# ielab/llm-rankers

Measured on AMD Instinct MI355X. Metric: passages/sec (pointwise yes_no reranking, flan-t5-large shape), higher is better.
Workload: dtype f16 (MFMA inputs), f32 accumulate + residual stream

## Files before the change

### llm-rankers_amd/csrc/rk_engine.hip

```cpp
#include <hip/hip_runtime.h>
#include <dlfcn.h>
#include <rccl/rccl.h>

#include <algorithm>
#include <cmath>
#include <cstdarg>
#include <cstdio>
#include <cstdlib>
#include <cstring>
#include <map>
#include <atomic>
#include <string>
#include <vector>

#include "../../include/rk_engine.h"
#include "attention.h"
#include "attention_d128.h"
#include "decoder_kernels.h"
#include "gemm.h"
#include "gemv_rows.h"
#include "llama_kernels.h"
#include "llama_kernels_hd64.h"
#include "llama_kernels_qknorm.h"
#include "misc_kernels.h"
// ... 36 lines not shown
struct Gemm;

struct NormStream {
  float* hidden = nullptr;
  half_t* xraw[2] = {nullptr, nullptr};
  float* ssq[2] = {nullptr, nullptr};
  float* factors = nullptr;
  half_t* xn = nullptr;
  int rows = 0; bool fold = false;
  int cur = 0, nb = 0;
  void begin(rk_engine* e, hipStream_t st, const int* ids, int rows_, bool fold_);
  const half_t* x() const { return fold ? xraw[cur] : xn; }
  Gemm consumer(rk_engine* e, hipStream_t st, const float* ln, Gemm c, bool own_factors) const;
  int producer(rk_engine* e, hipStream_t st, Gemm c, bool stats = true);
};

template <class T>
struct Grown {
  T* p = nullptr; size_t cap = 0;
  Grown() = default;
  Grown(const Grown&) = delete;
  Grown& operator=(const Grown&) = delete;
  ~Grown() { if (p) hipFree(p); }
  int reserve(rk_engine* e, size_t n, int* gen = nullptr);
};

enum DecBuf { IX_DEC_IDS, IX_OUT_IDS, IX_LAST_ROWS, IX_N_CACHED, IX_ROW_LABEL = IX_N_CACHED, IX_ROW_OFF, IX_OUT_IDX, IX_ROW_SEQ, IX_TREE_KEYS, IX_TREE_POS, IX_COUNT };
struct DecIndex {
  struct Src { DecBuf b; const std::vector<int>& v; };
  int* d[IX_COUNT] = {nullptr};
  int* pin = nullptr;
  static constexpr int PIN_INTS = 8192;
  int put(rk_engine* e, hipStream_t st, DecBuf b, const int* src, int n);
  int write(rk_engine* e, hipStream_t st, std::initializer_list<Src> srcs);
  int tree(rk_engine* e, hipStream_t st, std::vector<int>& sig, std::initializer_list<Src> srcs);
 private:
  std::vector<int> held[IX_N_CACHED], tree_sig;
  unsigned long epoch = 0, tree_epoch = ~0ul;
};

}

#define RK_SLOTS 2

struct Slot {
  hipStream_t se = nullptr, sd = nullptr;
  NormStream enc;
  half_t *qkv = nullptr, *ctx = nullptr, *ffh = nullptr, *enc_out = nullptr;
  int* d_tokens = nullptr; int* d_seq_off = nullptr;
  int* dec_seq_off = nullptr;
  int *stg_tokens[2] = {nullptr, nullptr}, *stg_seq_off[2] = {nullptr, nullptr};
  int gen = 0; bool gen_launched = false; unsigned stage_no = 0, off_of = 0;
  int n_seq = 0, T = 0, maxL = 0, minL = 0; bool staged = false; int last_floats = 0;
  half_t* cross_kv = nullptr;
  DecIndex idx; int* d_argmax = nullptr;
  NormStream dec;
  half_t *dqkv = nullptr, *dctx = nullptr, *dq = nullptr, *dffh = nullptr, *dlast = nullptr;
  float* dssq_few[2] = {nullptr, nullptr};
  half_t *xqk = nullptr, *xctx = nullptr;
  float *xpart = nullptr, *xstat = nullptr; bool have_cross_kv = false;
  float* d_scores = nullptr; float* h_scores = nullptr;
  hipEvent_t ev_enc[2] = {nullptr, nullptr}, ev_dec = nullptr; int enc_gen = -1; bool dec_pending = false;
};

struct rk_engine {
  rk_model_desc d{};
  int dev = 0;
  std::string err;
  bool finalized = false;
  int inner = 0;
  std::map<std::string, HostTensor> host;
  std::vector<void*> allocs;
  half_t *emb = nullptr, *lm_head = nullptr, *cross_kv_w = nullptr;
  std::vector<EncLayerW> enc;
  std::vector<DecLayerW> dec;
  float *enc_final_ln = nullptr, *dec_final_ln = nullptr, *lut_enc = nullptr, *lut_dec = nullptr;
  Grown<float> logits; int logits_gen = 0;
  Grown<float> amax_val; Grown<int> amax_idx; int amax_gen = 0;
  Grown<half_t> kv_cache; int kv_gen = 0;
  Grown<int> gen_buf; int* gen_pin = nullptr; hipEvent_t ev_gen[2] = {nullptr, nullptr};
  size_t scores_cap = 0;
  Slot slots[RK_SLOTS];
  struct Options {
    int glds = 1, skinny = 0x3F, overlap = 1, gemm_variant = 0, attn_short = 5, xattn_direct = 1, attn_heads_per_wg = 0, attn_ko = 0,
        gemm_persistent = 1, fold_norm = 1, s64_stages = 0, dec_fold_norm = 1, greedy_spec = 160, consumer_stats = 1, xattn_mfma = 1,
        dec_ffn_tiled = 1, gemm_split = 1, dec_fuse = 1, dec_fuse_rows = 0, dec_attn_seq = 1, attn_long = 1, attn_long_nw = 0,
        llama_attn_dma = 1, attn_long_xcd = 1, llama_attn_nw = 0, dec_graph = 1, gemm_sk = 1, dec_cross_mfma = 1, dec_gemv = 1, dec_gemv_rows = 4,
        dec_cached_attn = 1, llama_dec_r = 0, enc_serial = 0;
  } opt;
  float* attn_trace = nullptr;
  int n_cu = 256;
  struct SkWs { hipStream_t st = nullptr; float* slabs = nullptr; int* cnt = nullptr; };
  SkWs sk_ws[2 * RK_SLOTS];
  hipEvent_t t0 = nullptr, t1 = nullptr, t_tmp = nullptr;
  bool prof_on = false;
  std::vector<ProfRec> prof_recs; size_t prof_used = 0;
  double prof_flops[PC_COUNT] = {0}, prof_bytes[PC_COUNT] = {0}; int64_t prof_n[PC_COUNT] = {0};
  int family = 0; rk_llama_desc ld{};
  float rope_factor = 0.f, rope_low = 1.f, rope_high = 4.f; int rope_orig = 0;
  bool qkv_bias = false;
  bool qk_norm = false;
  int window = 0;
  std::vector<LlamaLayerW> ll; float *l_final_ln = nullptr, *rope_cos = nullptr, *rope_sin = nullptr; int* d_pos = nullptr;
  struct Sampling { float T = 0.f; int k = 0; float p = 1.f; bool on() const { return T > 0.f; } } samp;
  unsigned long long* d_seeds = nullptr;
  Grown<half_t> lkv; Grown<float> lpart; Grown<int> lints; int lkv_gen = 0;
  struct LlamaStep { NormStream stream; half_t *qkv = nullptr, *ctx = nullptr, *ffh = nullptr; } lg;
  struct LlamaSession {
    bool open = false; int n_slots = 0, max_len = 0, cap = 0, seen = 0;
    std::vector<int> busy, told, len, max_new, col, done;
    bool sampled = false; std::vector<unsigned long long> seeds;
  } ls;
  struct GraphEntry { int seen = 0; bool failed = false; hipGraphExec_t exec = nullptr; };
  std::map<std::vector<int>, GraphEntry> graphs; int opt_epoch = 0;
  struct GraphCount { int64_t eager = 0, captures = 0, replays = 0, failed = 0, evictions = 0; } graph_count;
  ncclComm_t comm = nullptr; int comm_rank = 0, comm_world = 1;
  float* d_gather[RK_SLOTS] = {nullptr}; float* h_gather[RK_SLOTS] = {nullptr}; size_t gather_cap = 0;
  hipEvent_t ev_gather[RK_SLOTS] = {nullptr}; bool gather_pending[RK_SLOTS] = {false}; int gather_n[RK_SLOTS] = {0};
  float *d_gsend = nullptr, *d_gall = nullptr, *h_gall = nullptr, *h_gstage = nullptr;
  hipEvent_t ev_gall = nullptr, ev_append = nullptr; bool gall_pending = false, append_foreign = false; int gall_n = 0;
};

namespace {

int fail(rk_engine* e, int code, const char* fmt, ...) {
  char buf[1024];
  va_list ap;
  va_start(ap, fmt);
  vsnprintf(buf, sizeof buf, fmt, ap);
  va_end(ap);
  if (e) e->err = buf; else g_create_error = buf;
  return code;
}

#define HIPCHK(E, call)                                                                              \
  do {                                                                                               \
    hipError_t _s = (call);                                                                          \
    if (_s != hipSuccess) return fail((E), RK_ERR_HIP, "%s failed: %s", #call, hipGetErrorString(_s)); \
  } while (0)
#define RC(x) do { rc = (x); if (rc) return rc; } while (0)

template <class T>
int dalloc(rk_engine* e, T** p, size_t n) {
  void* q = nullptr;
  HIPCHK(e, hipMalloc(&q, std::max<size_t>(n, 1) * sizeof(T)));
  e->allocs.push_back(q);
  *p = (T*)q;
  return RK_OK;
}

template <class T>
int upload(rk_engine* e, T** p, const T* src, size_t n) {
  int rc = dalloc(e, p, n);
  if (rc) return rc;
  HIPCHK(e, hipMemcpy(*p, src, n * sizeof(T), hipMemcpyHostToDevice));
  return RK_OK;
}

struct Bracket {
  rk_engine* e; hipStream_t st; int idx = -1;
  Bracket(rk_engine* e_, hipStream_t st_, int cls, double flops, double bytes) : e(e_), st(st_) {
    if (!e->prof_on) return;
    if (e->prof_used == e->prof_recs.size()) {
      ProfRec r{};
      if (hipEventCreate(&r.a) != hipSuccess || hipEventCreate(&r.b) != hipSuccess) return;
      e->prof_recs.push_back(r);
    }
    idx = (int)e->prof_used++;
    e->prof_recs[idx].cls = cls;
    e->prof_flops[cls] += flops; e->prof_bytes[cls] += bytes; e->prof_n[cls]++;
    hipEventRecord(e->prof_recs[idx].a, st);
  }
  ~Bracket() { if (idx >= 0) hipEventRecord(e->prof_recs[idx].b, st); }
};

hipStream_t enc_stream(rk_engine* e, Slot& sl) { return e->opt.overlap ? e->slots[(&sl - e->slots) & 1].se : e->slots[0].se; }
hipStream_t dec_stream(rk_engine* e, Slot& sl) { return e->opt.overlap ? sl.sd : e->slots[0].se; }

template <auto K, class Args>
void launch_lds(hipStream_t st, dim3 grid, dim3 block, int lds, int opt_in, const Args& a) {
  static std::atomic<uint64_t> done{0};
  if (opt_in > 0) {
    int dev = 0;
    if (hipGetDevice(&dev) != hipSuccess) dev = 0;
    const uint64_t bit = 1ull << (dev & 63);
    if (!(done.load(std::memory_order_acquire) & bit)) {
      hipError_t rc = hipFuncSetAttribute((const void*)K, hipFuncAttributeMaxDynamicSharedMemorySize, opt_in);
      if (rc != hipSuccess) fprintf(stderr, "[rk_engine] hipFuncSetAttribute(%d B LDS) failed: %s\n", opt_in, hipGetErrorString(rc));
      done.fetch_or(bit, std::memory_order_release);
    }
  }
  hipLaunchKernelGGL(K, grid, block, lds, st, a);
}

// ... 748 lines not shown
  else launch_lds<attn_causal128_dma_kernel<4>>(st, p.grid, p.block, p.lds, p.lds_opt_in, a);
}
int refuse_window(rk_engine* e, const char* entry, int maxL) {
  return fail(e, RK_ERR_STATE, "%s: a sequence of %d tokens on an engine with sliding window %d needs a windowed attention kernel, and option llama_attn_dma = 0 selects attn_causal128_kernel, which has none", entry, maxL, e->window);
}

struct LlamaDecAttnPlan { int R = 1, nch = 1, hd = 128, window = 0; dim3 grid, cgrid; };
LlamaDecAttnPlan plan_llama_dec_attn(const rk_engine* e, int rows, int P, int n_heads, int n_kv) {
  LlamaDecAttnPlan p;
  const int G = n_heads / n_kv;
  p.hd = head_width(e);
  p.R = G % 8 == 0 ? 8 : (G % 4 == 0 ? 4 : (G % 2 == 0 ? 2 : 1));
  if (e->opt.llama_dec_r == 1) p.R = 1;
  if (e->opt.llama_dec_r == 2 && G == 7 && p.hd == 128) p.R = 7;
  p.nch = (P + LDC_CHUNK - 1) / LDC_CHUNK;
  p.grid = dim3(p.nch, n_heads / p.R, rows);
  p.cgrid = dim3(n_heads, rows);
  p.window = e->window;
  return p;
}

void launch_llama_dec_attn(rk_engine* e, hipStream_t st, const LlamaDecAttnPlan& p, LlamaDecAttnArgs a, int rows) {
  a.nch = p.nch; a.window = p.window;
  Bracket br(e, st, PC_DEC_ATTN, 4.0 * rows * (double)a.P * a.n_heads * p.hd, 2.0 * rows * (double)a.P * a.n_kv * p.hd * 2.0);
  with_width(p.hd, [&](auto W) {
    constexpr int D = decltype(W)::value;
    auto go = [&](auto rc) {
      constexpr int R = decltype(rc)::value;
      if constexpr (R == 7 && D != 128) abort();
      else if (a.qkn) {
        if constexpr (D == 128) hipLaunchKernelGGL((attn_dec_cached_qkn_kernel<D, R>), p.grid, dim3(256), 0, st, a);
        else abort();
      }
      else if (p.window > 0) {
        if (a.bias) hipLaunchKernelGGL((attn_dec_cached_win_kernel<D, R, true>), p.grid, dim3(256), 0, st, a);
        else hipLaunchKernelGGL((attn_dec_cached_win_kernel<D, R, false>), p.grid, dim3(256), 0, st, a);
      }
      else if (a.bias) hipLaunchKernelGGL((attn_dec_cached_kernel<D, R, true>), p.grid, dim3(256), 0, st, a);
      else hipLaunchKernelGGL((attn_dec_cached_kernel<D, R, false>), p.grid, dim3(256), 0, st, a);
    };
    using std::integral_constant;
    switch (p.R) {
      case 8: go(integral_constant<int, 8>{}); break;
      case 7: go(integral_constant<int, 7>{}); break;
      case 4: go(integral_constant<int, 4>{}); break;
      case 2: go(integral_constant<int, 2>{}); break;
      default: go(integral_constant<int, 1>{}); break;
    }
    if (p.window > 0) hipLaunchKernelGGL(attn_dec_combine_win_kernel<D>, p.cgrid, dim3(D), 0, st, a);
    else hipLaunchKernelGGL(attn_dec_combine_kernel<D>, p.cgrid, dim3(D), 0, st, a);
  });
}

int wait_prev_decoder(rk_engine* e, Slot& sl) {
  hipStream_t se = enc_stream(e, sl);
  if (sl.dec_pending && dec_stream(e, sl) != se) HIPCHK(e, hipStreamWaitEvent(se, sl.ev_dec, 0));
  return RK_OK;
}

int run_encoder(rk_engine* e, Slot& sl, bool need_cross_kv) {
  const rk_model_desc& d = e->d;
  hipStream_t st = enc_stream(e, sl);
  const int T = sl.T, I = e->inner, dm = d.d_model, F = d.d_ff;
  const bool own = e->opt.consumer_stats != 0;
  int rc = RK_OK;
  NormStream ns = sl.enc;
  const EncAttnPlan ap = plan_enc_attn(e, sl.n_seq, sl.maxL, sl.minL, d.n_heads);
  const int* seq_off = sl.stg_seq_off[sl.gen];
  ns.begin(e, st, sl.stg_tokens[sl.gen], T, e->opt.fold_norm != 0);
  for (int l = 0; l < d.n_enc_layers; ++l) {
    const EncLayerW& w = e->enc[l];
    const bool last = l + 1 == d.n_enc_layers;
    RC(gemm(e, st, ns.consumer(e, st, w.ln0, Gemm(PC_ENC_GEMM_QKV, EPI_STORE_F16, ns.x(), dm, ns.fold ? w.qkv_f : w.qkv, dm, sl.qkv, 3 * I, T, 3 * I, dm), own)));
    launch_enc_attn(e, st, EncAttnCall{sl.qkv, sl.ctx, seq_off, e->lut_enc, 3 * I, I, I, d.n_heads, sl.n_seq, sl.maxL, sl.T}, ap);
    RC(ns.producer(e, st, Gemm(PC_ENC_GEMM_O, EPI_RESID_F32, sl.ctx, I, w.o, I, ns.hidden, dm, T, dm, I)));
    RC(gemm(e, st, ns.consumer(e, st, w.ln1, Gemm(PC_ENC_GEMM_FFN_IN, d.gated_gelu ? EPI_GEGLU_F16 : EPI_RELU_F16, ns.x(), dm, ns.fold ? w.ffn_in_f : w.ffn_in, dm,
                                                 sl.ffh, F, T, d.gated_gelu ? 2 * F : F, dm), own)));
    RC(ns.producer(e, st, Gemm(PC_ENC_GEMM_FFN_OUT, EPI_RESID_F32, sl.ffh, F, w.ffn_out, F, ns.hidden, dm, T, dm, F), !last));
  }
  RC(wait_prev_decoder(e, sl));
  if (sl.off_of != sl.stage_no) {
    HIPCHK(e, hipMemcpyAsync(sl.dec_seq_off, seq_off, (size_t)(sl.n_seq + 1) * sizeof(int), hipMemcpyDeviceToDevice, st));
    sl.off_of = sl.stage_no;
  }
  rmsnorm(e, st, ns.hidden, e->enc_final_ln, sl.enc_out, nullptr, T);
  if (need_cross_kv)
    RC(gemm(e, st, Gemm(PC_GEMM_CROSS_KV, EPI_STORE_F16, sl.enc_out, dm, e->cross_kv_w, dm, sl.cross_kv, 2 * I, T, d.n_dec_layers * 2 * I, dm)
                       .split(2 * I, (long)d.max_tokens * 2 * I)));
  sl.have_cross_kv = need_cross_kv;
  HIPCHK(e, hipGetLastError());
  return RK_OK;
}

struct DecRows {
  int rows; const int* keys; const int* pos; const int* seq;
  const int* row_off; int seq0, n_seq; bool cross_kv; const int* ids;
  bool tree() const { return keys != nullptr; }
};
struct DecCache { half_t* kv; int P; const int* pos; const int* tree_keys; int* tree_pos; };
void launch_dec_cached_step(const rk_engine* e, hipStream_t st, const AttnCachedArgs& ca, int B, int H, const int* tree_keys, int* tree_pos) {
  if (e->opt.dec_cached_attn) {
    hipLaunchKernelGGL(attn_dec_cached_kernel, dim3(H, B), dim3(256), attn_dec_lds(ca.P), st, ca);
  } else {
    hipLaunchKernelGGL(kv_append_kernel, dim3(B), dim3(256), 0, st, ca, tree_pos);
    hipLaunchKernelGGL(attn_dec_kernel, dim3(1, H, B), dim3(256), attn_dec_lds(ca.P), st,
                       AttnDecArgs{ca.qkv, ca.ldqkv, ca.cache, ca.cache + ca.inner, 2 * ca.inner, nullptr, ca.ctx, ca.ldctx, ca.bias_lut, ca.P, 1, ca.P,
                                   tree_keys, tree_pos});
  }
}
int run_decoder(rk_engine* e, Slot& sl, int Ld, const DecRows* rows = nullptr, const DecCache* cache = nullptr) {
  const rk_model_desc& d = e->d;
  hipStream_t st = dec_stream(e, sl);
  const bool tree = rows && rows->tree(), ragged = rows && !rows->tree();
  const int B = ragged ? rows->n_seq : sl.n_seq, M = rows ? rows->rows : B * Ld, I = e->inner, dm = d.d_model, F = d.d_ff;
  const bool have_kv = ragged ? rows->cross_kv : sl.have_cross_kv;
  const int* seq_off = sl.dec_seq_off + (ragged ? rows->seq0 : 0);
  const DecLenClass lc = dec_len_class(e, Ld);
  if (tree && (have_kv || lc.one)) return fail(e, RK_ERR_STATE, "the tree form needs the query-side cross-attention and L_d >= 2");
  if (ragged && have_kv && !sl.have_cross_kv) return fail(e, RK_ERR_STATE, "the ragged pass needs the K / V the encoder did not materialise");
  if (cache && (rows || have_kv || Ld != 1)) return fail(e, RK_ERR_STATE, "the incremental pass needs the query-side cross-attention and one row per sequence");
  if (wide_heads(e) && (!lc.one || rows || cache || have_kv || e->opt.dec_fuse == 2))
    return refuse_wide(e, "run_decoder", "this pass would launch a 64-wide kernel");
  const bool ws = lc.stream;
  const bool dfold = ws && e->opt.dec_fold_norm && (e->opt.skinny & 0x3F) == 0x3F;
  const bool fuse_asked = e->opt.dec_fuse == 2 || (e->opt.dec_fuse == 1 && lc.one);
  const bool few = dfold && e->opt.dec_gemv && !lc.one && M <= e->opt.dec_gemv_rows && !fuse_asked &&
                   gemv_fits(M, dm) && gemv_fits(M, I) && gemv_fits(M, F);
  const GemmFamily fam = few ? GEMM_GEMV : (ws ? GEMM_STREAM : GEMM_TILED);
  int rc = RK_OK;
  NormStream ns = sl.dec;
  if (few) { ns.ssq[0] = sl.dssq_few[0]; ns.ssq[1] = sl.dssq_few[1]; }
  auto normed = [&](const float* ln, Gemm c) { return ns.consumer(e, st, ln, c.on(fam), true); };
  auto resid = [&](Gemm c, bool stats = true) { return ns.producer(e, st, c.on(fam), stats); };
  ns.begin(e, st, ragged && rows->ids ? rows->ids : sl.idx.d[IX_DEC_IDS], M, dfold);
  const DecAttnPlan self_plan = plan_dec_attn(e, false, B, Ld, Ld, d.n_heads, tree ? rows->rows : 0);
  const DecAttnPlan cross_plan = plan_dec_attn(e, true, B, Ld, sl.maxL, d.n_heads, 0);
  for (int l = 0; l < d.n_dec_layers; ++l) {
    const DecLayerW& w = e->dec[l];
    if (!cache && lc.one) {
      RC(resid(normed(w.ln0, Gemm(PC_DEC_GEMM, EPI_RESID_F32, ns.x(), dm, dfold ? w.ov_f : w.ov, dm, ns.hidden, dm, M, dm, dm))));
    } else {
      RC(gemm(e, st, normed(w.ln0, Gemm(PC_DEC_GEMM, EPI_STORE_F16, ns.x(), dm, dfold ? w.qkv_f : w.qkv, dm, sl.dqkv, 3 * I, M, 3 * I, dm))));
      if (cache) {
        const AttnCachedArgs ca{sl.dqkv, 3 * I, cache->kv + (size_t)l * B * cache->P * 2 * I, cache->P, I, cache->pos, sl.dctx, I, e->lut_dec};
        Bracket br(e, st, PC_DEC_ATTN, 4.0 * B * (double)cache->P * I, (double)B * cache->P * 2 * I * 2.0);
        launch_dec_cached_step(e, st, ca, B, d.n_heads, cache->tree_keys, cache->tree_pos);
      } else {
        launch_dec_attn(e, st, self_plan, AttnDecArgs{sl.dqkv, 3 * I, sl.dqkv + I, sl.dqkv + 2 * I, 3 * I, nullptr, sl.dctx, I, e->lut_dec, Ld, 1, Ld,
                                                      tree ? rows->keys : nullptr, tree ? rows->pos : nullptr, 0, ragged ? rows->row_off : nullptr},
                        4.0 * M * Ld * I, 0);
      }
      RC(resid(Gemm(PC_DEC_GEMM, EPI_RESID_F32, sl.dctx, I, w.o, I, ns.hidden, dm, M, dm, I)));
    }
    const Gemm cq = normed(w.ln1, Gemm(PC_DEC_GEMM, EPI_STORE_F16, ns.x(), dm, dfold ? w.cq_f : w.cq, dm, sl.dq, I, M, I, dm));
    if (!have_kv) {
      RC(run_xattn_chain(e, st, XAttnChain{cq.A, cq.lda, cq.W, w.ckT, e->cross_kv_w + ((size_t)l * 2 * I + I) * dm, cq.fold, cq.family,
                                           sl.enc_out, sl.dec_seq_off, rows ? rows->seq : nullptr, Ld, 0, sl.dq, sl.xqk, sl.xpart, sl.xstat, sl.xctx,
                                           sl.dctx, I, M, d.n_heads, dm, sl.maxL, sl.T, fuse_asked, head_width(e)}));
    } else {
      RC(gemm(e, st, cq));
      const half_t* kv = sl.cross_kv + (size_t)l * d.max_tokens * 2 * I;
      launch_dec_attn(e, st, cross_plan, AttnDecArgs{sl.dq, I, kv, kv + I, 2 * I, seq_off, sl.dctx, I, nullptr, Ld, 0, sl.maxL, nullptr, nullptr, 0,
                                                       ragged ? rows->row_off : nullptr},
                      4.0 * Ld * (double)sl.T * I, (double)sl.T * 2 * I * 2.0);
    }
    RC(resid(Gemm(PC_DEC_GEMM, EPI_RESID_F32, sl.dctx, I, w.co, I, ns.hidden, dm, M, dm, I)));
    {
      const bool tiled_in = dfold && e->opt.dec_ffn_tiled && lc.one;
      RC(gemm(e, st, ns.consumer(e, st, w.ln2, Gemm(PC_DEC_GEMM, d.gated_gelu ? EPI_GEGLU_F16 : EPI_RELU_F16, ns.x(), dm, dfold ? w.ffn_in_f : w.ffn_in, dm,
                                                   sl.dffh, F, M, d.gated_gelu ? 2 * F : F, dm).on(tiled_in ? GEMM_TILED : fam), true)));
    }
    RC(resid(Gemm(PC_DEC_GEMM, EPI_RESID_F32, sl.dffh, F, w.ffn_out, F, ns.hidden, dm, M, dm, F), l + 1 < d.n_dec_layers));
  }
  HIPCHK(e, hipGetLastError());
  return RK_OK;
}

int encoder_then_handoff_kv(rk_engine* e, Slot& sl, bool need_cross_kv) {
  hipStream_t se = enc_stream(e, sl), sd = dec_stream(e, sl);
  if (need_cross_kv && !sl.cross_kv) return refuse_wide(e, "encoder", "the materialised cross-attention K / V are not allocated");
  static_assert(RK_SLOTS == 2, "the other slot");
  const Slot& other = e->slots[(&sl - e->slots) ^ 1];
  if (e->opt.enc_serial && sd != se && other.enc_gen >= 0) HIPCHK(e, hipStreamWaitEvent(se, other.ev_enc[other.enc_gen], 0));
  sl.gen_launched = true;
  const int rc = run_encoder(e, sl, need_cross_kv);
  HIPCHK(e, hipEventRecord(sl.ev_enc[sl.gen], se));
  sl.enc_gen = sl.gen;
  if (rc) return rc;
  if (sd != se) HIPCHK(e, hipStreamWaitEvent(sd, sl.ev_enc[sl.gen], 0));
  return RK_OK;
}

int encoder_then_handoff(rk_engine* e, Slot& sl, int max_ld, bool query_side = false) {
  return encoder_then_handoff_kv(e, sl, !query_side && !use_xattn_direct(e, sl, max_ld));
}

int mark_decoder_done(rk_engine* e, Slot& sl) {
  HIPCHK(e, hipEventRecord(sl.ev_dec, dec_stream(e, sl)));
  sl.dec_pending = true;
  return RK_OK;
}

int sync_all(rk_engine* e) {
  for (Slot& sl : e->slots) {
    HIPCHK(e, hipStreamSynchronize(sl.se));
    HIPCHK(e, hipStreamSynchronize(sl.sd));
  }
  return RK_OK;
}

int finish_blocking(rk_engine* e, Slot& sl) {
  int rc = mark_decoder_done(e, sl);
  if (rc || (rc = sync_all(e))) return rc;
  sl.dec_pending = false;
  return RK_OK;
}

template <class T>
int Grown<T>::reserve(rk_engine* e, size_t n, int* gen) {
  if (n <= cap) return RK_OK;
  int rc = sync_all(e);
  if (rc) return rc;
  if (p) HIPCHK(e, hipFree(p));
  p = nullptr; cap = 0;
  HIPCHK(e, hipMalloc((void**)&p, n * sizeof(T)));
  cap = n;
  if (gen) ++*gen;
  return RK_OK;
}

int ensure_logits(rk_engine* e, size_t rows) {
  return e->logits.reserve(e, rows * (2 * ((size_t)(e->d.vocab + 31) / 32) + 1), &e->logits_gen);
}

float head_scale(const rk_engine* e) {
  return e->d.tied_head ? 1.0f / std::sqrt((float)e->d.d_model) : 1.0f;
}

int check_batch(rk_engine* e, Slot* sl, const int32_t* tokens, const int32_t* off, int n_seq) {
  if (!e->finalized) return fail(e, RK_ERR_STATE, "engine not finalized");
  if (!tokens || !off || n_seq <= 0) return fail(e, RK_ERR_INVALID, "empty batch (n_seq=%d)", n_seq);
  if (n_seq > e->d.max_seqs) return fail(e, RK_ERR_CAPACITY, "n_seq %d > max_seqs %d", n_seq, e->d.max_seqs);
  if (off[0] != 0) return fail(e, RK_ERR_INVALID, "seq_offsets[0] must be 0");
  int maxL = 0, minL = 1 << 30;
  for (int b = 0; b < n_seq; ++b) {
    const int L = off[b + 1] - off[b];
    if (L <= 0) return fail(e, RK_ERR_INVALID, "sequence %d is empty", b);
    maxL = std::max(maxL, L);
    minL = std::min(minL, L);
  }
  const int T = off[n_seq];
  if (T > e->d.max_tokens) return fail(e, RK_ERR_CAPACITY, "%d tokens > max_tokens %d", T, e->d.max_tokens);
  for (int t = 0; t < T; ++t)
    if (tokens[t] < 0 || tokens[t] >= e->d.vocab) return fail(e, RK_ERR_INVALID, "token id %d out of range at %d", tokens[t], t);
  if (attn_dec_lds(maxL) > 160 * 1024 || maxL > 65536)
    return fail(e, RK_ERR_CAPACITY, "sequence of %d tokens exceeds the cross-attention LDS budget", maxL);
  if (sl) { sl->maxL = maxL; sl->minL = minL; sl->T = T; sl->n_seq = n_seq; }
  return RK_OK;
}

int check_ids(rk_engine* e, const int32_t* ids, int n, const char* what) {
  for (int i = 0; i < n; ++i)
    if (ids[i] < 0 || ids[i] >= e->d.vocab) return fail(e, RK_ERR_INVALID, "%s id %d out of range", what, ids[i]);
  return RK_OK;
}

int put_dec_ids_shared(rk_engine* e, Slot& sl, const int32_t* prefix, int Ld) {
  std::vector<int> ids((size_t)sl.n_seq * Ld);
  for (int b = 0; b < sl.n_seq; ++b) memcpy(&ids[(size_t)b * Ld], prefix, Ld * sizeof(int));
  return sl.idx.put(e, dec_stream(e, sl), IX_DEC_IDS, ids.data(), (int)ids.size());
}

void shift_right(const int32_t* labels, int n, std::vector<int>* out) {
  for (int t = 0; t < n; ++t) out->push_back(t ? labels[t - 1] : 0);
}

int check_greedy_args(rk_engine* e, const int32_t* dec_prefix, int dec_len, int max_new) {
  if (!dec_prefix || dec_len <= 0 || max_new <= 0 || dec_len + max_new - 1 > e->d.max_dec_len)
    return fail(e, RK_ERR_CAPACITY, "dec_len %d + max_new %d exceeds max_dec_len %d", dec_len, max_new, e->d.max_dec_len);
  return RK_OK;
}

int read_scores_blocking(rk_engine* e, Slot& sl, hipStream_t st, size_t n, float* out) {
  HIPCHK(e, hipMemcpyAsync(sl.h_scores, sl.d_scores, n * sizeof(float), hipMemcpyDeviceToHost, st));
  if (e->family == 0) { const int rc = finish_blocking(e, sl); if (rc) return rc; }
  else HIPCHK(e, hipStreamSynchronize(st));
  HIPCHK(e, hipGetLastError());
  memcpy(out, sl.h_scores, n * sizeof(float));
  return RK_OK;
}

int stage_slot(rk_engine* e, int slot, const int32_t* tokens, const int32_t* seq_offsets, int n_seq) {
  if (slot < 0 || slot >= RK_SLOTS) return fail(e, RK_ERR_INVALID, "slot %d out of range", slot);
  if (e->family != 0) return fail(e, RK_ERR_STATE, "T5 entry point called on a Llama engine (use rk_llama_*)");
  int rc = set_device(e);
  if (rc) return rc;
  Slot& sl = e->slots[slot];
  sl.staged = false;
  if ((rc = check_batch(e, &sl, tokens, seq_offsets, n_seq))) return rc;
  const int g = sl.gen_launched ? sl.gen ^ 1 : sl.gen;
  HIPCHK(e, hipEventSynchronize(sl.ev_enc[g]));
  HIPCHK(e, hipMemcpy(sl.stg_tokens[g], tokens, (size_t)sl.T * sizeof(int), hipMemcpyHostToDevice));
  HIPCHK(e, hipMemcpy(sl.stg_seq_off[g], seq_offsets, (size_t)(n_seq + 1) * sizeof(int), hipMemcpyHostToDevice));
  sl.gen = g; sl.gen_launched = false; ++sl.stage_no;
  sl.staged = true;
  return RK_OK;
}

enum GraphKind { GK_T5_SCORE, GK_T5_GREEDY_STEP, GK_T5_GREEDY2, GK_T5_GENERATE_STEP, GK_LLAMA_STEP, GK_T5_COMPARE, GK_LLAMA_SESSION_STEP, GK_LLAMA_STEP_SAMPLED, GK_LLAMA_SESSION_STEP_SAMPLED };
int evict_graphs(rk_engine* e, const rk_engine::GraphEntry* keep) {
  for (Slot& sl : e->slots) HIPCHK(e, hipStreamSynchronize(sl.sd));
  HIPCHK(e, hipStreamSynchronize(e->slots[0].se));
  for (auto it = e->graphs.begin(); it != e->graphs.end();) {
    if (&it->second == keep) { ++it; continue; }
    if (it->second.exec) { hipGraphExecDestroy(it->second.exec); ++e->graph_count.evictions; }
    it = e->graphs.erase(it);
  }
  return RK_OK;
}
template <class F>
int run_graphed(rk_engine* e, hipStream_t st, std::vector<int> key, F&& body) {
  auto& n = e->graph_count;
  auto eager = [&]() -> int { ++n.eager; return body(); };
  key.push_back(e->opt_epoch);
  if (!e->opt.dec_graph || e->prof_on) return eager();
  auto& g = e->graphs[key];
  if (g.exec) { HIPCHK(e, hipGraphLaunch(g.exec, st)); ++n.replays; return RK_OK; }
  if ((int)e->graphs.size() > RK_GRAPH_CACHE_KEYS) {
    const int rc = evict_graphs(e, &g);
    if (rc) return rc;
  }
  if (g.failed || g.seen++ == 0) return eager();
  auto failed = [&]() -> int { g.failed = true; ++n.failed; return eager(); };
  hipGraph_t graph = nullptr;
  if (hipStreamBeginCapture(st, hipStreamCaptureModeThreadLocal) != hipSuccess) { (void)hipGetLastError(); return failed(); }
  const int rc = body();
  const hipError_t ec = hipStreamEndCapture(st, &graph);
  if (rc != RK_OK || ec != hipSuccess || !graph) {
    (void)hipGetLastError();
    if (graph) hipGraphDestroy(graph);
    if (rc != RK_OK) { g.failed = true; ++n.failed; return rc; }
    return failed();
  }
  const hipError_t ei = hipGraphInstantiate(&g.exec, graph, nullptr, nullptr, 0);
  hipGraphDestroy(graph);
  if (ei != hipSuccess || !g.exec) { (void)hipGetLastError(); g.exec = nullptr; return failed(); }
  HIPCHK(e, hipGraphLaunch(g.exec, st));
  ++n.captures;
  return RK_OK;
}

int ensure_decode_ring(rk_engine* e) {
  if (e->gen_pin) return RK_OK;
  HIPCHK(e, hipHostMalloc((void**)&e->gen_pin, 16 * sizeof(int), hipHostMallocDefault));
  for (hipEvent_t& ev : e->ev_gen) HIPCHK(e, hipEventCreateWithFlags(&ev, hipEventDisableTiming));
  return RK_OK;
}
template <class F>
int decode_cached(rk_engine* e, hipStream_t st, const std::vector<int>& key, F&& step, int forced, int first_col, int n_seq, int max_new,
                  const int* d_word, const int* d_out, int32_t* out_tokens, int32_t* out_steps) {
  int* pin = e->gen_pin;
  auto request = [&](int c) -> int {
    HIPCHK(e, hipMemcpyAsync(pin + (c & 1), d_word, sizeof(int), hipMemcpyDeviceToHost, st));
    HIPCHK(e, hipEventRecord(e->ev_gen[c & 1], st));
    return RK_OK;
  };
  int rc = RK_OK;
  if (first_col > 0) RC(request(first_col - 1));
  bool stop = false;
  for (int c = first_col - forced; c < max_new && !stop; ++c) {
    RC(run_graphed(e, st, key, step));
    if (c >= 0) RC(request(c));
    if (c >= 1) {
      HIPCHK(e, hipEventSynchronize(e->ev_gen[(c - 1) & 1]));
      stop = pin[(c - 1) & 1] != 0;
    }
  }
  std::vector<int> res((size_t)n_seq * max_new + 1);
  HIPCHK(e, hipMemcpyAsync(res.data(), d_out, (size_t)n_seq * max_new * sizeof(int), hipMemcpyDeviceToHost, st));
  HIPCHK(e, hipMemcpyAsync(res.data() + (size_t)n_seq * max_new, d_word, sizeof(int), hipMemcpyDeviceToHost, st));
  HIPCHK(e, hipStreamSynchronize(st));
  HIPCHK(e, hipGetLastError());
  memcpy(out_tokens, res.data(), (size_t)n_seq * max_new * sizeof(int));
  if (out_steps) *out_steps = res[(size_t)n_seq * max_new];
  return RK_OK;
}

int score_slot(rk_engine* e, int slot, const int32_t* dec_prefix, int dec_len, const int32_t* out_token_ids, int n_out) {
  if (slot < 0 || slot >= RK_SLOTS) return fail(e, RK_ERR_INVALID, "slot %d out of range", slot);
  int rc = set_device(e);
  if (rc) return rc;
  Slot& sl = e->slots[slot];
  if (!sl.staged) return fail(e, RK_ERR_STATE, "no staged batch in slot %d", slot);
  if (!dec_prefix || dec_len <= 0 || dec_len > e->d.max_dec_len) return fail(e, RK_ERR_CAPACITY, "dec_len %d out of range (max %d)", dec_len, e->d.max_dec_len);
  if (!out_token_ids || n_out <= 0 || n_out > 64) return fail(e, RK_ERR_INVALID, "n_out must be in 1..64 (got %d)", n_out);
  if ((rc = check_ids(e, dec_prefix, dec_len, "decoder")) || (rc = check_ids(e, out_token_ids, n_out, "output"))) return rc;
  if (wide_heads(e) && dec_len > 1) return refuse_wide(e, "rk_t5_score", "dec_len > 1 has no 128-wide decoder self-attention");
  if ((rc = check_wide_one(e, "rk_t5_score"))) return rc;
  hipStream_t sd = dec_stream(e, sl);
  if ((rc = put_dec_ids_shared(e, sl, dec_prefix, dec_len))) return rc;
  if ((rc = sl.idx.put(e, sd, IX_OUT_IDS, out_token_ids, n_out))) return rc;
  std::vector<int> rows(sl.n_seq);
  for (int b = 0; b < sl.n_seq; ++b) rows[b] = b * dec_len + dec_len - 1;
  if ((rc = sl.idx.put(e, sd, IX_LAST_ROWS, rows.data(), sl.n_seq))) return rc;
  if ((rc = encoder_then_handoff(e, sl, dec_len))) return rc;
#ifdef RK_MEASURE
  static const bool skip_dec = getenv("RK_DEBUG_SKIP_DECODER") != nullptr;
#else
  constexpr bool skip_dec = false;
#endif
  rc = run_graphed(e, sd, {GK_T5_SCORE, slot, sl.n_seq, dec_len, sl.have_cross_kv ? sl.maxL : (sl.maxL + 63) / 64, (int)sl.have_cross_kv, n_out, (int)skip_dec}, [&]() -> int {
    int r = RK_OK;
    if (!skip_dec && (r = run_decoder(e, sl, dec_len))) return r;
    rmsnorm(e, sd, sl.dec.hidden, e->dec_final_ln, sl.dlast, sl.idx.d[IX_LAST_ROWS], sl.n_seq, head_scale(e));
    Bracket br(e, sd, PC_HEAD, 2.0 * sl.n_seq * n_out * e->d.d_model, 0);
    launch_head_rows(sd, sl.dlast, e->lm_head, sl.idx.d[IX_OUT_IDS], sl.d_scores, sl.n_seq, n_out, e->d.d_model);
    return RK_OK;
  });
  if (rc) return rc;
  HIPCHK(e, hipMemcpyAsync(sl.h_scores, sl.d_scores, (size_t)sl.n_seq * n_out * sizeof(float), hipMemcpyDeviceToHost, sd));
  HIPCHK(e, hipGetLastError());
  sl.last_floats = sl.n_seq * n_out;
  return mark_decoder_done(e, sl);
}

int compare_slot(rk_engine* e, int slot, int dec_start_id, int false_id, int true_id) {
  if (slot < 0 || slot >= RK_SLOTS) return fail(e, RK_ERR_INVALID, "slot %d out of range", slot);
  if (e->family != 0) return fail(e, RK_ERR_STATE, "T5 entry point called on a Llama engine (use rk_llama_*)");
  int rc = set_device(e);
  if (rc) return rc;
  Slot& sl = e->slots[slot];
  if (!sl.staged) return fail(e, RK_ERR_STATE, "no staged batch in slot %d", slot);
  if (sl.n_seq % 2) return fail(e, RK_ERR_INVALID, "a compare needs pairs of sequences (staged n_seq = %d)", sl.n_seq);
  const int32_t out_ids[2] = {false_id, true_id};
  if ((rc = check_ids(e, &dec_start_id, 1, "decoder")) || (rc = check_ids(e, out_ids, 2, "output"))) return rc;
  if (false_id == true_id) return fail(e, RK_ERR_INVALID, "false_id and true_id are the same id %d", false_id);
  if ((rc = check_wide_one(e, "rk_t5_compare"))) return rc;
  hipStream_t sd = dec_stream(e, sl);
  if ((rc = put_dec_ids_shared(e, sl, &dec_start_id, 1))) return rc;
  std::vector<int> rows(sl.n_seq);
  for (int b = 0; b < sl.n_seq; ++b) rows[b] = b;
  if ((rc = sl.idx.put(e, sd, IX_LAST_ROWS, rows.data(), sl.n_seq))) return rc;
  if ((rc = encoder_then_handoff(e, sl, 1))) return rc;
  rc = run_graphed(e, sd, {GK_T5_COMPARE, slot, sl.n_seq, sl.have_cross_kv ? sl.maxL : (sl.maxL + 63) / 64, (int)sl.have_cross_kv, false_id, true_id}, [&]() -> int {
    int r = RK_OK;
    if ((r = run_decoder(e, sl, 1))) return r;
    rmsnorm(e, sd, sl.dec.hidden, e->dec_final_ln, sl.dlast, sl.idx.d[IX_LAST_ROWS], sl.n_seq, head_scale(e));
    Bracket br(e, sd, PC_HEAD, 2.0 * sl.n_seq * 2 * e->d.d_model, 0);
    launch_pair_verdict(sd, sl.dlast, e->lm_head, false_id, true_id, sl.d_scores, sl.n_seq, e->d.d_model);
    return RK_OK;
  });
  if (rc) return rc;
  const int n_floats = 3 * sl.n_seq + sl.n_seq / 2;
  HIPCHK(e, hipMemcpyAsync(sl.h_scores, sl.d_scores, (size_t)n_floats * sizeof(float), hipMemcpyDeviceToHost, sd));
  HIPCHK(e, hipGetLastError());
  sl.last_floats = n_floats;
  return mark_decoder_done(e, sl);
}


struct RcclApi {
  void* h = nullptr; bool tried = false; std::string err;
  decltype(&ncclGetUniqueId) GetUniqueId = nullptr;
  decltype(&ncclCommInitRank) CommInitRank = nullptr;
  decltype(&ncclCommDestroy) CommDestroy = nullptr;
  decltype(&ncclAllGather) AllGather = nullptr;
  decltype(&ncclGetErrorString) GetErrorString = nullptr;
  decltype(&ncclGetVersion) GetVersion = nullptr;
};
RcclApi g_rccl;

std::string mapped_rccl_path() {
  FILE* f = fopen("/proc/self/maps", "r");
  if (!f) return "";
  char line[4096];
  std::string found;
  while (fgets(line, sizeof line, f)) {
    const char* p = strstr(line, "librccl");
    if (!p) continue;
    const char* path = strchr(line, '/');
    if (!path) continue;
    found.assign(path);
    while (!found.empty() && (found.back() == '\n' || found.back() == ' ')) found.pop_back();
// ... 81 lines not shown
    return fail(nullptr, RK_ERR_INVALID, "d_kv=%d unsupported: the gfx950 attention kernels are built for d_kv=64 and, for one decoder position, d_kv=128", d.d_kv);
  if (d.d_model % 64 || (d.n_heads * d.d_kv) % 64 || d.d_ff % 64 || d.vocab % 4)
    return fail(nullptr, RK_ERR_INVALID, "d_model, n_heads*d_kv, d_ff must be multiples of 64 and vocab of 4");
  if (d.d_model > 4096)
    return fail(nullptr, RK_ERR_INVALID, "d_model=%d unsupported: rmsnorm_kernel holds a row of at most 4096 columns in registers (d_model <= 4096)", d.d_model);
  if (d.max_distance > RK_LUT_R || d.n_buckets < 4 || d.n_buckets > 256)
    return fail(nullptr, RK_ERR_INVALID, "relative attention config unsupported (max_distance<=%d)", RK_LUT_R);
  if (d.max_tokens <= 0 || d.max_seqs <= 0 || d.max_dec_len <= 0 || d.n_enc_layers <= 0 || d.n_dec_layers <= 0)
    return fail(nullptr, RK_ERR_INVALID, "capacities and layer counts must be positive");
  if ((long)d.max_seqs * d.max_dec_len > 8192 * 8) return fail(nullptr, RK_ERR_INVALID, "max_seqs*max_dec_len too large");
  int n_dev = 0;
  if (hipGetDeviceCount(&n_dev) != hipSuccess || n_dev <= 0)
    return fail(nullptr, RK_ERR_NO_DEVICE, "no HIP device visible: this engine has no CPU path");
  if (device_ordinal < 0 || device_ordinal >= n_dev)
    return fail(nullptr, RK_ERR_NO_DEVICE, "device ordinal %d out of range (%d devices)", device_ordinal, n_dev);
  hipDeviceProp_t prop;
  if (hipGetDeviceProperties(&prop, device_ordinal) != hipSuccess)
    return fail(nullptr, RK_ERR_HIP, "hipGetDeviceProperties failed");
  if (strncmp(prop.gcnArchName, "gfx950", 6) != 0)
    return fail(nullptr, RK_ERR_NO_DEVICE, "device %d is %s; kernels are built for gfx950 (MI355X) only", device_ordinal, prop.gcnArchName);
  rk_engine* e = new rk_engine();
  e->d = d; e->dev = device_ordinal; e->n_cu = prop.multiProcessorCount > 0 ? prop.multiProcessorCount : 256; e->inner = d.n_heads * d.d_kv;
  int prio_lo = 0, prio_hi = 0;
  bool ok = hipSetDevice(device_ordinal) == hipSuccess;
  ok = ok && hipDeviceGetStreamPriorityRange(&prio_lo, &prio_hi) == hipSuccess;
  for (int i = 0; ok && i < RK_SLOTS; ++i)
    ok = hipStreamCreateWithPriority(&e->slots[i].se, hipStreamNonBlocking, prio_lo) == hipSuccess &&
         hipStreamCreateWithPriority(&e->slots[i].sd, hipStreamNonBlocking, prio_hi) == hipSuccess;
  ok = ok && hipEventCreate(&e->t0) == hipSuccess && hipEventCreate(&e->t1) == hipSuccess &&
       hipEventCreateWithFlags(&e->t_tmp, hipEventDisableTiming) == hipSuccess;
  for (int i = 0; ok && i < RK_SLOTS; ++i)
    ok = hipEventCreateWithFlags(&e->slots[i].ev_enc[0], hipEventDisableTiming) == hipSuccess &&
         hipEventCreateWithFlags(&e->slots[i].ev_enc[1], hipEventDisableTiming) == hipSuccess &&
         hipEventCreateWithFlags(&e->slots[i].ev_dec, hipEventDisableTiming) == hipSuccess;
  for (int i = 0; ok && i < 2 * RK_SLOTS; ++i) {
    rk_engine::SkWs& w = e->sk_ws[i];
    w.st = (i & 1) ? e->slots[i >> 1].sd : e->slots[i >> 1].se;
    ok = hipMalloc((void**)&w.slabs, (size_t)KSPLIT_MAX_SLABS * 65536 * sizeof(float)) == hipSuccess &&
         hipMalloc((void**)&w.cnt, KSPLIT_MAX_SLABS * sizeof(int)) == hipSuccess &&
         hipMemset(w.cnt, 0, KSPLIT_MAX_SLABS * sizeof(int)) == hipSuccess;
  }
  if (!ok) {
    for (auto& w : e->sk_ws) { if (w.slabs) hipFree(w.slabs); if (w.cnt) hipFree(w.cnt); }
    delete e;
    return fail(nullptr, RK_ERR_HIP, "stream/event/workspace creation failed");
  }
  *out = e;
  return RK_OK;
}

void rk_engine_destroy(rk_engine* e) {
  if (!e) return;
  hipSetDevice(e->dev);
  for (auto& sl : e->slots) {
    if (sl.se) hipStreamSynchronize(sl.se);
    if (sl.sd) hipStreamSynchronize(sl.sd);
  }
  comm_release(e);
  for (auto& kv : e->graphs) if (kv.second.exec) hipGraphExecDestroy(kv.second.exec);
  e->graphs.clear();
  for (void* p : e->allocs) hipFree(p);
  if (e->gen_pin) hipHostFree(e->gen_pin);
  for (hipEvent_t ev : e->ev_gen) if (ev) hipEventDestroy(ev);
  for (auto& w : e->sk_ws) { if (w.slabs) hipFree(w.slabs); if (w.cnt) hipFree(w.cnt); }
  for (auto& sl : e->slots) {
    if (sl.h_scores) hipHostFree(sl.h_scores);
    if (sl.idx.pin) hipHostFree(sl.idx.pin);
    for (hipEvent_t ev : sl.ev_enc) if (ev) hipEventDestroy(ev);
    if (sl.ev_dec) hipEventDestroy(sl.ev_dec);
  }
  for (auto& r : e->prof_recs) { hipEventDestroy(r.a); hipEventDestroy(r.b); }
  if (e->t0) hipEventDestroy(e->t0);
  if (e->t1) hipEventDestroy(e->t1);
  if (e->t_tmp) hipEventDestroy(e->t_tmp);
  for (auto& sl : e->slots) {
    if (sl.se) hipStreamDestroy(sl.se);
    if (sl.sd) hipStreamDestroy(sl.sd);
  }
  delete e;
}

int rk_engine_load_tensor(rk_engine* e, const char* hf_name, const void* data, int dtype, const int64_t* shape, int ndim) {
  if (!e || !hf_name || !data || !shape) return fail(e, RK_ERR_INVALID, "null argument");
  if (e->finalized) return fail(e, RK_ERR_STATE, "engine already finalized");
  if (ndim < 1 || ndim > 2) return RK_OK;
  std::string name(hf_name);
  if (name == "encoder.embed_tokens.weight" || name == "decoder.embed_tokens.weight") return RK_OK;
  size_t n = 1;
  for (int i = 0; i < ndim; ++i) n *= (size_t)shape[i];
  HostTensor t;
  t.shape.assign(shape, shape + ndim);
  const bool keep_f32 = ndim == 1 || name.find("relative_attention_bias") != std::string::npos;
  auto get = [&](size_t i) -> float {
    switch (dtype) {
      case RK_F32: return ((const float*)data)[i];
      case RK_F16: return (float)((const half_t*)data)[i];
      case RK_BF16: { uint32_t u = (uint32_t)((const uint16_t*)data)[i] << 16; float f; memcpy(&f, &u, 4); return f; }
      default: return 0.f;
    }
  };
  if (dtype < RK_F32 || dtype > RK_BF16) return fail(e, RK_ERR_INVALID, "unknown dtype %d", dtype);
  if (keep_f32) { t.f.resize(n); for (size_t i = 0; i < n; ++i) t.f[i] = get(i); }
  else if (dtype == RK_F16) { t.h.assign((const half_t*)data, (const half_t*)data + n); }
  else { t.h.resize(n); for (size_t i = 0; i < n; ++i) t.h[i] = (half_t)get(i); }
  e->host[name] = std::move(t);
  return RK_OK;
}

static int llama_finalize(rk_engine* e);

// ... 91 lines not shown
    RC(up_f(&w.ln1, Fv(p + ".1.layer_norm.weight")));
    RC(up_h(&w.qkv_f, folded(cat3(p + ".0.SelfAttention."), Fv(p + ".0.layer_norm.weight"))));
    RC(up_h(&w.ffn_in_f, folded(ffn_in(p + ".1.DenseReluDense"), Fv(p + ".1.layer_norm.weight"))));
  }
  e->dec.resize(d.n_dec_layers);
  std::vector<half_t> ckv;
  ckv.reserve((size_t)d.n_dec_layers * 2 * I * dm);
  for (int l = 0; l < d.n_dec_layers; ++l) {
    const std::string p = "decoder.block." + std::to_string(l) + ".layer";
    DecLayerW& w = e->dec[l];
    RC(up_h(&w.qkv, cat3(p + ".0.SelfAttention.")));
    RC(up_h(&w.o, H(p + ".0.SelfAttention.o.weight")));
    RC(up_h(&w.cq, H(p + ".1.EncDecAttention.q.weight")));
    RC(up_h(&w.co, H(p + ".1.EncDecAttention.o.weight")));
    RC(up_h(&w.ckT, regroup_ckT(H(p + ".1.EncDecAttention.k.weight").data(), d.n_heads, dm, d.d_kv)));
    RC(up_h(&w.ffn_in, ffn_in(p + ".2.DenseReluDense")));
    RC(up_h(&w.ffn_out, H(p + ".2.DenseReluDense.wo.weight")));
    RC(up_f(&w.ln0, Fv(p + ".0.layer_norm.weight")));
    RC(up_f(&w.ln1, Fv(p + ".1.layer_norm.weight")));
    RC(up_f(&w.ln2, Fv(p + ".2.layer_norm.weight")));
    RC(up_h(&w.qkv_f, folded(cat3(p + ".0.SelfAttention."), Fv(p + ".0.layer_norm.weight"))));
    RC(up_h(&w.cq_f, folded(H(p + ".1.EncDecAttention.q.weight"), Fv(p + ".1.layer_norm.weight"))));
    RC(up_h(&w.ffn_in_f, folded(ffn_in(p + ".2.DenseReluDense"), Fv(p + ".2.layer_norm.weight"))));
    for (const char* m : {"k", "v"}) { const auto& s = H(p + ".1.EncDecAttention." + m + ".weight"); ckv.insert(ckv.end(), s.begin(), s.end()); }
  }
  RC(up_h(&e->cross_kv_w, ckv));
  {
    half_t* d_vT = nullptr; float* d_ov32 = nullptr;
    RC(dalloc(e, &d_vT, (size_t)dm * I)); RC(dalloc(e, &d_ov32, (size_t)dm * dm));
    std::vector<half_t> vT((size_t)dm * I), ov16((size_t)dm * dm);
    std::vector<float> ov32((size_t)dm * dm);
    for (int l = 0; l < d.n_dec_layers; ++l) {
      const std::string p = "decoder.block." + std::to_string(l) + ".layer.0.SelfAttention.";
      const auto& wv = H(p + "v.weight");
      for (int j = 0; j < I; ++j)
        for (int k = 0; k < dm; ++k) vT[(size_t)k * I + j] = wv[(size_t)j * dm + k];
      HIPCHK(e, hipMemcpy(d_vT, vT.data(), vT.size() * 2, hipMemcpyHostToDevice));
      RC(gemm(e, e->slots[0].se, Gemm(PC_OTHER, EPI_STORE_F32, e->dec[l].o, I, d_vT, I, d_ov32, dm, dm, dm, I)));
      HIPCHK(e, hipStreamSynchronize(e->slots[0].se));
      HIPCHK(e, hipMemcpy(ov32.data(), d_ov32, ov32.size() * 4, hipMemcpyDeviceToHost));
      for (size_t i = 0; i < ov32.size(); ++i) ov16[i] = (half_t)ov32[i];
      RC(up_h(&e->dec[l].ov, ov16));
      const auto& ln0 = Fv("decoder.block." + std::to_string(l) + ".layer.0.layer_norm.weight");
      for (size_t i = 0; i < ov32.size(); ++i) ov16[i] = (half_t)(ov32[i] * ln0[i % dm]);
      RC(up_h(&e->dec[l].ov_f, ov16));
    }
    HIPCHK(e, hipGetLastError());
  }
  e->host.clear();

  const size_t Tc = d.max_tokens, Bc = d.max_seqs, Mc = (size_t)d.max_seqs * d.max_dec_len;
  e->scores_cap = Bc * 64;
  if (2 * e->scores_cap < 7 * Bc) return fail(e, RK_ERR_CAPACITY, "score buffer of %zu floats cannot hold a compare of %zu sequences", e->scores_cap, Bc);
  for (Slot& sl : e->slots) {
    RC(dalloc(e, &sl.enc.hidden, Tc * dm)); RC(dalloc(e, &sl.enc.xn, Tc * dm)); RC(dalloc(e, &sl.qkv, Tc * 3 * I));
    RC(dalloc(e, &sl.ctx, Tc * I)); RC(dalloc(e, &sl.ffh, Tc * F)); RC(dalloc(e, &sl.enc_out, Tc * dm));
    RC(dalloc(e, &sl.enc.xraw[0], Tc * dm)); RC(dalloc(e, &sl.enc.ssq[0], Tc * ((dm + 63) / 64))); RC(dalloc(e, &sl.enc.factors, Tc + 512));
    HIPCHK(e, hipMemset(sl.enc.factors, 0, (Tc + 512) * sizeof(float)));
    for (int g = 0; g < 2; ++g) { RC(dalloc(e, &sl.stg_tokens[g], Tc)); RC(dalloc(e, &sl.stg_seq_off[g], Bc + 1)); }
    RC(dalloc(e, &sl.dec_seq_off, Bc + 1));
    if (!wide_heads(e)) RC(dalloc(e, &sl.cross_kv, (size_t)d.n_dec_layers * Tc * 2 * I));
    RC(dalloc(e, &sl.idx.d[IX_DEC_IDS], Mc)); RC(dalloc(e, &sl.idx.d[IX_LAST_ROWS], Bc)); RC(dalloc(e, &sl.idx.d[IX_OUT_IDS], 8192));
    RC(dalloc(e, &sl.idx.d[IX_ROW_LABEL], Mc)); RC(dalloc(e, &sl.idx.d[IX_ROW_OFF], 2 * Bc + 1)); RC(dalloc(e, &sl.idx.d[IX_OUT_IDX], Bc)); RC(dalloc(e, &sl.d_argmax, Bc));
    RC(dalloc(e, &sl.idx.d[IX_ROW_SEQ], Mc)); RC(dalloc(e, &sl.idx.d[IX_TREE_KEYS], Mc * (size_t)d.max_dec_len)); RC(dalloc(e, &sl.idx.d[IX_TREE_POS], Mc));
    RC(dalloc(e, &sl.dec.hidden, Mc * dm)); RC(dalloc(e, &sl.dec.xn, Mc * dm)); RC(dalloc(e, &sl.dqkv, Mc * 3 * I));
    RC(dalloc(e, &sl.dctx, Mc * I)); RC(dalloc(e, &sl.dq, Mc * I)); RC(dalloc(e, &sl.dffh, Mc * F));
    RC(dalloc(e, &sl.dlast, Bc * dm));
    for (int i = 0; i < 2; ++i) { RC(dalloc(e, &sl.dec.xraw[i], Mc * dm)); RC(dalloc(e, &sl.dec.ssq[i], Mc * ((dm + 31) / 32))); RC(dalloc(e, &sl.dssq_few[i], (size_t)GEMV_MAX_ROWS * e->n_cu)); }
    RC(dalloc(e, &sl.dec.factors, Mc));
    RC(dalloc(e, &sl.xqk, (size_t)XA_MAX_ROWS * d.n_heads * dm)); RC(dalloc(e, &sl.xctx, (size_t)XA_MAX_ROWS * d.n_heads * dm));
    RC(dalloc(e, &sl.xpart, (size_t)XA_MAX_CHUNKS * d.n_heads * dm)); RC(dalloc(e, &sl.xstat, (size_t)XA_MAX_CHUNKS * d.n_heads * 2));
    RC(dalloc(e, &sl.d_scores, e->scores_cap));
    HIPCHK(e, hipHostMalloc((void**)&sl.h_scores, e->scores_cap * sizeof(float), hipHostMallocDefault));
    HIPCHK(e, hipHostMalloc((void**)&sl.idx.pin, IX_N_CACHED * DecIndex::PIN_INTS * sizeof(int), hipHostMallocDefault));
  }
  const int dec_smem_max = (int)attn_dec_lds(std::max(d.max_tokens, d.max_dec_len));
  (void)hipFuncSetAttribute((const void*)attn_dec_kernel, hipFuncAttributeMaxDynamicSharedMemorySize, std::min(dec_smem_max, 160 * 1024));
  (void)hipFuncSetAttribute((const void*)attn_dec_seq_kernel, hipFuncAttributeMaxDynamicSharedMemorySize, 160 * 1024);
#define GEMM_ATTR(EPI)                                                                                              \
  (void)hipFuncSetAttribute((const void*)gemm_f16_kernel<EPI, true>, hipFuncAttributeMaxDynamicSharedMemorySize, GEMM_LDS_BYTES); \
  (void)hipFuncSetAttribute((const void*)gemm_f16_kernel<EPI, false>, hipFuncAttributeMaxDynamicSharedMemorySize, GEMM_LDS_BYTES);
  GEMM_ATTR(EPI_STORE_F16) GEMM_ATTR(EPI_RESID_F32) GEMM_ATTR(EPI_GEGLU_F16) GEMM_ATTR(EPI_RELU_F16) GEMM_ATTR(EPI_STORE_F32) GEMM_ATTR(EPI_SWIGLU_F16)
#undef GEMM_ATTR
  (void)hipGetLastError();
  HIPCHK(e, hipDeviceSynchronize());
  e->finalized = true;
  return RK_OK;
}

int rk_t5_stage_slot(rk_engine* e, int slot, const int32_t* tokens, const int32_t* seq_offsets, int n_seq) {
  if (!e) return RK_ERR_INVALID;
  return stage_slot(e, slot, tokens, seq_offsets, n_seq);
}
int rk_t5_stage(rk_engine* e, const int32_t* tokens, const int32_t* seq_offsets, int n_seq) {
  return rk_t5_stage_slot(e, 0, tokens, seq_offsets, n_seq);
}

int rk_t5_score_slot(rk_engine* e, int slot, const int32_t* dec_prefix, int dec_len, const int32_t* out_token_ids, int n_out) {
  if (!e) return RK_ERR_INVALID;
  return score_slot(e, slot, dec_prefix, dec_len, out_token_ids, n_out);
}
int rk_t5_score_staged(rk_engine* e, const int32_t* dec_prefix, int dec_len, const int32_t* out_token_ids, int n_out) {
  return rk_t5_score_slot(e, 0, dec_prefix, dec_len, out_token_ids, n_out);
}

int rk_engine_sync(rk_engine* e) {
  if (!e) return RK_ERR_INVALID;
  int rc = set_device(e);
  if (rc) return rc;
  return sync_all(e);
}

int rk_t5_read_scores_slot(rk_engine* e, int slot, float* out_logits, int n_floats) {
  if (!e || !out_logits || slot < 0 || slot >= RK_SLOTS) return RK_ERR_INVALID;
  Slot& sl = e->slots[slot];
  if (n_floats > sl.last_floats) return fail(e, RK_ERR_INVALID, "asked for %d floats, have %d", n_floats, sl.last_floats);
  if (sl.dec_pending) { HIPCHK(e, hipEventSynchronize(sl.ev_dec)); sl.dec_pending = false; }
  memcpy(out_logits, sl.h_scores, (size_t)n_floats * sizeof(float));
  return RK_OK;
}
int rk_t5_read_scores(rk_engine* e, float* out_logits, int n_floats) { return rk_t5_read_scores_slot(e, 0, out_logits, n_floats); }

int rk_t5_scores_device_ptr(rk_engine* e, void** out_ptr) {
  if (!e || !out_ptr) return RK_ERR_INVALID;
  *out_ptr = e->slots[0].d_scores;
  return RK_OK;
}

int rk_engine_num_slots(void) { return RK_SLOTS; }

int rk_t5_score(rk_engine* e, const int32_t* tokens, const int32_t* seq_offsets, int n_seq, const int32_t* dec_prefix,
                int dec_len, const int32_t* out_token_ids, int n_out, float* out_logits) {
  int rc;
  if ((rc = rk_t5_stage(e, tokens, seq_offsets, n_seq))) return rc;
  if ((rc = rk_t5_score_staged(e, dec_prefix, dec_len, out_token_ids, n_out))) return rc;
  return rk_t5_read_scores(e, out_logits, n_seq * n_out);
}

int rk_t5_compare_slot(rk_engine* e, int slot, int dec_start_id, int false_id, int true_id) {
  if (!e) return RK_ERR_INVALID;
  return compare_slot(e, slot, dec_start_id, false_id, true_id);
}

int rk_t5_compare(rk_engine* e, const int32_t* tokens, const int32_t* seq_offsets, int n_pairs, int dec_start_id, int false_id,
                  int true_id, float* out_logits, float* out_p_true, int32_t* out_first_wins) {
  if (!e) return RK_ERR_INVALID;
  if (n_pairs <= 0 || n_pairs > (1 << 28) || !out_logits || !out_p_true || !out_first_wins) return fail(e, RK_ERR_INVALID, "empty compare (n_pairs=%d)", n_pairs);
  const int n_seq = 2 * n_pairs;
  int rc;
  if ((rc = rk_t5_stage(e, tokens, seq_offsets, n_seq))) return rc;
  if ((rc = rk_t5_compare_slot(e, 0, dec_start_id, false_id, true_id))) return rc;
  std::vector<float> res((size_t)7 * n_pairs);
  if ((rc = rk_t5_read_scores(e, res.data(), 7 * n_pairs))) return rc;
  memcpy(out_logits, res.data(), (size_t)2 * n_seq * sizeof(float));
  memcpy(out_p_true, res.data() + (size_t)2 * n_seq, (size_t)n_seq * sizeof(float));
  for (int p = 0; p < n_pairs; ++p) out_first_wins[p] = res[(size_t)3 * n_seq + p] != 0.f;
  return RK_OK;
}

struct QlmPass { int s0, n_seq, r0, rows, ld, off0; bool cross_kv; };

static int run_qlm(rk_engine* e, Slot& sl, const std::vector<QlmPass>& passes, float* out_scores) {
  hipStream_t sd = dec_stream(e, sl);
  int* const* ix = sl.idx.d;
  int rc = RK_OK, max_rows = 0;
  bool need_kv = false;
  for (const QlmPass& p : passes) { max_rows = std::max(max_rows, p.rows); need_kv = need_kv || p.cross_kv; }
  RC(ensure_logits(e, (size_t)max_rows));
  RC(encoder_then_handoff_kv(e, sl, need_kv));
  const int nblk = (e->d.vocab + 31) / 32, dm = e->d.d_model;
  for (const QlmPass& p : passes) {
    const bool ragged = p.off0 >= 0;
    const int* off = ragged ? ix[IX_ROW_OFF] + p.off0 : nullptr;
    const DecRows rows{p.rows, nullptr, nullptr, ix[IX_ROW_SEQ] + p.r0, off, p.s0, p.n_seq, p.cross_kv, ix[IX_DEC_IDS] + p.r0};
    RC(run_decoder(e, sl, p.ld, ragged ? &rows : nullptr));
    rmsnorm(e, sd, sl.dec.hidden, e->dec_final_ln, sl.dec.xn, nullptr, p.rows, head_scale(e));
    float* xlab = e->logits.p + (size_t)p.rows * nblk * 2;
    RC(gemm(e, sd, Gemm(PC_HEAD, EPI_LSE_F32, sl.dec.xn, dm, e->lm_head, dm, e->logits.p, nblk, p.rows, e->d.vocab, dm).lse(ix[IX_ROW_LABEL] + p.r0, xlab)));
    launch_qlm_lse(sd, (const float2*)e->logits.p, nblk, xlab, ragged ? 0 : p.ld, off, ragged ? ix[IX_OUT_IDX] + p.s0 : nullptr, sl.d_scores, p.n_seq);
  }
  return read_scores_blocking(e, sl, sd, (size_t)sl.n_seq, out_scores);
}

int rk_t5_qlm(rk_engine* e, const int32_t* tokens, const int32_t* seq_offsets, int n_seq, const int32_t* labels,
              int n_labels, float* out_scores) {
  int rc;
  if (e && wide_heads(e)) return refuse_wide(e, "rk_t5_qlm", "qlm scores several decoder positions");
  if ((rc = rk_t5_stage(e, tokens, seq_offsets, n_seq))) return rc;
  Slot& sl = e->slots[0];
  if (!labels || n_labels <= 0 || n_labels > e->d.max_dec_len) return fail(e, RK_ERR_CAPACITY, "n_labels %d out of range (max %d)", n_labels, e->d.max_dec_len);
  if ((rc = check_ids(e, labels, n_labels, "label"))) return rc;
  std::vector<int> dec_in, row_label;
  shift_right(labels, n_labels, &dec_in);
  for (int b = 0; b < n_seq; ++b) row_label.insert(row_label.end(), labels, labels + n_labels);
  if ((rc = put_dec_ids_shared(e, sl, dec_in.data(), n_labels))) return rc;
  if ((rc = sl.idx.write(e, dec_stream(e, sl), {{IX_ROW_LABEL, row_label}}))) return rc;
  return run_qlm(e, sl, {{0, n_seq, 0, n_seq * n_labels, n_labels, -1, !use_xattn_direct(e, sl, n_labels)}}, out_scores);
}

int rk_t5_qlm_many(rk_engine* e, const int32_t* tokens, const int32_t* seq_offsets, int n_seq, const int32_t* labels,
                   const int32_t* label_offsets, float* out_scores) {
  if (!e) return RK_ERR_INVALID;
  if (e->family != 0) return fail(e, RK_ERR_STATE, "T5 entry point called on a Llama engine (use rk_llama_*)");
  if (wide_heads(e)) return refuse_wide(e, "rk_t5_qlm_many", "qlm scores several decoder positions");
  int rc;
  if ((rc = check_batch(e, nullptr, tokens, seq_offsets, n_seq))) return rc;
  if (!out_scores || !labels || !label_offsets || label_offsets[0] != 0) return fail(e, RK_ERR_INVALID, "labels, label_offsets (from 0) or output missing");
  const int max_ld = e->d.max_dec_len;
  auto n_of = [&](int b) { return label_offsets[b + 1] - label_offsets[b]; };
  for (int b = 0; b < n_seq; ++b)
    if (n_of(b) <= 0 || n_of(b) > max_ld) return fail(e, RK_ERR_CAPACITY, "sequence %d: n_labels %d out of range (max %d)", b, n_of(b), max_ld);
  if ((rc = check_ids(e, labels, label_offsets[n_seq], "label"))) return rc;
  std::vector<int> cls_of((size_t)max_ld + 1, 0), keys;
  std::vector<DecLenClass> classes;
  for (int n = 1; n <= max_ld; ++n) {
    const DecLenClass c = dec_len_class(e, n);
    size_t i = 0;
    while (i < keys.size() && keys[i] != c.key()) ++i;
    if (i == keys.size()) { keys.push_back(c.key()); classes.push_back(c); }
    cls_of[n] = (int)i;
  }
  std::vector<int> order((size_t)n_seq);
  for (int b = 0; b < n_seq; ++b) order[b] = b;
  std::stable_sort(order.begin(), order.end(), [&](int x, int y) { return cls_of[n_of(x)] < cls_of[n_of(y)]; });
  std::vector<int> ptok((size_t)seq_offsets[n_seq]), poff((size_t)n_seq + 1, 0);
  for (int s = 0; s < n_seq; ++s) {
    const int b = order[s], L = seq_offsets[b + 1] - seq_offsets[b];
    memcpy(&ptok[poff[s]], tokens + seq_offsets[b], (size_t)L * sizeof(int));
    poff[s + 1] = poff[s] + L;
  }
  if ((rc = rk_t5_stage(e, ptok.data(), poff.data(), n_seq))) return rc;
  Slot& sl = e->slots[0];
  std::vector<QlmPass> passes;
  std::vector<int> ids, rlab, rseq, roff;
  for (int s = 0; s < n_seq;) {
    const int cls = cls_of[n_of(order[s])];
    QlmPass p{s, 0, (int)ids.size(), 0, 0, (int)roff.size(), !classes[cls].direct};
    for (; s < n_seq && cls_of[n_of(order[s])] == cls; ++s, ++p.n_seq) {
      const int b = order[s], nb = n_of(b);
      const int32_t* lab = labels + label_offsets[b];
      roff.push_back(p.rows);
      shift_right(lab, nb, &ids);
      rlab.insert(rlab.end(), lab, lab + nb);
      rseq.insert(rseq.end(), nb, s);
      p.rows += nb; p.ld = std::max(p.ld, nb);
    }
    roff.push_back(p.rows);
    passes.push_back(p);
  }
  if ((rc = sl.idx.write(e, dec_stream(e, sl), {{IX_DEC_IDS, ids}, {IX_ROW_LABEL, rlab}, {IX_ROW_SEQ, rseq}, {IX_ROW_OFF, roff}, {IX_OUT_IDX, order}}))) return rc;
  return run_qlm(e, sl, passes, out_scores);
}

static int ensure_amax(rk_engine* e, size_t rows) {
  const size_t n = rows * ((size_t)(e->d.vocab + 31) / 32);
// ... 6 lines not shown
  if (rc == RK_OK) launch_argmax_blocks(st, e->amax_val.p, e->amax_idx.p, nblk, d_out, rows);
  return rc;
}
static int ensure_sample_head(rk_engine* e, size_t rows) {
  if (e->d.vocab > sampling::MAX_VOCAB) return fail(e, RK_ERR_STATE, "sampling head: vocabulary %d beyond %d (the fixed-point sums' headroom)", e->d.vocab, sampling::MAX_VOCAB);
  int rc = e->logits.reserve(e, rows * (size_t)e->d.vocab, &e->logits_gen);
  if (rc == RK_OK && !e->d_seeds) rc = dalloc(e, &e->d_seeds, (size_t)e->d.max_seqs);
  return rc;
}
static void launch_sample_rows(hipStream_t st, const float* logits, int n_logit_rows, int vocab, const rk_engine::Sampling& sp,
                               const unsigned long long* seeds, const int* seed_map, const int* pos, const int* pos_map, int pos_add,
                               int* d_out, int* kept, int rows) {
  hipLaunchKernelGGL(sample_rows_kernel, dim3(rows), dim3(sampling::THREADS), 0, st, logits, n_logit_rows, (long)vocab, vocab, sp.T, sp.k, sp.p,
                     seeds, seed_map, pos, pos_map, pos_add, d_out, kept);
}
static int head_sample(rk_engine* e, hipStream_t st, const half_t* x, int rows, int d_model, int vocab, const rk_engine::Sampling& sp,
                       const int* seed_map, const int* pos, const int* pos_map, int* d_out) {
  const int rc = gemm(e, st, Gemm(PC_HEAD, EPI_STORE_F32, x, d_model, e->lm_head, d_model, e->logits.p, vocab, rows, vocab, d_model).on(GEMM_STREAM));
  if (rc) return rc;
  Bracket br(e, st, PC_HEAD, 0, 10.0 * rows * vocab * 4.0);
  launch_sample_rows(st, e->logits.p, rows, vocab, sp, e->d_seeds, seed_map, pos, pos_map, 1, d_out, nullptr, rows);
  return RK_OK;
}
static int final_argmax(rk_engine* e, hipStream_t st, Slot& sl, const int* row_map, int rows) {
  rmsnorm(e, st, sl.dec.hidden, e->dec_final_ln, sl.dlast, row_map, rows, head_scale(e));
  return head_argmax(e, st, sl.dlast, rows, e->d.d_model, e->d.vocab, sl.d_argmax);
}
static int read_argmax(rk_engine* e, hipStream_t st, const Slot& sl, int* out, int n) {
  HIPCHK(e, hipMemcpyAsync(out, sl.d_argmax, (size_t)n * sizeof(int), hipMemcpyDeviceToHost, st));
  HIPCHK(e, hipStreamSynchronize(st));
  HIPCHK(e, hipGetLastError());
  return RK_OK;
}

static int greedy_step(rk_engine* e, Slot& sl, const std::vector<std::vector<int>>& rows, int Ld, std::vector<int>& amax) {
  const int n_seq = (int)rows.size();
  hipStream_t sd = dec_stream(e, sl);
  std::vector<int> flat((size_t)n_seq * Ld), rowmap(n_seq);
  for (int b = 0; b < n_seq; ++b) { memcpy(&flat[(size_t)b * Ld], rows[b].data(), Ld * sizeof(int)); rowmap[b] = b * Ld + Ld - 1; }
  int rc = sl.idx.write(e, sd, {{IX_DEC_IDS, flat}, {IX_LAST_ROWS, rowmap}});
  if (rc) return rc;
  rc = run_graphed(e, sd, {GK_T5_GREEDY_STEP, 0, n_seq, Ld, sl.have_cross_kv ? sl.maxL : (sl.maxL + 63) / 64, (int)sl.have_cross_kv, e->amax_gen}, [&]() -> int {
    const int r = run_decoder(e, sl, Ld);
    return r ? r : final_argmax(e, sd, sl, sl.idx.d[IX_LAST_ROWS], n_seq);
  });
  if (rc) return rc;
  amax.resize(n_seq);
  return read_argmax(e, sd, sl, amax.data(), n_seq);
}

int rk_t5_greedy(rk_engine* e, const int32_t* tokens, const int32_t* seq_offsets, int n_seq, const int32_t* dec_prefix,
                 int dec_len, int max_new, int eos_id, int pad_id, int32_t* out_tokens, int32_t* out_steps) {
  int rc;
  if (e && wide_heads(e)) return refuse_wide(e, "rk_t5_greedy", "greedy decoding runs the decoder self-attention");
  if ((rc = rk_t5_stage(e, tokens, seq_offsets, n_seq))) return rc;
  Slot& sl = e->slots[0];
  if ((rc = check_greedy_args(e, dec_prefix, dec_len, max_new))) return rc;
  if ((rc = check_ids(e, dec_prefix, dec_len, "decoder"))) return rc;
  if ((rc = ensure_amax(e, (size_t)n_seq))) return rc;
  if ((rc = encoder_then_handoff(e, sl, dec_len + max_new - 1))) return rc;
  std::vector<std::vector<int>> rows(n_seq, std::vector<int>(dec_prefix, dec_prefix + dec_len));
  std::vector<char> done(n_seq, 0);
  std::vector<int> amax(n_seq);
  for (int b = 0; b < n_seq; ++b)
    for (int t = 0; t < max_new; ++t) out_tokens[b * max_new + t] = pad_id;
  int steps = 0;
  for (int t = 0; t < max_new; ++t) {
    if ((rc = greedy_step(e, sl, rows, dec_len + t, amax))) return rc;
    ++steps;
    bool all_done = true;
    for (int b = 0; b < n_seq; ++b) {
      const int tok = done[b] ? pad_id : amax[b];
      out_tokens[b * max_new + t] = tok;
      rows[b].push_back(tok);
      if (tok == eos_id) done[b] = 1;
      all_done = all_done && done[b];
    }
    if (all_done) break;
  }
  if ((rc = finish_blocking(e, sl))) return rc;
  if (out_steps) *out_steps = steps;
  return RK_OK;
}

static int ensure_gen(rk_engine* e, int n_seq, int P) {
  const size_t L = (size_t)e->d.max_dec_len, S = (size_t)e->d.max_seqs;
  int rc = RK_OK;
  RC(e->kv_cache.reserve(e, (size_t)e->d.n_dec_layers * n_seq * P * 2 * e->inner, &e->kv_gen));
  RC(e->gen_buf.reserve(e, 8 + L + 2 * S + S * L + S * (L + 1)));
  return ensure_decode_ring(e);
}

int rk_t5_generate(rk_engine* e, const int32_t* tokens, const int32_t* seq_offsets, int n_seq, const int32_t* dec_prefix,
                   int dec_len, int max_new, int eos_id, int pad_id, int32_t* out_tokens, int32_t* out_steps) {
  int rc;
  if (e && wide_heads(e)) return refuse_wide(e, "rk_t5_generate", "cached decoding runs the decoder self-attention");
  if ((rc = rk_t5_stage(e, tokens, seq_offsets, n_seq))) return rc;
  Slot& sl = e->slots[0];
  if ((rc = check_greedy_args(e, dec_prefix, dec_len, max_new))) return rc;
  if (!out_tokens) return fail(e, RK_ERR_INVALID, "null output");
  if ((rc = check_ids(e, dec_prefix, dec_len, "decoder"))) return rc;
  const int P = dec_len + max_new;
  if ((rc = ensure_amax(e, (size_t)n_seq))) return rc;
  if ((rc = ensure_gen(e, n_seq, P))) return rc;
  if ((rc = encoder_then_handoff(e, sl, 1, true))) return rc;
  hipStream_t sd = dec_stream(e, sl);
  const size_t o_pre = 8, o_done = o_pre + dec_len, o_tpos = o_done + n_seq, o_out = o_tpos + n_seq, o_keys = o_out + (size_t)n_seq * max_new;
  const size_t n_ints = o_keys + (size_t)n_seq * P;
  std::vector<int> init(n_ints, 0);
  init[2] = eos_id; init[3] = pad_id;
  memcpy(&init[o_pre], dec_prefix, dec_len * sizeof(int));
  for (size_t k = 0; k < (size_t)n_seq * max_new; ++k) init[o_out + k] = pad_id;
  for (int b = 0; b < n_seq; ++b)
    for (int j = 0; j < P; ++j) init[o_keys + (size_t)b * P + j] = b * P + j;
  std::vector<int> ids0(n_seq, dec_prefix[0]);
  int* g = e->gen_buf.p;
  if ((rc = sl.idx.write(e, sd, {{IX_DEC_IDS, ids0}}))) return rc;
  HIPCHK(e, hipMemcpy(g, init.data(), n_ints * sizeof(int), hipMemcpyHostToDevice));
  const DecCache kc{e->kv_cache.p, P, g, g + o_keys, g + o_tpos};
  auto step = [&]() -> int {
    int r = run_decoder(e, sl, 1, nullptr, &kc);
    if (r || (r = final_argmax(e, sd, sl, nullptr, n_seq))) return r;
    Bracket br(e, sd, PC_OTHER, 0, 0);
    launch_greedy_advance(sd, sl.d_argmax, g, g + o_pre, g + o_done, g + o_out, sl.idx.d[IX_DEC_IDS], n_seq, dec_len, max_new);
    return RK_OK;
  };
  const std::vector<int> key{GK_T5_GENERATE_STEP, 0, n_seq, (sl.maxL + 63) / 64, dec_len, max_new, e->amax_gen, e->kv_gen};
  if ((rc = decode_cached(e, sd, key, step, dec_len - 1, 0, n_seq, max_new, g + 1, g + o_out, out_tokens, out_steps))) return rc;
  return finish_blocking(e, sl);
}

int rk_t5_greedy2(rk_engine* e, const int32_t* tokens, const int32_t* seq_offsets, int n_seq, const int32_t* dec_prefix,
                  int dec_len, const int32_t* cand_ids, int n_cand, int eos_id, int pad_id, int32_t* out_tokens, int32_t* out_steps) {
  if (!e) return RK_ERR_INVALID;
  if (wide_heads(e)) return refuse_wide(e, "rk_t5_greedy2", "greedy decoding runs the decoder self-attention");
  const int Ld = dec_len + 1;
  const long per_seq = (long)dec_len + n_cand;
  const long M = (long)n_seq * per_seq, R = (long)n_seq * (1 + n_cand);
  const bool fits = cand_ids && n_cand > 0 && dec_prefix && dec_len > 0 && Ld <= e->d.max_dec_len && R <= e->d.max_seqs &&
                    M <= (long)e->d.max_seqs * e->d.max_dec_len && M <= XA_MAX_ROWS && M <= e->opt.greedy_spec &&
                    use_xattn_direct(e, e->slots[0], Ld);
  if (!fits) return rk_t5_greedy(e, tokens, seq_offsets, n_seq, dec_prefix, dec_len, 2, eos_id, pad_id, out_tokens, out_steps);
  int rc;
  if ((rc = check_ids(e, cand_ids, n_cand, "candidate"))) return rc;
  if ((rc = rk_t5_stage(e, tokens, seq_offsets, n_seq))) return rc;
  Slot& sl = e->slots[0];
  if ((rc = check_ids(e, dec_prefix, dec_len, "decoder"))) return rc;
  if ((rc = ensure_amax(e, (size_t)R))) return rc;
  if ((rc = encoder_then_handoff(e, sl, Ld))) return rc;
  hipStream_t sd = dec_stream(e, sl);
  std::vector<int> ids((size_t)M), rows((size_t)R), rseq((size_t)M), rpos((size_t)M), keys((size_t)M * Ld, 0), amax((size_t)R);
  for (int b = 0; b < n_seq; ++b) {
    const int r0 = (int)(b * per_seq);
    for (int i = 0; i < dec_len; ++i) {
      const int r = r0 + i;
      ids[r] = dec_prefix[i]; rseq[r] = b; rpos[r] = i;
      for (int j = 0; j <= i; ++j) keys[(size_t)r * Ld + j] = r0 + j;
    }
    rows[b] = r0 + dec_len - 1;
    for (int c = 0; c < n_cand; ++c) {
      const int r = r0 + dec_len + c;
      ids[r] = cand_ids[c]; rseq[r] = b; rpos[r] = dec_len;
      for (int j = 0; j < dec_len; ++j) keys[(size_t)r * Ld + j] = r0 + j;
      keys[(size_t)r * Ld + dec_len] = r;
      rows[n_seq + b * n_cand + c] = r;
    }
  }
  std::vector<int> sig;
  sig.reserve(ids.size() + rows.size() + rseq.size() + rpos.size() + keys.size() + 2);
  sig.push_back(n_seq); sig.push_back(Ld);
  for (const std::vector<int>* v : {&ids, &rows, &rseq, &rpos, &keys}) sig.insert(sig.end(), v->begin(), v->end());
  if ((rc = sl.idx.tree(e, sd, sig, {{IX_DEC_IDS, ids}, {IX_LAST_ROWS, rows}, {IX_ROW_SEQ, rseq}, {IX_TREE_POS, rpos}, {IX_TREE_KEYS, keys}}))) return rc;
  const DecRows tree{(int)M, sl.idx.d[IX_TREE_KEYS], sl.idx.d[IX_TREE_POS], sl.idx.d[IX_ROW_SEQ]};
  rc = run_graphed(e, sd, {GK_T5_GREEDY2, 0, n_seq, Ld, (sl.maxL + 63) / 64, n_cand, e->amax_gen}, [&]() -> int {
    const int r = run_decoder(e, sl, Ld, &tree);
    return r ? r : final_argmax(e, sd, sl, sl.idx.d[IX_LAST_ROWS], (int)R);
  });
  if (rc || (rc = read_argmax(e, sd, sl, amax.data(), (int)R))) return rc;
  bool all_done = true, miss = false;
  for (int b = 0; b < n_seq; ++b) {
    const int t1 = amax[b];
    out_tokens[b * 2] = t1;
    out_tokens[b * 2 + 1] = pad_id;
    if (t1 == eos_id) continue;
    all_done = false;
    int c = 0;
    while (c < n_cand && cand_ids[c] != t1) ++c;
// ... 525 lines not shown
  }
  int nf = 0;
  for (int b = 0; b < ls.n_slots; ++b)
    if (ls.busy[b] && ls.done[b] && !ls.told[b]) { out_finished[nf++] = b; ls.told[b] = 1; }
  *out_n_finished = nf;
  if (out_steps) *out_steps = steps;
  return RK_OK;
}

int rk_llama_session_read(rk_engine* e, int slot, int32_t* out_tokens, int cap, int32_t* out_n) {
  int rc = session_check(e, "rk_llama_session_read");
  if (rc) return rc;
  auto& ls = e->ls;
  if (!out_tokens || !out_n) return fail(e, RK_ERR_INVALID, "null output");
  if (slot < 0 || slot >= ls.n_slots) return fail(e, RK_ERR_INVALID, "slot %d out of range (the session has %d)", slot, ls.n_slots);
  if (!ls.busy[slot] || !ls.done[slot]) return fail(e, RK_ERR_STATE, "slot %d %s", slot, ls.busy[slot] ? "has not finished" : "is idle");
  const int n = ls.col[slot];
  if (cap < n) return fail(e, RK_ERR_CAPACITY, "slot %d holds %d tokens, the caller's buffer %d", slot, n, cap);
  const SessionInts d = session_ints(e);
  HIPCHK(e, hipMemcpy(out_tokens, d.out + (size_t)slot * ls.cap, (size_t)n * sizeof(int), hipMemcpyDeviceToHost));
  const int zero = 0;
  HIPCHK(e, hipMemcpy(d.pos + slot, &zero, sizeof(int), hipMemcpyHostToDevice));
  *out_n = n;
  ls.busy[slot] = 0; ls.told[slot] = 0;
  return RK_OK;
}

int rk_llama_session_close(rk_engine* e) {
  if (!e) return RK_ERR_INVALID;
  if (!e->ls.open) return RK_OK;
  int rc = set_device(e);
  if (rc) return rc;
  e->ls.open = false;
  HIPCHK(e, hipStreamSynchronize(e->slots[0].se));
  return RK_OK;
}

int rk_comm_unique_id(uint8_t* out_id, int n_bytes) {
  if (!out_id || n_bytes != RK_COMM_ID_BYTES) return fail(nullptr, RK_ERR_INVALID, "unique id buffer must be %d bytes", RK_COMM_ID_BYTES);
  static_assert(RK_COMM_ID_BYTES == NCCL_UNIQUE_ID_BYTES, "rk_engine.h and rccl.h disagree on the id size");
  const RcclApi* r = rccl_api();
  if (!r) return fail(nullptr, RK_ERR_HIP, "%s", g_rccl.err.c_str());
  ncclUniqueId id;
  const ncclResult_t rc = r->GetUniqueId(&id);
  if (rc != ncclSuccess) return fail(nullptr, RK_ERR_HIP, "ncclGetUniqueId: %s", r->GetErrorString(rc));
  memcpy(out_id, id.internal, RK_COMM_ID_BYTES);
  return RK_OK;
}

int rk_comm_init(rk_engine* e, const uint8_t* id_bytes, int n_bytes, int rank, int world, int max_floats_per_rank) {
  if (!e || !id_bytes || n_bytes != RK_COMM_ID_BYTES) return fail(e, RK_ERR_INVALID, "bad unique id");
  if (world < 1 || rank < 0 || rank >= world || max_floats_per_rank <= 0) return fail(e, RK_ERR_INVALID, "bad rank %d / world %d / capacity %d", rank, world, max_floats_per_rank);
  if (!e->finalized) return fail(e, RK_ERR_STATE, "engine not finalized");
  int rc = set_device(e);
  if (rc) return rc;
  const RcclApi* r = rccl_api();
  if (!r) return fail(e, RK_ERR_HIP, "%s", g_rccl.err.c_str());
  comm_release(e);
  ncclUniqueId id;
  memcpy(id.internal, id_bytes, RK_COMM_ID_BYTES);
  const ncclResult_t nrc = r->CommInitRank(&e->comm, world, id, rank);
  if (nrc != ncclSuccess) { e->comm = nullptr; return fail(e, RK_ERR_HIP, "ncclCommInitRank(rank %d of %d): %s", rank, world, r->GetErrorString(nrc)); }
  e->comm_rank = rank; e->comm_world = world; e->gather_cap = (size_t)max_floats_per_rank;
  if ((rc = comm_alloc_buffers(e))) {
    const std::string why = e->err;
    comm_release(e);
    e->err = why;
    return rc;
  }
  return RK_OK;
}

int rk_comm_world(const rk_engine* e, int* out_rank, int* out_world) {
  if (!e) return RK_ERR_INVALID;
  if (out_rank) *out_rank = e->comm ? e->comm_rank : 0;
  if (out_world) *out_world = e->comm ? e->comm_world : 1;
  return RK_OK;
}

int rk_comm_capacity(const rk_engine* e) { return (e && e->comm) ? (int)e->gather_cap : 0; }

int rk_comm_library_info(char* buf, int n_bytes) {
  if (!buf || n_bytes <= 1) return RK_ERR_INVALID;
  const RcclApi* r = rccl_api();
  if (!r) return fail(nullptr, RK_ERR_HIP, "%s", g_rccl.err.c_str());
  Dl_info info{};
  const char* path = (dladdr((void*)r->AllGather, &info) && info.dli_fname) ? info.dli_fname : "?";
  int ver = 0;
  if (r->GetVersion) r->GetVersion(&ver);
  const int n = snprintf(buf, (size_t)n_bytes, "%s|%d", path, ver);
  return n < n_bytes ? n : n_bytes - 1;
}

int rk_comm_all_gather_slot(rk_engine* e, int slot, int n_floats) {
  if (!e || slot < 0 || slot >= RK_SLOTS) return RK_ERR_INVALID;
  if (!e->comm) return fail(e, RK_ERR_STATE, "rk_comm_init has not been called");
  if (n_floats <= 0 || (size_t)n_floats > e->gather_cap || (size_t)n_floats > e->scores_cap) return fail(e, RK_ERR_CAPACITY, "n_floats %d out of range (capacity %zu, score buffer %zu)", n_floats, e->gather_cap, e->scores_cap);
  int rc = set_device(e);
  if (rc) return rc;
  Slot& sl = e->slots[slot];
  hipStream_t sd = dec_stream(e, sl);
  if (e->gather_pending[slot]) { HIPCHK(e, hipEventSynchronize(e->ev_gather[slot])); e->gather_pending[slot] = false; }
  const ncclResult_t nrc = rccl_api()->AllGather(sl.d_scores, e->d_gather[slot], (size_t)n_floats, ncclFloat, e->comm, sd);
  if (nrc != ncclSuccess) return fail(e, RK_ERR_HIP, "ncclAllGather: %s", rccl_api()->GetErrorString(nrc));
  HIPCHK(e, hipMemcpyAsync(e->h_gather[slot], e->d_gather[slot], (size_t)n_floats * e->comm_world * sizeof(float), hipMemcpyDeviceToHost, sd));
  HIPCHK(e, hipEventRecord(e->ev_gather[slot], sd));
  e->gather_pending[slot] = true; e->gather_n[slot] = n_floats;
  return mark_decoder_done(e, sl);
}

int rk_comm_read_gathered_slot(rk_engine* e, int slot, float* out, int n_floats_total) {
  if (!e || !out || slot < 0 || slot >= RK_SLOTS) return RK_ERR_INVALID;
  if (!e->comm) return fail(e, RK_ERR_STATE, "rk_comm_init has not been called");
  if (n_floats_total != e->gather_n[slot] * e->comm_world) return fail(e, RK_ERR_INVALID, "asked for %d floats, the last gather of slot %d holds %d", n_floats_total, slot, e->gather_n[slot] * e->comm_world);
  if (e->gather_pending[slot]) { HIPCHK(e, hipEventSynchronize(e->ev_gather[slot])); e->gather_pending[slot] = false; }
  memcpy(out, e->h_gather[slot], (size_t)n_floats_total * sizeof(float));
  return RK_OK;
}

int rk_comm_append_scores_slot(rk_engine* e, int slot, int n_floats, int dst_offset) {
  if (!e || slot < 0 || slot >= RK_SLOTS) return RK_ERR_INVALID;
  if (!e->comm) return fail(e, RK_ERR_STATE, "rk_comm_init has not been called");
  if (n_floats < 0 || dst_offset < 0 || (size_t)n_floats + (size_t)dst_offset > e->gather_cap || (size_t)n_floats > e->scores_cap)
    return fail(e, RK_ERR_CAPACITY, "append of %d floats at %d exceeds the send buffer (%zu) or the score buffer (%zu)", n_floats, dst_offset, e->gather_cap, e->scores_cap);
  int rc = set_device(e);
  if (rc) return rc;
  if (n_floats == 0) return RK_OK;
  Slot& sl = e->slots[slot];
  hipStream_t sd = dec_stream(e, sl);
  if (e->gall_pending) { HIPCHK(e, hipEventSynchronize(e->ev_gall)); e->gall_pending = false; }
  HIPCHK(e, hipMemcpyAsync(e->d_gsend + dst_offset, sl.d_scores, (size_t)n_floats * sizeof(float), hipMemcpyDeviceToDevice, sd));
  if (sd != dec_stream(e, e->slots[0])) { HIPCHK(e, hipEventRecord(e->ev_append, sd)); e->append_foreign = true; }
  return mark_decoder_done(e, sl);
}

int rk_comm_append_host(rk_engine* e, const float* values, int n_floats, int dst_offset) {
  if (!e || (!values && n_floats > 0)) return RK_ERR_INVALID;
  if (!e->comm) return fail(e, RK_ERR_STATE, "rk_comm_init has not been called");
  if (n_floats < 0 || dst_offset < 0 || (size_t)n_floats + (size_t)dst_offset > e->gather_cap)
    return fail(e, RK_ERR_CAPACITY, "append of %d host floats at %d exceeds the send buffer (%zu)", n_floats, dst_offset, e->gather_cap);
  int rc = set_device(e);
  if (rc) return rc;
  if (n_floats == 0) return RK_OK;
  if (e->gall_pending) { HIPCHK(e, hipEventSynchronize(e->ev_gall)); e->gall_pending = false; }
  hipStream_t s0 = dec_stream(e, e->slots[0]);
  memcpy(e->h_gstage + dst_offset, values, (size_t)n_floats * sizeof(float));
  HIPCHK(e, hipMemcpyAsync(e->d_gsend + dst_offset, e->h_gstage + dst_offset, (size_t)n_floats * sizeof(float), hipMemcpyHostToDevice, s0));
  return RK_OK;
}

int rk_comm_all_gather_appended(rk_engine* e, int n_floats) {
  if (!e) return RK_ERR_INVALID;
  if (!e->comm) return fail(e, RK_ERR_STATE, "rk_comm_init has not been called");
  if (n_floats <= 0 || (size_t)n_floats > e->gather_cap) return fail(e, RK_ERR_CAPACITY, "n_floats %d out of range (capacity %zu)", n_floats, e->gather_cap);
  int rc = set_device(e);
  if (rc) return rc;
  hipStream_t s0 = dec_stream(e, e->slots[0]);
  if (e->gall_pending) { HIPCHK(e, hipEventSynchronize(e->ev_gall)); e->gall_pending = false; }
  if (e->append_foreign) { HIPCHK(e, hipStreamWaitEvent(s0, e->ev_append, 0)); e->append_foreign = false; }
  const ncclResult_t nrc = rccl_api()->AllGather(e->d_gsend, e->d_gall, (size_t)n_floats, ncclFloat, e->comm, s0);
  if (nrc != ncclSuccess) return fail(e, RK_ERR_HIP, "ncclAllGather: %s", rccl_api()->GetErrorString(nrc));
  HIPCHK(e, hipMemcpyAsync(e->h_gall, e->d_gall, (size_t)n_floats * e->comm_world * sizeof(float), hipMemcpyDeviceToHost, s0));
  HIPCHK(e, hipEventRecord(e->ev_gall, s0));
  e->gall_pending = true; e->gall_n = n_floats;
  return RK_OK;
}

int rk_comm_read_appended(rk_engine* e, float* out, int n_floats_total) {
  if (!e || !out) return RK_ERR_INVALID;
  if (!e->comm) return fail(e, RK_ERR_STATE, "rk_comm_init has not been called");
  if (n_floats_total != e->gall_n * e->comm_world) return fail(e, RK_ERR_INVALID, "asked for %d floats, the last appended gather holds %d", n_floats_total, e->gall_n * e->comm_world);
  if (e->gall_pending) { HIPCHK(e, hipEventSynchronize(e->ev_gall)); e->gall_pending = false; }
  memcpy(out, e->h_gall, (size_t)n_floats_total * sizeof(float));
  return RK_OK;
}

int rk_comm_destroy(rk_engine* e) {
  if (!e) return RK_ERR_INVALID;
  if (set_device(e) == RK_OK) sync_all(e);
  comm_release(e);
  return RK_OK;
}

int rk_timer_begin(rk_engine* e) {
  if (!e) return RK_ERR_INVALID;
  int rc = set_device(e);
  if (rc) return rc;
  hipStream_t s0 = e->slots[0].se;
  HIPCHK(e, hipEventRecord(e->t0, s0));
  for (Slot& sl : e->slots) {
    if (sl.se != s0) HIPCHK(e, hipStreamWaitEvent(sl.se, e->t0, 0));
    HIPCHK(e, hipStreamWaitEvent(sl.sd, e->t0, 0));
  }
  return RK_OK;
}

int rk_timer_end(rk_engine* e, float* out_ms) {
  if (!e || !out_ms) return RK_ERR_INVALID;
  int rc = set_device(e);
  if (rc) return rc;
  hipStream_t s0 = e->slots[0].se;
  for (Slot& sl : e->slots) {
    if (sl.se != s0) { HIPCHK(e, hipEventRecord(e->t_tmp, sl.se)); HIPCHK(e, hipStreamWaitEvent(s0, e->t_tmp, 0)); }
    HIPCHK(e, hipEventRecord(e->t_tmp, sl.sd)); HIPCHK(e, hipStreamWaitEvent(s0, e->t_tmp, 0));
  }
  HIPCHK(e, hipEventRecord(e->t1, s0));
  HIPCHK(e, hipEventSynchronize(e->t1));
  HIPCHK(e, hipEventElapsedTime(out_ms, e->t0, e->t1));
  return RK_OK;
}

int rk_profile_enable(rk_engine* e, int on) { if (!e) return RK_ERR_INVALID; e->prof_on = on != 0; return RK_OK; }

int rk_profile_reset(rk_engine* e) {
  if (!e) return RK_ERR_INVALID;
  int rc = set_device(e);
  if (rc) return rc;
  if ((rc = sync_all(e))) return rc;
  e->prof_used = 0;
  for (int c = 0; c < PC_COUNT; ++c) { e->prof_flops[c] = 0; e->prof_bytes[c] = 0; e->prof_n[c] = 0; }
  return RK_OK;
}

int rk_profile_get(rk_engine* e, int cls, double* total_ms, int64_t* launches, double* flops, double* bytes) {
  if (!e || cls < 0 || cls >= PC_COUNT) return RK_ERR_INVALID;
  int rc = set_device(e);
  if (rc) return rc;
  if ((rc = sync_all(e))) return rc;
  double ms = 0;
  for (size_t i = 0; i < e->prof_used; ++i) {
    if (e->prof_recs[i].cls != cls) continue;
    float t = 0;
    HIPCHK(e, hipEventElapsedTime(&t, e->prof_recs[i].a, e->prof_recs[i].b));
    ms += t;
  }
  if (total_ms) *total_ms = ms;
  if (launches) *launches = e->prof_n[cls];
  if (flops) *flops = e->prof_flops[cls];
  if (bytes) *bytes = e->prof_bytes[cls];
  return RK_OK;
}

}

namespace {
struct OptionDesc { const char* key; int rk_engine::Options::*field; int lo, hi; const char* allowed; const char* what; };
const OptionDesc kOptions[] = {
  {"dec_graph", &rk_engine::Options::dec_graph, 0, 1, nullptr, "decoder chains replayed as HIP graphs (1) or launched eagerly (0)"},
  {"gemm_glds", &rk_engine::Options::glds, 0, 1, nullptr, "128x128 GEMM staging by LDS-DMA (1) or through registers (0); same bits"},
  {"gemm_skinny", &rk_engine::Options::skinny, 0, 0x3F, nullptr, "bit per epilogue kind: few-row GEMMs on the weight-streaming kernel (1 = all)"},
  {"dec_ffn_tiled", &rk_engine::Options::dec_ffn_tiled, 0, 1, nullptr, "one-position decoder: FFN-in on the tiled kernels (1) or the weight-streaming kernel (0)"},
  {"gemm_persistent", &rk_engine::Options::gemm_persistent, 0, 1024, nullptr, "ping-pong GEMM: 1 = one workgroup per CU walks the tiles, 0 = one per tile, n > 1 = n workgroups"},
  {"gemm_s64_stages", &rk_engine::Options::s64_stages, 0, 4, "0,2,3,4", "LDS stages of the 64x64 GEMM (0 = from the tile count); same bits"},
  {"consumer_stats", &rk_engine::Options::consumer_stats, 0, 1, nullptr, "encoder row factors formed by the non-persistent consumer GEMMs themselves (1) or always by rowscale_kernel (0); same bits"},
  {"greedy_spec", &rk_engine::Options::greedy_spec, 0, 65536, nullptr, "rk_t5_greedy2: most decoder rows of a speculative pass; 0 = never speculate; same tokens"},
  {"dec_fold_norm", &rk_engine::Options::dec_fold_norm, 0, 1, nullptr, "decoder RMSNorms folded into the weight-streaming GEMMs (1) or separate kernels (0)"},
  {"fold_norm", &rk_engine::Options::fold_norm, 0, 1, nullptr, "encoder RMSNorm folded into the GEMMs (1) or separate kernels (0)"},
  {"xattn_mfma", &rk_engine::Options::xattn_mfma, 0, 1, nullptr, "query-side cross-attention: weighted sums on the matrix cores (1) or the VALU form (0)"},
  {"attn_heads_per_wg", &rk_engine::Options::attn_heads_per_wg, 0, 4096, nullptr, "short-sequence attention: (sequence, head) items per wave group, 0 = dealt evenly; same bits"},
  {"xattn_direct", &rk_engine::Options::xattn_direct, 0, 1, nullptr, "decoder prefixes <= 16: query-side cross-attention (1) or materialised K / V (0)"},
  {"attn_short", &rk_engine::Options::attn_short, 0, 6, "0,5,6", "sequences <= 192 keys: DMA kernel with two (5) / one (6) wave group per workgroup, or the tiled kernel (0); same bits"},
  {"gemm_variant", &rk_engine::Options::gemm_variant, 0, 120, nullptr, "tile variant: 0 auto, 1..6 see choose_variant; measurement builds: 80+ / 100+ knock-outs"},
  {"dec_fuse_rows", &rk_engine::Options::dec_fuse_rows, 0, 32, nullptr, "rows per workgroup of dec_cross_qk_kernel (0 = auto); same bits"},
  {"dec_fuse", &rk_engine::Options::dec_fuse, 0, 2, nullptr, "few-row decoder: projections around the query-side cross-attention fused at one position (1), always (2), never (0)"},
  {"llama_attn_nw", &rk_engine::Options::llama_attn_nw, 0, 8, "0,4,8", "waves per workgroup of the Llama LDS-DMA attention kernel (0 = default 4); same bits"},
  {"llama_attn_dma", &rk_engine::Options::llama_attn_dma, 0, 1, nullptr, "Llama causal attention: LDS-DMA kernel (1) or the register-staged first kernel (0); differ within fp16 noise"},
  {"attn_long_xcd", &rk_engine::Options::attn_long_xcd, 0, 1, nullptr, "long-sequence attention: workgroups of a (sequence, head) pair on one XCD (1) or dealt over all eight (0); same bits"},
  {"attn_long_nw", &rk_engine::Options::attn_long_nw, 0, 12, "0,3,4,6,12", "waves per workgroup of the long-sequence attention kernel (0 = default 4); same bits"},
  {"attn_long", &rk_engine::Options::attn_long, 0, 1, nullptr, "sequences > 192 keys: the chunked LDS-DMA kernel (1) or the tiled kernel (0)"},
  {"dec_gemv", &rk_engine::Options::dec_gemv, 0, 1, nullptr, "decoder pass of at most 16 rows at >= 2 positions (one setwise compare): plain projections on the wave-per-column GEMV kernel (1) or the weight-streaming MFMA kernel (0); differ within fp32 summation-order noise"},
  {"dec_gemv_rows", &rk_engine::Options::dec_gemv_rows, 1, GEMV_MAX_ROWS, nullptr, "largest row count of a decoder pass that takes the few-row GEMV family (default 4 = the measured cross-over; the kernel takes up to 16)"},
  {"dec_cross_mfma", &rk_engine::Options::dec_cross_mfma, 0, 1, nullptr, "long decoder prefixes (qlm), cross-attention over the materialised K / V: matrix-core kernel for sequences <= 192 keys (1) or the staged fma-chain kernels (0); differ within fp16 noise"},
  {"dec_attn_seq", &rk_engine::Options::dec_attn_seq, 0, 1, nullptr, "decoder attention at several positions: one workgroup per (head, sequence) (1) or per query row (0); same bits"},
  {"gemm_sk", &rk_engine::Options::gemm_sk, 0, 2, nullptr, "ping-pong GEMM, fp32 residual projections with few tiles and a long K: K split over two workgroups (1: choose_ksplit), never (0), wherever it fits (2: tests)"},
  {"dec_cached_attn", &rk_engine::Options::dec_cached_attn, 0, 1, nullptr, "rk_t5_generate's self-attention: attn_dec_cached_kernel (1) or the cache append + attn_dec_kernel's tree form (0); same bits"},
  {"llama_dec_r", &rk_engine::Options::llama_dec_r, 0, 2, nullptr, "rk_llama_generate's attention: query heads per workgroup by plan_llama_dec_attn's rule (0), one (1), or, where a kv head has 7, all seven (2: measurement and tests; every cached K / V byte read once per step); same bits"},
  {"enc_serial", &rk_engine::Options::enc_serial, 0, 1, nullptr, "two slots: an encoder chain starts behind the other slot's (1: one encoder at a time beside the decoder before it) or as soon as it is enqueued (0: two chains interleave); same bits"},
  {"gemm_split", &rk_engine::Options::gemm_split, 0, 1, nullptr, "rows beyond the ping-pong kernel's last whole round on a fill-in tile variant (1) or one launch (0); same bits"},
#ifdef RK_MEASURE
  {"attn_ko", &rk_engine::Options::attn_ko, 0, 1 << 20, nullptr, "timing-only knock-outs of the attention kernels (measurement builds)"},
#endif
};
bool option_value_ok(const OptionDesc& o, int value) {
  if (value < o.lo || value > o.hi) return false;
  if (!o.allowed) return true;
  for (const char* p = o.allowed; *p;) {
    if (atoi(p) == value) return true;
    while (*p && *p != ',') ++p;
    if (*p == ',') ++p;
  }
  return false;
}
}

extern "C" {

int rk_engine_set_option(rk_engine* e, const char* key, int value) {
  if (!e || !key) return RK_ERR_INVALID;
  if (!strcmp(key, "overlap")) {
    if (value < 0 || value > 1) return fail(e, RK_ERR_INVALID, "option overlap: 0..1");
    if (set_device(e) || sync_all(e)) return RK_ERR_HIP;
    for (Slot& sl : e->slots) sl.dec_pending = false;
    e->opt.overlap = value;
    e->opt_epoch++;
    return RK_OK;
  }
#ifdef RK_MEASURE
  if (!strcmp(key, "attn_trace")) {
    if (value && !e->attn_trace) { if (hipMalloc(&e->attn_trace, 12 * 16 * 16 * sizeof(float)) != hipSuccess) return RK_ERR_HIP; hipMemset(e->attn_trace, 0, 12 * 16 * 16 * sizeof(float)); }
    if (!value && e->attn_trace) { hipFree(e->attn_trace); e->attn_trace = nullptr; }
    return RK_OK;
  }
#endif
  for (const OptionDesc& o : kOptions) {
    if (strcmp(key, o.key)) continue;
    if (!strcmp(key, "gemm_skinny") && value == 1) value = 0x3F;
    if (!option_value_ok(o, value))
      return fail(e, RK_ERR_INVALID, "option %s: value %d outside %d..%d%s%s (%s)", key, value, o.lo, o.hi, o.allowed ? ", allowed: " : "", o.allowed ? o.allowed : "", o.what);
    e->opt.*(o.field) = value;
    e->opt_epoch++;
    return RK_OK;
  }
  return fail(e, RK_ERR_INVALID, "unknown option %s", key);
}

int rk_debug_gemm_ex(rk_engine* e, rk_debug_gemm_call* q) {
  if (!e || !q) return RK_ERR_INVALID;
  int rc = set_device(e);
  if (rc) return rc;
  const int epi = q->epi, M = q->M, N = q->N, K = q->K, batch = q->batch > 0 ? q->batch : 1;
  if (epi < 0 || epi > EPI_LSE_F32 || q->family < 0 || q->family > 2 || M <= 0 || N <= 0 || K <= 0 || q->lda <= 0 || q->ldw <= 0 || q->ldc <= 0 ||
      q->n_split < 0 || q->split_stride < 0 || q->bsA < 0 || q->bsW < 0 || q->bsC < 0 || q->c_off < 0 || (long)M * batch > (1 << 22))
    return fail(e, RK_ERR_INVALID, "debug gemm: bad shape");
  const bool gated = EPI_IS_GATED(epi), blocks = epi == EPI_ARGMAX_F32 || epi == EPI_LSE_F32;
  const bool f16 = epi == EPI_STORE_F16 || epi == EPI_RELU_F16 || gated;
  const size_t celt = f16 ? 2 : (epi == EPI_LSE_F32 ? 8 : 4);
  const GemmFamily fam = q->family == 2 ? GEMM_GEMV : (q->family == 1 ? GEMM_STREAM : GEMM_TILED);
  const bool producer = q->xraw_out || q->ssq_out, planning = q->plan_only != 0;
  half_t* const dummy = (half_t*)(uintptr_t)256;
  Gemm c(PC_OTHER, epi, dummy, q->lda, dummy, q->ldw, (char*)dummy + (size_t)q->c_off * celt, q->ldc, M, N, K);
  c.on(fam).heads(batch, q->bsA, q->bsW, q->bsC).split(q->n_split, q->split_stride);
  if (q->rowscale || (q->ssq_in && q->factors_kernel)) c.fold.rowscale = (const float*)dummy;
  else if (q->ssq_in) { c.fold.ssq_in = (const float*)dummy; c.fold.nb_in = q->nb_in; }
  if (q->ssq_in && q->nb_in <= 0) return fail(e, RK_ERR_INVALID, "debug gemm: ssq_in without nb_in");
  if (producer) { c.fold.xraw = dummy; c.fold.ssq = (float*)dummy; }
  c.lse((const int*)dummy, (float*)dummy).argmax((int*)dummy);
  hipStream_t st = e->slots[0].se;
  const GemmPlan p = plan_gemm(e, c, st);
  q->out_family = (int)p.family; q->out_variant = p.variant; q->out_m_pp2 = p.m_pp2; q->out_ksplit = p.m_pp2 > 0 ? p.ks_pp2 : p.ksplit;
  q->out_nb = p.nb; q->out_n_cu = e->n_cu; q->out_eps = e->d.eps; q->out_xs = RK_XRAW_SCALE;
  if (p.family == GEMM_NONE)
    return fail(e, RK_ERR_STATE, "no kernel of family %d takes the GEMM M=%d N=%d K=%d (epilogue %d, batch %d): %s", (int)fam, M, N, K, epi, batch, p.why ? p.why : "");
  if (planning) return RK_OK;
  if (!q->A || !q->W || !q->C || !q->C_out || q->band_rows < 256) return fail(e, RK_ERR_INVALID, "debug gemm: A, W, C, C_out and band_rows >= 256");
  const long nsb = q->n_split > 0 ? (N + q->n_split - 1) / q->n_split : 1;
  const long width = blocks ? (N + 31) / 32 : (q->n_split > 0 ? q->n_split : (gated ? N / 2 : N));
  const long a_need = (long)(batch - 1) * q->bsA + (long)(M - 1) * q->lda + K, w_need = (long)(batch - 1) * q->bsW + (long)(N - 1) * q->ldw + K;
  const long c_need = q->c_off + (long)(batch - 1) * q->bsC + (nsb - 1) * q->split_stride + (long)(M - 1) * q->ldc + width;
  if (a_need > q->a_elems || w_need > q->w_elems || c_need > q->c_elems)
    return fail(e, RK_ERR_INVALID, "debug gemm: the call reaches beyond A (%ld of %ld), W (%ld of %ld) or C (%ld of %ld)", a_need, (long)q->a_elems, w_need, (long)q->w_elems, c_need, (long)q->c_elems);
  if (epi == EPI_ARGMAX_F32 && !q->idx_out) return fail(e, RK_ERR_INVALID, "debug gemm: argmax needs idx_out");
  if (epi == EPI_LSE_F32 && (!q->labels || !q->xlab)) return fail(e, RK_ERR_INVALID, "debug gemm: LSE needs labels and xlab");
  if (producer && (!q->xraw_out || !q->ssq_out || (long)(M + 2 * q->band_rows) * p.nb > q->ssq_cap))
    return fail(e, RK_ERR_INVALID, "debug gemm: producer needs xraw_out and ssq_out of (M + 2 band_rows) x %d floats", p.nb);
  const size_t band = (size_t)q->band_rows * q->ldc, c_all = 2 * band + (size_t)q->c_elems;
  const size_t xband = (size_t)q->band_rows * N, x_all = 2 * xband + (size_t)M * N;
  const size_t sband = (size_t)q->band_rows * p.nb, s_all = 2 * sband + (size_t)M * p.nb;
  const size_t m_pad = ((size_t)M + 255) / 256 * 256 + 256;
  std::vector<void*> dev;
  auto alloc = [&](size_t bytes, int fill) -> void* {
    void* ptr = nullptr;
    if (hipMalloc(&ptr, bytes ? bytes : 16) != hipSuccess) return nullptr;
    dev.push_back(ptr);
    if (fill >= 0 && hipMemset(ptr, fill, bytes) != hipSuccess) return nullptr;
    return ptr;
  };
  auto done = [&](int r) { for (void* ptr : dev) hipFree(ptr); return r; };
#define DBG_HIP(x) do { if ((x) != hipSuccess) return done(fail(e, RK_ERR_HIP, "debug gemm: %s", #x)); } while (0)
  half_t* dA = (half_t*)alloc((size_t)q->a_elems * 2, -1);
  half_t* dW = (half_t*)alloc((size_t)q->w_elems * 2, -1);
  char* dC = (char*)alloc(c_all * celt, RK_DEBUG_SENTINEL);
  int* dI = epi == EPI_ARGMAX_F32 ? (int*)alloc(c_all * 4, RK_DEBUG_SENTINEL) : nullptr;
  half_t* dX = producer ? (half_t*)alloc(x_all * 2, RK_DEBUG_SENTINEL) : nullptr;
  float* dS = producer ? (float*)alloc(s_all * 4, RK_DEBUG_SENTINEL) : nullptr;
  float* dR = (q->rowscale || q->ssq_in) ? (float*)alloc(m_pad * 4, 0) : nullptr;
  float* dQ = q->ssq_in ? (float*)alloc((size_t)M * q->nb_in * 4, -1) : nullptr;
  int* dL = epi == EPI_LSE_F32 ? (int*)alloc((size_t)M * 4, -1) : nullptr;
  float* dXl = epi == EPI_LSE_F32 ? (float*)alloc((size_t)M * 4, -1) : nullptr;
  if (!dA || !dW || !dC || (epi == EPI_ARGMAX_F32 && !dI) || (producer && (!dX || !dS)) || ((q->rowscale || q->ssq_in) && !dR) ||
      (q->ssq_in && !dQ) || (epi == EPI_LSE_F32 && (!dL || !dXl)))
    return done(fail(e, RK_ERR_HIP, "debug gemm: device allocation failed"));
  DBG_HIP(hipMemcpy(dA, q->A, (size_t)q->a_elems * 2, hipMemcpyHostToDevice));
  DBG_HIP(hipMemcpy(dW, q->W, (size_t)q->w_elems * 2, hipMemcpyHostToDevice));
  DBG_HIP(hipMemcpy(dC + band * celt, q->C, (size_t)q->c_elems * celt, hipMemcpyHostToDevice));
  if (q->rowscale) DBG_HIP(hipMemcpy(dR, q->rowscale, (size_t)M * 4, hipMemcpyHostToDevice));
  if (q->ssq_in) DBG_HIP(hipMemcpy(dQ, q->ssq_in, (size_t)M * q->nb_in * 4, hipMemcpyHostToDevice));
  if (dL) { DBG_HIP(hipMemcpy(dL, q->labels, (size_t)M * 4, hipMemcpyHostToDevice)); DBG_HIP(hipMemcpy(dXl, q->xlab, (size_t)M * 4, hipMemcpyHostToDevice)); }
  DBG_HIP(hipDeviceSynchronize());
  c.A = dA; c.W = dW; c.C = dC + (band + (size_t)q->c_off) * celt;
  c.fold = GemmFold();
  if (q->rowscale) c.fold.rowscale = dR;
  else if (q->ssq_in && q->factors_kernel) {
    launch_rowscale(st, dQ, dR, M, q->nb_in, K, e->d.eps, RK_XRAW_SCALE);
    c.fold.rowscale = dR;
  } else if (q->ssq_in) { c.fold.ssq_in = dQ; c.fold.nb_in = q->nb_in; }
  if (producer) { c.fold.xraw = dX + xband; c.fold.ssq = dS + sband; }
  c.lse(dL, dXl).argmax(dI ? dI + band + q->c_off : nullptr);
  int nb = 0;
  rc = gemm(e, st, c, &nb);
  if (rc) return done(rc);
  DBG_HIP(hipStreamSynchronize(st));
  DBG_HIP(hipGetLastError());
  q->out_nb = nb;
  DBG_HIP(hipMemcpy(q->C_out, dC, c_all * celt, hipMemcpyDeviceToHost));
  if (dI) DBG_HIP(hipMemcpy(q->idx_out, dI, c_all * 4, hipMemcpyDeviceToHost));
  if (producer) { DBG_HIP(hipMemcpy(q->xraw_out, dX, x_all * 2, hipMemcpyDeviceToHost)); DBG_HIP(hipMemcpy(q->ssq_out, dS, s_all * 4, hipMemcpyDeviceToHost)); }
  if (dXl) DBG_HIP(hipMemcpy(q->xlab, dXl, (size_t)M * 4, hipMemcpyDeviceToHost));
#undef DBG_HIP
  return done(RK_OK);
}

int rk_debug_gemm_chain(rk_engine* e, rk_debug_gemm_chain_call* q) {
  if (!e || !q) return RK_ERR_INVALID;
  int rc = set_device(e);
  if (rc) return rc;
  const int epi = q->epi, M = q->M, N = q->N, K = q->K, nl = q->n_launch;
  if (epi < 0 || epi > EPI_SWIGLU_F16 || q->family < 0 || q->family > 2 || M <= 0 || N <= 0 || K <= 0 || q->lda <= 0 || q->ldw <= 0 || q->ldc <= 0 ||
      M > (1 << 22))
    return fail(e, RK_ERR_INVALID, "debug gemm chain: bad shape");
  if (nl < 1 || nl > 64) return fail(e, RK_ERR_INVALID, "debug gemm chain: n_launch 1..64");
  if (q->accumulate && epi != EPI_RESID_F32) return fail(e, RK_ERR_INVALID, "debug gemm chain: accumulate is the fp32 residual epilogue's");
  const bool bg = q->bg_per_fg > 0;
  if (q->bg_per_fg < 0 || q->bg_per_fg > 16) return fail(e, RK_ERR_INVALID, "debug gemm chain: bg_per_fg 0..16");
  if (bg && (q->bg_M <= 0 || q->bg_N <= 0 || q->bg_K <= 0 || q->bg_M > (1 << 16) || q->bg_N > (1 << 16) || q->bg_K > (1 << 16) || q->bg_family < 0 ||
             q->bg_family > 2 || q->bg_variant < 0 || q->bg_variant > 6 ||
             !(q->bg_epi == EPI_STORE_F16 || q->bg_epi == EPI_RESID_F32 || q->bg_epi == EPI_RELU_F16 || q->bg_epi == EPI_STORE_F32)))
    return fail(e, RK_ERR_INVALID, "debug gemm chain: bad background call");
  const bool gated = EPI_IS_GATED(epi), f16 = epi == EPI_STORE_F16 || epi == EPI_RELU_F16 || gated;
  const size_t celt = f16 ? 2 : 4;
  auto family_of = [](int f) { return f == 2 ? GEMM_GEMV : (f == 1 ? GEMM_STREAM : GEMM_TILED); };
  half_t* const dummy = (half_t*)(uintptr_t)256;
  hipStream_t st = e->slots[0].se, sb = e->slots[0].sd;
  Gemm c(PC_OTHER, epi, dummy, q->lda, dummy, q->ldw, dummy, q->ldc, M, N, K);
  c.on(family_of(q->family));
  if (q->rowscale) c.fold.rowscale = (const float*)dummy;
  const GemmPlan p = plan_gemm(e, c, st);
  q->out_family = (int)p.family; q->out_variant = p.variant; q->out_m_pp2 = p.m_pp2; q->out_ksplit = p.m_pp2 > 0 ? p.ks_pp2 : p.ksplit;
  q->out_n_cu = e->n_cu;
  q->bg_out_family = GEMM_NONE; q->bg_out_variant = q->bg_out_m_pp2 = 0; q->bg_out_ksplit = 1;
  if (p.family == GEMM_NONE)
    return fail(e, RK_ERR_STATE, "no kernel of family %d takes the GEMM M=%d N=%d K=%d (epilogue %d, batch 1): %s", q->family, M, N, K, epi, p.why ? p.why : "");
  const int fg_variant = e->opt.gemm_variant;
  Gemm b(PC_OTHER, bg ? q->bg_epi : EPI_STORE_F16, dummy, q->bg_K, dummy, q->bg_K, dummy, q->bg_N, q->bg_M, q->bg_N, q->bg_K);
  if (bg) {
    b.on(family_of(q->bg_family));
    e->opt.gemm_variant = q->bg_variant;
    const GemmPlan pb = plan_gemm(e, b, sb);
    e->opt.gemm_variant = fg_variant;
    q->bg_out_family = (int)pb.family; q->bg_out_variant = pb.variant; q->bg_out_m_pp2 = pb.m_pp2; q->bg_out_ksplit = pb.m_pp2 > 0 ? pb.ks_pp2 : pb.ksplit;
    if (pb.family == GEMM_NONE)
      return fail(e, RK_ERR_STATE, "no kernel of family %d takes the background GEMM M=%d N=%d K=%d (epilogue %d): %s", q->bg_family, q->bg_M, q->bg_N, q->bg_K, q->bg_epi, pb.why ? pb.why : "");
    if (pb.pp2()) return fail(e, RK_ERR_INVALID, "debug gemm chain: the background's plan puts rows on the ping-pong kernel");
  }
  if (q->plan_only) return RK_OK;
  if (!q->A || !q->W || !q->C || !q->C_out || q->band_rows < 256) return fail(e, RK_ERR_INVALID, "debug gemm chain: A, W, C, C_out and band_rows >= 256");
  const long width = gated ? N / 2 : N;
  const long a_need = (long)(M - 1) * q->lda + K, w_need = (long)(N - 1) * q->ldw + K, c_need = (long)(M - 1) * q->ldc + width;
  if (a_need > q->a_elems || w_need > q->w_elems || c_need > q->c_elems)
    return fail(e, RK_ERR_INVALID, "debug gemm chain: the call reaches beyond A (%ld of %ld), W (%ld of %ld) or C (%ld of %ld)", a_need, (long)q->a_elems, w_need, (long)q->w_elems, c_need, (long)q->c_elems);
  const int n_out = q->accumulate ? 1 : nl;
  const size_t band = (size_t)q->band_rows * q->ldc, c_all = 2 * band + (size_t)q->c_elems;
  const size_t m_pad = ((size_t)M + 255) / 256 * 256 + 256;
  std::vector<void*> dev;
  auto alloc = [&](size_t bytes, int fill) -> void* {
    void* ptr = nullptr;
    if (hipMalloc(&ptr, bytes ? bytes : 16) != hipSuccess) return nullptr;
// ... 6 lines not shown
  half_t* dA = (half_t*)alloc((size_t)nl * q->a_elems * 2, -1);
  half_t* dW = (half_t*)alloc((size_t)q->w_elems * 2, -1);
  char* dC = (char*)alloc((size_t)n_out * c_all * celt, RK_DEBUG_SENTINEL);
  float* dR = q->rowscale ? (float*)alloc((size_t)nl * m_pad * 4, 0) : nullptr;
  const size_t bga = (size_t)q->bg_M * q->bg_K, bgw = (size_t)q->bg_N * q->bg_K, bgc = (size_t)q->bg_M * q->bg_N;
  half_t* dBA = bg ? (half_t*)alloc(bga * 2, -1) : nullptr;
  half_t* dBW = bg ? (half_t*)alloc(bgw * 2, -1) : nullptr;
  float* dBC = bg ? (float*)alloc(bgc * 4, 0) : nullptr;
  if (!dA || !dW || !dC || (q->rowscale && !dR) || (bg && (!dBA || !dBW || !dBC)))
    return done(fail(e, RK_ERR_HIP, "debug gemm chain: device allocation failed"));
  DBG_HIP(hipMemcpy(dA, q->A, (size_t)nl * q->a_elems * 2, hipMemcpyHostToDevice));
  DBG_HIP(hipMemcpy(dW, q->W, (size_t)q->w_elems * 2, hipMemcpyHostToDevice));
  for (int i = 0; i < n_out; ++i)
    DBG_HIP(hipMemcpy(dC + ((size_t)i * c_all + band) * celt, (const char*)q->C + (size_t)i * q->c_elems * celt, (size_t)q->c_elems * celt, hipMemcpyHostToDevice));
  for (int i = 0; q->rowscale && i < nl; ++i)
    DBG_HIP(hipMemcpy(dR + (size_t)i * m_pad, q->rowscale + (size_t)i * M, (size_t)M * 4, hipMemcpyHostToDevice));
  if (bg) {
    std::vector<half_t> h(std::max(bga, bgw));
    uint32_t x = 2463534242u;
    for (size_t i = 0; i < h.size(); ++i) { x = x * 1664525u + 1013904223u; h[i] = (half_t)(((int)(x >> 16) % 2001 - 1000) * 1e-3f); }
    DBG_HIP(hipMemcpy(dBA, h.data(), bga * 2, hipMemcpyHostToDevice));
    DBG_HIP(hipMemcpy(dBW, h.data(), bgw * 2, hipMemcpyHostToDevice));
    b.A = dBA; b.W = dBW; b.C = dBC;
  }
  DBG_HIP(hipDeviceSynchronize());
  c.W = dW;
  auto background = [&]() {
    e->opt.gemm_variant = q->bg_variant;
    int r = RK_OK;
    for (int j = 0; r == RK_OK && j < q->bg_per_fg; ++j) r = gemm(e, sb, b);
    e->opt.gemm_variant = fg_variant;
    return r;
  };
  for (int i = 0; rc == RK_OK && i < nl; ++i) {
    c.A = dA + (size_t)i * q->a_elems;
    c.C = dC + ((size_t)(q->accumulate ? 0 : i) * c_all + band) * celt;
    c.fold = GemmFold();
    if (q->rowscale) c.fold.rowscale = dR + (size_t)i * m_pad;
    if (bg && q->bg_first) rc = background();
    if (rc == RK_OK) rc = gemm(e, st, c);
    if (rc == RK_OK && bg && !q->bg_first) rc = background();
  }
  const hipError_t s1 = hipStreamSynchronize(st), s2 = hipStreamSynchronize(sb);
  if (rc) return done(rc);
  DBG_HIP(s1); DBG_HIP(s2);
  DBG_HIP(hipGetLastError());
  DBG_HIP(hipMemcpy(q->C_out, dC, (size_t)n_out * c_all * celt, hipMemcpyDeviceToHost));
#undef DBG_HIP
  return done(RK_OK);
}

int rk_debug_attn(rk_engine* e, rk_debug_attn_call* q) {
  if (!e || !q) return RK_ERR_INVALID;
  int rc = set_device(e);
  if (rc) return rc;
  if (!e->finalized) return fail(e, RK_ERR_STATE, "debug attn: engine not finalized");
  const int kind = q->kind, B = q->n_seq, H = q->H;
  if (kind < 1 || kind > 6) return fail(e, RK_ERR_INVALID, "debug attn: kind 1..6");
  const bool llama_kind = kind == 4 || kind == 5;
  if (e->family != (llama_kind ? 1 : 0)) return fail(e, RK_ERR_STATE, "debug attn: kind %d needs a %s engine", kind, llama_kind ? "Llama" : "T5");
  if (B <= 0 || B > (1 << 16) || H <= 0 || H > 1024) return fail(e, RK_ERR_INVALID, "debug attn: n_seq and H");
  const bool planning = q->plan_only != 0;
  const int hd = head_width(e), band = q->band_rows;
  if ((kind == 2 || kind == 6) && hd != 64) return refuse_wide(e, "debug attn", "kinds 2 and 6 (the decoder kernels) have no 128-wide form");
  if (!planning && (!q->q || !q->out || !q->out_all || band < 1)) return fail(e, RK_ERR_INVALID, "debug attn: q, out, out_all and band_rows >= 1");
  int maxL = 0, minL = 1 << 30, T = 0;
  const bool has_off = kind == 1 || kind == 3 || kind == 4 || (kind == 2 && q->cross);
  if (has_off) {
    if (!q->seq_off || q->seq_off[0] != 0) return fail(e, RK_ERR_INVALID, "debug attn: seq_off[n_seq + 1] starting at 0");
    for (int b = 0; b < B; ++b) {
      const int L = q->seq_off[b + 1] - q->seq_off[b];
      if (L <= 0 || L > (1 << 20)) return fail(e, RK_ERR_INVALID, "debug attn: sequence %d has %d keys", b, L);
      maxL = std::max(maxL, L); minL = std::min(minL, L);
    }
    T = q->seq_off[B];
  }
  long q_rows_need = 0, kv_rows_need = 0, out_rows_need = 0;
  long ldq_min = 0, ldkv_min = 0, ldctx_min = 0;
  auto plan_out = [&](int k, int tp, dim3 g1, dim3 g2, int lds) {
    q->out_kind = k; q->out_tparam = tp; q->out_lds = lds; q->out_n_cu = e->n_cu;
    q->out_grid[0] = (int)g1.x; q->out_grid[1] = (int)g1.y; q->out_grid[2] = (int)g1.z;
    q->out_grid2[0] = (int)g2.x; q->out_grid2[1] = (int)g2.y; q->out_grid2[2] = (int)g2.z;
  };
  q->out_staged = q->out_mfma = q->out_part = q->out_R = q->out_nch = q->out_skip_long = q->out_heads_per_wg = 0;
  EncAttnPlan ep; DecAttnPlan dp; XAttnPlan xp; CausalAttnPlan cp; LlamaDecAttnPlan lp;
  int dec_rows = 0, dec_keys = 0;
  if (kind == 1) {
    const int I = H * hd;
    ldq_min = 3L * I; ldctx_min = I; q_rows_need = out_rows_need = T;
    if (!planning && !q->bias_lut) return fail(e, RK_ERR_INVALID, "debug attn: the encoder needs bias_lut");
    ep = plan_enc_attn(e, B, maxL, minL, H);
    plan_out((int)ep.kind, ep.kind == EncAttnPlan::DMA ? ep.ng : ep.nw, ep.grid, ep.tiled_grid, ep.lds);
    q->out_skip_long = ep.skip_long; q->out_heads_per_wg = ep.heads_per_wg;
  } else if (kind == 2) {
    const int Ld = q->Ld;
    if (Ld <= 0 || Ld > (1 << 16) || q->k_col < 0 || q->v_col < 0) return fail(e, RK_ERR_INVALID, "debug attn: Ld, k_col, v_col");
    const bool tree = q->tree_rows > 0;
    if (tree && (q->cross || q->row_off || !q->tree_keys || !q->tree_pos)) return fail(e, RK_ERR_INVALID, "debug attn: the tree form is the self-attention's, with tree_keys and tree_pos, without row_off");
    if (q->row_off) {
      if (q->row_off[0] != 0) return fail(e, RK_ERR_INVALID, "debug attn: row_off starts at 0");
      int longest = 0;
      for (int b = 0; b < B; ++b) {
        const int n = q->row_off[b + 1] - q->row_off[b];
        if (n <= 0) return fail(e, RK_ERR_INVALID, "debug attn: sequence %d has %d rows", b, n);
        longest = std::max(longest, n);
      }
// ... 126 lines not shown
                                           q->Ld, q->cross ? 0 : 1, dec_keys, dTk, dTp, 0, dRow}, 0, 0);
  } else if (kind == 3) {
    int* dRs = nullptr;
    if (q->row_seq && !(dRs = (int*)up(q->row_seq, (size_t)q->n_row_seq * 4))) return done(fail(e, RK_ERR_HIP, "debug attn: upload failed"));
    float* dPart = (float*)alloc((size_t)q->M * xp.nch * H * q->d * 4, RK_DEBUG_SENTINEL);
    float* dStat = (float*)alloc((size_t)q->M * xp.nch * H * 2 * 4, RK_DEBUG_SENTINEL);
    if (!dPart || !dStat) return done(fail(e, RK_ERR_HIP, "debug attn: device allocation failed"));
    DBG_HIP(hipDeviceSynchronize());
    launch_xattn_part(e, st, xp, XAttnArgs{qi, kvi, dOff, dPart, dStat, oi, q->Ld, H, q->d, xp.nch, q->row0, dRs}, maxL, T);
  } else if (kind == 4) {
    DBG_HIP(hipDeviceSynchronize());
    launch_llama_attn(e, st, CausalAttnCall{qi, oi, dOff, q->ldq, q->ldctx, H, q->n_kv, B, maxL, T}, cp);
  } else if (kind == 6) {
    const int I = H * 64, P = q->P;
    const size_t c_in = (size_t)B * P * 2 * I, c_band = (size_t)band * 64;
    c_all = c_in + 2 * c_band;
    dC = (half_t*)alloc(c_all * 2, RK_DEBUG_SENTINEL);
    std::vector<int> keys((size_t)B * P);
    for (int b = 0; b < B; ++b) for (int j = 0; j < P; ++j) keys[(size_t)b * P + j] = b * P + j;
    int* dPos = (int*)up(q->pos, 4);
    int* dTk = (int*)up(keys.data(), keys.size() * 4);
    int* dTp = (int*)alloc((size_t)B * 4, 0);
    if (!dC || !dPos || !dTk || !dTp) return done(fail(e, RK_ERR_HIP, "debug attn: device allocation or upload failed"));
    DBG_HIP(hipMemcpy(dC + c_band, q->cache, c_in * 2, hipMemcpyHostToDevice));
    DBG_HIP(hipDeviceSynchronize());
    launch_dec_cached_step(e, st, AttnCachedArgs{qi, q->ldq, dC + c_band, P, I, dPos, oi, q->ldctx, dLut}, B, H, dTk, dTp);
  } else {
    const size_t half_layer = (size_t)B * q->n_kv * q->P * hd, c_band = (size_t)band * hd;
    c_all = 2 * half_layer + 2 * c_band;
    dC = (half_t*)alloc(c_all * 2, RK_DEBUG_SENTINEL);
    int* dPos = (int*)up(q->pos, (size_t)B * 4);
    float* dCos = (float*)up(q->cos_t, (size_t)q->max_pos * (hd / 2) * 4);
    float* dSin = (float*)up(q->sin_t, (size_t)q->max_pos * (hd / 2) * 4);
    float* dBias = q->qkv_bias ? (float*)up(q->qkv_bias, (size_t)(H + 2 * q->n_kv) * hd * 4) : nullptr;
    float* dQkn = q->qk_norm ? (float*)up(q->qk_norm, (size_t)2 * hd * 4) : nullptr;
    float* dPart = (float*)alloc((size_t)B * H * lp.nch * ldc_pstr(hd) * 4, RK_DEBUG_SENTINEL);
    if (!dC || !dPos || !dCos || !dSin || (q->qkv_bias && !dBias) || (q->qk_norm && !dQkn) || !dPart) return done(fail(e, RK_ERR_HIP, "debug attn: device allocation or upload failed"));
    DBG_HIP(hipMemcpy(dC + c_band, q->cache, 2 * half_layer * 2, hipMemcpyHostToDevice));
    DBG_HIP(hipDeviceSynchronize());
    const float scale_log2e = (1.0f / std::sqrt((float)hd)) * 1.4426950408889634f;
    half_t* kc = dC + c_band;
    launch_llama_dec_attn(e, st, lp, LlamaDecAttnArgs{qi, kc, kc + half_layer, dPos, dCos, dSin, dPart, oi, q->ldq, H, q->n_kv, q->P, lp.nch, scale_log2e, dBias, 0, dQkn, q->qk_eps}, B);
  }
  DBG_HIP(hipStreamSynchronize(st));
  DBG_HIP(hipGetLastError());
  DBG_HIP(hipMemcpy(q->out_all, dO, o_all * 2, hipMemcpyDeviceToHost));
  if (dC) DBG_HIP(hipMemcpy(q->cache_all, dC, c_all * 2, hipMemcpyDeviceToHost));
#undef DBG_HIP
  return done(RK_OK);
}

int rk_debug_xattn_chain(rk_engine* e, rk_debug_xattn_chain_call* q) {
  if (!e || !q) return RK_ERR_INVALID;
  int rc = set_device(e);
  if (rc) return rc;
  if (!e->finalized) return fail(e, RK_ERR_STATE, "debug xattn chain: engine not finalized");
  if (e->family != 0) return fail(e, RK_ERR_STATE, "debug xattn chain: needs a T5 engine");
  const int hd = head_width(e);
  const int M = q->M, H = q->H, d = q->d, Ld = q->Ld, B = q->n_seq, band = q->band_rows, I = H * hd;
  if (B <= 0 || B > (1 << 16) || H <= 0 || H > 1024) return fail(e, RK_ERR_INVALID, "debug xattn chain: n_seq and H");
  if (M <= 0 || M > (1 << 16) || d <= 0 || d % 32 || d > 16384 || Ld <= 0 || q->row0 < 0)
    return fail(e, RK_ERR_INVALID, "debug xattn chain: M, Ld, row0 and d (a multiple of 32)");
  if (!q->seq_off || q->seq_off[0] != 0) return fail(e, RK_ERR_INVALID, "debug xattn chain: seq_off[n_seq + 1] starting at 0");
  int maxL = 0;
  for (int b = 0; b < B; ++b) {
    const int L = q->seq_off[b + 1] - q->seq_off[b];
    if (L <= 0 || L > (1 << 20)) return fail(e, RK_ERR_INVALID, "debug xattn chain: sequence %d has %d keys", b, L);
    maxL = std::max(maxL, L);
  }
  const int T = q->seq_off[B];
  if (maxL > 65536) return fail(e, RK_ERR_STATE, "debug xattn chain: the chunk merge takes sequences of at most 65536 keys");
  for (int m = 0; m < M; ++m) {
    if (q->row_seq && q->row0 + m >= q->n_row_seq) return fail(e, RK_ERR_INVALID, "debug xattn chain: row_seq has %d entries, row %d is read", q->n_row_seq, q->row0 + m);
    const int b = q->row_seq ? q->row_seq[q->row0 + m] : (q->row0 + m) / Ld;
    if (b < 0 || b >= B) return fail(e, RK_ERR_INVALID, "debug xattn chain: row %d belongs to sequence %d of %d", q->row0 + m, b, B);
  }
  if (q->rowscale && q->ssq_in) return fail(e, RK_ERR_INVALID, "debug xattn chain: rowscale or ssq_in, not both");
  if (q->ssq_in && (q->nb_in <= 0 || q->nb_in > 4096)) return fail(e, RK_ERR_INVALID, "debug xattn chain: ssq_in needs nb_in in 1..4096");
  XAttnChain c{};
  c.ldx = q->ldx; c.Ld = Ld; c.row0 = q->row0; c.ldo = q->ldo; c.M = M; c.H = H; c.dm = d; c.maxL = maxL; c.T = T; c.fuse_asked = q->fuse_asked != 0; c.hd = hd;
  c.family = dec_len_class(e, Ld).stream ? GEMM_STREAM : GEMM_TILED;
  const bool fuse = xattn_chain_fused(c);
  const int blk = xattn_block_rows(maxL), n_blocks = (M + blk - 1) / blk, wrows = std::min(blk, M), nch = (maxL + 63) / 64;
  q->out_fused = fuse; q->out_block_rows = blk; q->out_n_blocks = n_blocks; q->out_nch = nch; q->out_n_cu = e->n_cu;
  q->out_eps = e->d.eps; q->out_xs = RK_XRAW_SCALE;
  for (int i = 0; i < 2; ++i) {
    const int r0 = i ? (n_blocks - 1) * blk : 0;
    const XAttnPlan xp = plan_xattn(e, fuse, std::min(blk, M - r0), maxL, H, d);
    q->out_qk_R[i] = xp.fuse_qk ? xp.qk_R : 0; q->out_qk_CS[i] = xp.fuse_qk ? xp.qk_CS : 0; q->out_part_kind[i] = (int)xp.part;
    q->out_part_grid[i][0] = (int)xp.part_grid.x; q->out_part_grid[i][1] = (int)xp.part_grid.y; q->out_part_grid[i][2] = (int)xp.part_grid.z;
    q->out_fuse_cv[i] = xp.fuse_cv; q->out_cv_R[i] = xp.fuse_cv ? xp.cv_R : 0;
  }
  if (q->plan_only) return RK_OK;
  if (!q->x || !q->wq || !q->wk || !q->wv || !q->enc || !q->qk_all || !q->part_all || !q->stat_all || !q->xctx_all || !q->ctx_all || band < 1)
    return fail(e, RK_ERR_INVALID, "debug xattn chain: x, wq, wk, wv, enc, the five outputs and band_rows >= 1");
  if (q->ldx < d || q->ldx % 8 || q->ldx > (1 << 20) || q->ldo < I || q->ldo % 8 || q->ldo > (1 << 20))
    return fail(e, RK_ERR_INVALID, "debug xattn chain: leading dimensions (ldx %d >= %d, ldo %d >= %d; multiples of 8, at most 2^20)", q->ldx, d, q->ldo, I);
  if (q->enc_rows < T) return fail(e, RK_ERR_INVALID, "debug xattn chain: the call reaches beyond enc (%d of %ld rows)", T, (long)q->enc_rows);
  const size_t Hd = (size_t)H * d;
  const size_t part_in = (size_t)wrows * nch * Hd, part_band = (size_t)band * Hd, part_all = part_in + 2 * part_band;
  const size_t stat_in = (size_t)wrows * nch * H * 2, stat_band = (size_t)band * H * 2, stat_all = stat_in + 2 * stat_band;
  const size_t xc_in = (size_t)wrows * Hd, xc_all = xc_in + 2 * part_band;
  const size_t qk_all = ((size_t)M + 2 * band) * Hd, ctx_band = (size_t)band * q->ldo, ctx_in = (size_t)M * q->ldo, ctx_all = ctx_in + 2 * ctx_band;
  const size_t enc_all = ((size_t)q->enc_rows + 2 * band) * d;
  if (enc_all >= (1ul << 31) || qk_all >= (1ul << 31) || part_all >= (1ul << 31) || stat_all >= (1ul << 31) || ctx_all >= (1ul << 31) || (size_t)M * q->ldx >= (1ul << 31))
    return fail(e, RK_ERR_INVALID, "debug xattn chain: operands of 2^31 elements or more");
// ... 34 lines not shown
  if (q->ctx) DBG_HIP(hipMemcpy(dCtx + ctx_band, q->ctx, ctx_in * 2, hipMemcpyHostToDevice));
  c.x = dX; c.wq = dWq; c.wkT = dWkT; c.wv = dWv;
  c.fold.rowscale = dScale; c.fold.ssq_in = dSsq; c.fold.nb_in = q->ssq_in ? q->nb_in : 0;
  c.enc = dEnc + (size_t)band * d; c.seq_off = dOff; c.row_seq = dRs;
  c.q = dQ; c.qk = dQk + (size_t)band * Hd; c.part = dPart + part_band; c.stat = dStat + stat_band; c.xctx = dXc + part_band;
  c.ctx = dCtx + ctx_band;
  hipStream_t st = e->slots[0].se;
  if (!fuse || nch > DECV_MAXCH) {
    std::vector<Gemm> gs;
    if (!fuse) { gs.push_back(xattn_q_gemm(c)); gs.push_back(xattn_qk_gemm(c, 0, wrows, c.qk)); }
    gs.push_back(xattn_cv_gemm(c, 0, wrows));
    for (const Gemm& g : gs) {
      const GemmPlan gp = plan_gemm(e, g, st);
      if (q->ssq_in && &g == &gs[0] && !fuse && gp.pp2())
        return done(fail(e, RK_ERR_STATE, "debug xattn chain: the q GEMM of this shape takes ready-made row factors: pass rowscale, not ssq_in"));
      if (gp.family == GEMM_NONE) return done(fail(e, RK_ERR_STATE, "debug xattn chain: no kernel takes the GEMM M=%d N=%d K=%d of the unfused form: %s", g.M, g.N, g.K, gp.why ? gp.why : ""));
    }
  }
  struct Ctx { rk_engine* e; rk_debug_xattn_chain_call* q; const XAttnChain* c; hipStream_t st; half_t* qk0; float *dPart, *dStat; half_t* dXc;
               size_t Hd, part_all, stat_all, xc_all, part_in, stat_in; int blk; } hc{e, q, &c, st, c.qk, dPart, dStat, dXc, Hd, part_all, stat_all, xc_all, part_in, stat_in, blk};
  XAttnChainHook hook{[](void* user, bool front, int r0, const XAttnPlan&, half_t** qk) -> int {
    Ctx& h = *(Ctx*)user;
    const int k = r0 / h.blk;
    bool ok = true;
    if (front) {
      *qk = h.qk0 + (size_t)r0 * h.Hd;
      ok = hipMemsetAsync(h.dPart, RK_DEBUG_SENTINEL, h.part_all * 4, h.st) == hipSuccess && hipMemsetAsync(h.dStat, RK_DEBUG_SENTINEL, h.stat_all * 4, h.st) == hipSuccess &&
           hipMemsetAsync(h.dXc, RK_DEBUG_SENTINEL, h.xc_all * 2, h.st) == hipSuccess;
      if (ok && h.q->ws_fill)
        ok = hipMemsetD32Async((hipDeviceptr_t)h.c->part, (int)h.q->ws_fill, h.part_in, h.st) == hipSuccess &&
             hipMemsetD32Async((hipDeviceptr_t)h.c->stat, (int)h.q->ws_fill, h.stat_in, h.st) == hipSuccess;
    } else {
      ok = hipStreamSynchronize(h.st) == hipSuccess && hipGetLastError() == hipSuccess &&
           hipMemcpy(h.q->part_all + (size_t)k * h.part_all, h.dPart, h.part_all * 4, hipMemcpyDeviceToHost) == hipSuccess &&
           hipMemcpy(h.q->stat_all + (size_t)k * h.stat_all, h.dStat, h.stat_all * 4, hipMemcpyDeviceToHost) == hipSuccess &&
           hipMemcpy(h.q->xctx_all + (size_t)k * h.xc_all, h.dXc, h.xc_all * 2, hipMemcpyDeviceToHost) == hipSuccess;
    }
    if (!ok) { return fail(h.e, RK_ERR_HIP, "debug xattn chain: a HIP call failed at the block of row %d", r0); }
    return RK_OK;
  }, &hc};
  DBG_HIP(hipDeviceSynchronize());
  rc = run_xattn_chain(e, st, c, &hook);
  if (rc) { hipStreamSynchronize(st); return done(rc); }
  DBG_HIP(hipStreamSynchronize(st));
  DBG_HIP(hipGetLastError());
  DBG_HIP(hipMemcpy(q->qk_all, dQk, qk_all * 2, hipMemcpyDeviceToHost));
  DBG_HIP(hipMemcpy(q->ctx_all, dCtx, ctx_all * 2, hipMemcpyDeviceToHost));
#undef DBG_HIP
  return done(RK_OK);
}

int rk_debug_rows(rk_engine* e, rk_debug_rows_call* q) {
  if (!e || !q) return RK_ERR_INVALID;
  int rc = set_device(e);
  if (rc) return rc;
  const int op = q->op, rows = q->rows, d = q->d;
  const long R = rows;
  if (op < 1 || op > 11) return fail(e, RK_ERR_INVALID, "debug rows: op 1..11");
  if (rows <= 0 || rows > (1 << 20)) return fail(e, RK_ERR_INVALID, "debug rows: rows = %d", rows);
  const int n_steps = op == 10 ? q->n_steps : 1;
  if (n_steps < 1 || n_steps > 4096) return fail(e, RK_ERR_INVALID, "debug rows: n_steps = %d", n_steps);
  long in_need[4] = {0, 0, 0, 0}, out_need[8] = {0, 0, 0, 0, 0, 0, 0, 0};
  bool in_opt[4] = {false, false, false, false};
  dim3 grid(1);
  int tparam = 0, variant = 0, maxL = 0;
  auto ints = [&](int i, long n) -> const int* { return (q->in[i].data && q->in[i].off >= 0 && q->in[i].off + n * 4 <= q->in[i].bytes) ? (const int*)((const char*)q->in[i].data + q->in[i].off) : nullptr; };
  auto state = [&](int i, long n) -> const int* { return (q->out[i].interior && n * 4 <= q->out[i].bytes) ? (const int*)q->out[i].interior : nullptr; };
  const bool planning = q->plan_only != 0;
  auto bad = [&](const char* what) { return fail(e, RK_ERR_INVALID, "debug rows: op %d: %s", op, what); };
  switch (op) {
    case 1: {
      if (d <= 0 || d % 8 || d > (1 << 16) || q->vocab <= 0 || q->vocab > (1 << 22)) return bad("d (a multiple of 8) and vocab");
      in_need[0] = R * 4; in_need[1] = (long)q->vocab * d * 2;
      out_need[0] = R * d * 4; out_need[1] = R * d * 2; out_need[2] = R * 4;
      grid = grid_waves(rows); variant = q->kind != 0;
    } break;
    case 2: {
      if (q->nb <= 0 || q->nb > (1 << 16) || d <= 0) return bad("nb and d");
      in_need[0] = R * q->nb * 4; out_need[0] = R * 4;
      grid = grid_rowscale(rows);
    } break;
    case 3: {
      if (d <= 0 || d % 4 || d > 4096) return bad("d must be a multiple of 4 and at most 4096 (rmsnorm_kernel<16> holds 4096 columns)");
      if (q->src_rows <= 0 || q->src_rows > (1 << 20)) return bad("src_rows");
      in_need[0] = (long)q->src_rows * d * 4; in_need[1] = (long)d * 4; in_need[2] = R * 4; in_opt[2] = true;
      out_need[0] = R * d * 2;
      grid = grid_waves(rows); tparam = rmsnorm_nv(d);
      if (!planning) {
        if (q->in[2].data) {
          const int* m = ints(2, R);
          if (!m) return bad("row_map of rows ints");
          for (long r = 0; r < R; ++r) if (m[r] < 0 || m[r] >= q->src_rows) return bad("row_map entry outside [0, src_rows)");
        } else if (rows > q->src_rows) return bad("rows beyond src_rows without a row_map");
      }
    } break;
    case 4: case 5: {
      const int n_out = op == 4 ? q->n_out : 2;
      if (d <= 0 || d % 8 || d > (1 << 16) || q->vocab <= 0 || q->vocab > (1 << 22) || n_out <= 0 || n_out > 4096) return bad("d (a multiple of 8), vocab and n_out");
      if (op == 5 && (rows < 2 || q->false_id < 0 || q->false_id >= q->vocab || q->true_id < 0 || q->true_id >= q->vocab)) return bad("at least 2 sequences, false_id and true_id inside the vocabulary");
      in_need[0] = R * d * 2; in_need[1] = (long)q->vocab * d * 2;
      if (op == 4) {
        in_need[2] = (long)n_out * 4; out_need[0] = R * n_out * 4;
        if (!planning) {
          const int* ids = ints(2, n_out);
          if (!ids) return bad("out_ids of n_out ints");
          for (int j = 0; j < n_out; ++j) if (ids[j] < 0 || ids[j] >= q->vocab) return bad("out_ids entry outside the vocabulary");
// ... 149 lines not shown
  }
  DBG_HIP(hipDeviceSynchronize());
  hipStream_t st = e->slots[0].se;
  const long A = (op == 10 && q->kind == 2) ? std::max<long>(R, q->max_admit) : R, rec = 1 + 3L * q->max_admit;
  for (int s = 0; s < n_steps; ++s) {
    switch (op) {
      case 1: launch_embed(st, (const int*)din[0], (const half_t*)din[1], (float*)dout[0], rows, d, q->vocab, q->kind ? (half_t*)dout[1] : nullptr,
                           q->kind ? (float*)dout[2] : nullptr, q->xs, q->eps); break;
      case 2: launch_rowscale(st, (const float*)din[0], (float*)dout[0], rows, q->nb, d, q->eps, q->xs); break;
      case 3: launch_rmsnorm(st, (const float*)din[0], (const float*)din[1], (half_t*)dout[0], (const int*)din[2], rows, d, q->eps, q->out_scale); break;
      case 4: launch_head_rows(st, (const half_t*)din[0], (const half_t*)din[1], (const int*)din[2], (float*)dout[0], rows, q->n_out, d); break;
      case 5: launch_pair_verdict(st, (const half_t*)din[0], (const half_t*)din[1], q->false_id, q->true_id, (float*)dout[0], rows, d); break;
      case 6: launch_argmax_blocks(st, (const float*)din[0], (const int*)din[1], q->nb, (int*)dout[0], rows); break;
      case 7: launch_qlm_lse(st, (const float2*)din[0], q->nb, (const float*)din[1], q->n_pos, (const int*)din[2], (const int*)din[3], (float*)dout[0], rows); break;
      case 8: launch_rope(st, q->hd, (half_t*)dout[0], (const int*)din[0], (const float*)din[1], (const float*)din[2], q->ld, q->H + q->n_kv,
                          (const float*)din[3], q->n_kv, rows); break;
      case 11: launch_rope(st, q->hd, (half_t*)dout[0], (const int*)din[0], (const float*)din[1], (const float*)din[2], q->ld, q->H + q->n_kv,
                           nullptr, q->n_kv, rows, (const float*)din[3], q->eps); break;
      case 9: {
        half_t* kc = (half_t*)dout[0];
        launch_kv_fill(st, q->hd, (const half_t*)din[0], (const int*)din[1], (const int*)din[2], q->n_slots, kc,
                       kc + (size_t)(din[2] ? q->n_slots : rows) * q->n_kv * q->P * q->hd, q->ld, q->H, q->n_kv, q->P, maxL, rows);
      } break;
      default: {
        const int* am = (const int*)din[0] + (size_t)s * A;
        if (q->kind == 0)
          launch_greedy_advance(st, am, (int*)dout[0], (const int*)din[1], (int*)dout[1], (int*)dout[2], (int*)dout[3], rows, q->dec_len, q->max_new);
        else if (q->kind == 1)
          launch_llama_advance(st, am, (int*)dout[0], (const int*)din[1], (int*)dout[1], (int*)dout[2], (int*)dout[3], (int*)dout[4], rows);
        else {
          const int* host_rec = din[1] ? (const int*)((const char*)q->in[1].data + q->in[1].off) + (size_t)s * rec : nullptr;
          const int n_admit = host_rec ? host_rec[0] : -1;
          const int* adm = n_admit >= 0 ? (const int*)din[1] + (size_t)s * rec + 1 : nullptr;
          launch_session_advance(st, am, (int*)dout[0], (int*)dout[1], (int*)dout[2], (int*)dout[3], (int*)dout[4], (int*)dout[5], (int*)dout[6],
                                 (int*)dout[7], rows, adm, n_admit >= 0 ? n_admit : 0);
        }
      } break;
    }
    DBG_HIP(hipStreamSynchronize(st));
    DBG_HIP(hipGetLastError());
    for (int i = 0; i < 8; ++i)
      if (dall[i]) {
        const size_t all = (size_t)(q->out[i].bytes + 2 * q->out[i].band);
        DBG_HIP(hipMemcpy((char*)q->out[i].all + (size_t)s * all, dall[i], all, hipMemcpyDeviceToHost));
      }
  }
#undef DBG_HIP
  return done(RK_OK);
}


int rk_debug_gemm(rk_engine* e, const uint16_t* A, const uint16_t* W, float* C, int M, int N, int K, int use_glds) {
  if (!e || !A || !W || !C) return RK_ERR_INVALID;
  if (K % 64 || N % 4) return fail(e, RK_ERR_INVALID, "debug gemm needs K%%64==0 and N%%4==0");
  if (M <= 0) return RK_OK;
  rk_debug_gemm_call q{};
  q.epi = EPI_STORE_F32; q.family = use_glds == 3 ? 2 : (use_glds >= 2 ? 1 : 0);
  q.M = M; q.N = N; q.K = K; q.lda = q.ldw = K; q.ldc = N;
  q.A = A; q.a_elems = (int64_t)M * K; q.W = W; q.w_elems = (int64_t)N * K;
  q.C = C; q.c_elems = (int64_t)M * N; q.band_rows = 256; q.batch = 1;
  std::vector<float> all((size_t)(M + 512) * N);
  q.C_out = all.data();
  const int saved = e->opt.glds;
  e->opt.glds = use_glds != 0;
  const int rc = rk_debug_gemm_ex(e, &q);
  e->opt.glds = saved;
  if (rc) return rc;
  memcpy(C, all.data() + (size_t)256 * N, (size_t)M * N * 4);
  return RK_OK;
}

int rk_debug_gemm_bench(rk_engine* e, int M, int N, int K, int epi, int iters, float* out_ms) {
  if (!e || !out_ms || M <= 0 || N <= 0 || K <= 0 || iters <= 0) return RK_ERR_INVALID;
  int rc = set_device(e);
  if (rc) return rc;
  if (K % 64 || N % 4) return fail(e, RK_ERR_INVALID, "gemm bench needs K%%64==0 and N%%4==0");
  const char* pad_env = getenv("RK_BENCH_PAD");
  const int pad = pad_env ? atoi(pad_env) : 0;
  const int ldk = K + pad;
  const size_t na = (size_t)M * ldk, nw = (size_t)N * ldk, nc = (size_t)M * N;
  half_t *dA = nullptr, *dW = nullptr; void* dC = nullptr;
  HIPCHK(e, hipMalloc((void**)&dA, na * 2)); HIPCHK(e, hipMalloc((void**)&dW, nw * 2));
  HIPCHK(e, hipMalloc(&dC, nc * 4));
  {
    std::vector<half_t> h(std::max(na, nw));
    uint32_t x = 12345u;
    for (size_t i = 0; i < h.size(); ++i) { x = x * 1664525u + 1013904223u; h[i] = (half_t)(((int)(x >> 16) % 2001 - 1000) * 1e-3f); }
    HIPCHK(e, hipMemcpy(dA, h.data(), na * 2, hipMemcpyHostToDevice));
    HIPCHK(e, hipMemcpy(dW, h.data(), nw * 2, hipMemcpyHostToDevice));
    HIPCHK(e, hipMemset(dC, 0, nc * 4));
  }
  const int ldc = EPI_IS_GATED(epi) ? N / 2 : N;
  GemmFold fold;
  half_t* dX = nullptr; float* dS = nullptr;
  if (getenv("RK_BENCH_FOLD") && atoi(getenv("RK_BENCH_FOLD")) && epi == EPI_RESID_F32) {
    HIPCHK(e, hipMalloc((void**)&dX, nc * 2)); HIPCHK(e, hipMalloc((void**)&dS, (size_t)M * ((N + 31) / 32) * 4));
    fold.xraw = dX; fold.ssq = dS;
  }
  const Gemm c = Gemm(PC_OTHER, epi, dA, ldk, dW, ldk, dC, ldc, M, N, K).with(fold);
  for (int i = 0; i < 2; ++i) RC(gemm(e, e->slots[0].se, c));
  HIPCHK(e, hipEventRecord(e->t0, e->slots[0].se));
  for (int i = 0; i < iters; ++i) RC(gemm(e, e->slots[0].se, c));
  HIPCHK(e, hipEventRecord(e->t1, e->slots[0].se));
  HIPCHK(e, hipEventSynchronize(e->t1));
  float ms = 0;
  HIPCHK(e, hipEventElapsedTime(&ms, e->t0, e->t1));
  HIPCHK(e, hipGetLastError());
  *out_ms = ms / iters;
  hipFree(dA); hipFree(dW); hipFree(dC); if (dX) hipFree(dX); if (dS) hipFree(dS);
  return RK_OK;
}

int rk_debug_graph_stats(rk_engine* e, rk_debug_graph_stats_t* out) {
  if (!e || !out) return RK_ERR_INVALID;
  int ready = 0;
  for (const auto& kv : e->graphs) ready += kv.second.exec != nullptr;
  const auto& n = e->graph_count;
  out->n_keys = (int)e->graphs.size(); out->n_ready = ready; out->max_keys = RK_GRAPH_CACHE_KEYS;
  out->eager = n.eager; out->captures = n.captures; out->replays = n.replays; out->failed = n.failed; out->evictions = n.evictions;
  return RK_OK;
}

int rk_debug_buffers(rk_engine* e, rk_debug_buffers_t* out) {
  if (!e || !out) return RK_ERR_INVALID;
  int i = 0;
  auto put = [&](const auto& b) { out->addr[i] = (uint64_t)(uintptr_t)b.p; out->cap[i] = (uint64_t)b.cap; ++i; };
  put(e->logits); put(e->amax_val); put(e->amax_idx); put(e->kv_cache); put(e->gen_buf); put(e->lkv); put(e->lpart); put(e->lints);
  static_assert(RK_DEBUG_N_BUFFERS == 8, "one put per grown buffer");
  out->amax_gen = e->amax_gen; out->kv_gen = e->kv_gen; out->lkv_gen = e->lkv_gen;
  return RK_OK;
}

int rk_debug_sample(rk_engine* e, rk_debug_sample_call* q) {
  if (!e || !q) return RK_ERR_INVALID;
  if (q->rows <= 0 || q->rows > (1 << 20) || q->logit_rows <= 0 || q->logit_rows > q->rows || q->V <= 0 || q->V > sampling::MAX_VOCAB)
    return fail(e, RK_ERR_INVALID, "rk_debug_sample: rows %d (1 .. 2^20), logit_rows %d (1 .. rows), V %d (1 .. %d)", q->rows, q->logit_rows, q->V, sampling::MAX_VOCAB);
  if (!q->logits || !q->seeds || !q->index || !q->out_token) return fail(e, RK_ERR_INVALID, "rk_debug_sample: null logits, seeds, index or out_token");
  if (!(q->temperature > 0.f) || std::isinf(q->temperature) || q->top_k < 0 || !(q->top_p > 0.f && q->top_p <= 1.f))
    return fail(e, RK_ERR_INVALID, "rk_debug_sample: temperature %g (> 0), top_k %d (>= 0), top_p %g (in (0, 1])", (double)q->temperature, q->top_k, (double)q->top_p);
  for (int r = 0; r < q->rows; ++r)
    if (q->index[r] < 0) return fail(e, RK_ERR_INVALID, "rk_debug_sample: token index %d of row %d is negative", q->index[r], r);
  int rc = set_device(e);
  if (rc) return rc;
  const size_t rows = (size_t)q->rows, nl = (size_t)q->logit_rows * q->V;
  float* d_logits = nullptr; unsigned long long* d_seeds = nullptr; int* d_ints = nullptr;
  auto done = [&](int r) { if (d_logits) hipFree(d_logits); if (d_seeds) hipFree(d_seeds); if (d_ints) hipFree(d_ints); return r; };
  if (hipMalloc((void**)&d_logits, nl * sizeof(float)) != hipSuccess || hipMalloc((void**)&d_seeds, rows * sizeof(uint64_t)) != hipSuccess ||
      hipMalloc((void**)&d_ints, 4 * rows * sizeof(int)) != hipSuccess)
    return done(fail(e, RK_ERR_HIP, "rk_debug_sample: hipMalloc failed"));
  hipStream_t st = e->slots[0].se;
  std::vector<int> ints(4 * rows, -1);
  memcpy(ints.data(), q->index, rows * sizeof(int));
  if (hipMemcpy(d_logits, q->logits, nl * sizeof(float), hipMemcpyHostToDevice) != hipSuccess ||
      hipMemcpy(d_seeds, q->seeds, rows * sizeof(uint64_t), hipMemcpyHostToDevice) != hipSuccess ||
      hipMemcpy(d_ints, ints.data(), ints.size() * sizeof(int), hipMemcpyHostToDevice) != hipSuccess)
    return done(fail(e, RK_ERR_HIP, "rk_debug_sample: upload failed"));
  const rk_engine::Sampling sp{q->temperature, q->top_k, q->top_p};
  launch_sample_rows(st, d_logits, q->logit_rows, q->V, sp, d_seeds, nullptr, d_ints, nullptr, 0, d_ints + rows, d_ints + 2 * rows, q->rows);
  if (hipStreamSynchronize(st) != hipSuccess || hipGetLastError() != hipSuccess ||
      hipMemcpy(ints.data(), d_ints, ints.size() * sizeof(int), hipMemcpyDeviceToHost) != hipSuccess)
    return done(fail(e, RK_ERR_HIP, "rk_debug_sample: the launch failed"));
  for (size_t r = 0; r < rows; ++r) {
    q->out_token[r] = ints[rows + r];
    if (q->out_kept_k) q->out_kept_k[r] = ints[2 * rows + 2 * r];
    if (q->out_kept_p) q->out_kept_p[r] = ints[2 * rows + 2 * r + 1];
  }
  return done(RK_OK);
}

int64_t rk_debug_read(rk_engine* e, const char* name, float* out, int64_t max_floats) {
  if (!e || !name || !out) return RK_ERR_INVALID;
  if (set_device(e)) return RK_ERR_HIP;
  if (sync_all(e)) return RK_ERR_HIP;
  if (!strcmp(name, "occupancy")) {
    if (max_floats < 6) return RK_ERR_INVALID;
    int n = 0;
    hipOccupancyMaxActiveBlocksPerMultiprocessor(&n, attn_enc_kernel, 256, 0); out[0] = (float)n;
    out[1] = 0.f;
    hipOccupancyMaxActiveBlocksPerMultiprocessor(&n, gemm_f16_kernel<EPI_STORE_F16, true>, 256, GEMM_LDS_BYTES); out[2] = (float)n;
    hipOccupancyMaxActiveBlocksPerMultiprocessor(&n, gemm_pp2_kernel<EPI_STORE_F16, 0>, 512, 163840); out[3] = (float)n;
    out[4] = 0.f;
    hipOccupancyMaxActiveBlocksPerMultiprocessor(&n, rmsnorm_kernel<4>, 256, 0); out[5] = (float)n;
    if (max_floats >= 10) {
      hipOccupancyMaxActiveBlocksPerMultiprocessor(&n, attn_enc_dma_kernel<1>, 384, ATTD_LDS_BYTES); out[6] = (float)n;
      hipOccupancyMaxActiveBlocksPerMultiprocessor(&n, attn_enc_dma_kernel<2>, 768, 2 * ATTD_LDS_BYTES); out[7] = (float)n;
      out[8] = out[9] = 0.f;
      return 10;
    }
    return 6;
  }
  const Slot& sl = e->slots[0];
  const std::string n(name);
  const int I = e->inner, dm = e->d.d_model;
  const void* src = nullptr; int64_t cnt = 0; bool is_half = true;
  if (n == "enc_hidden") { src = sl.enc.hidden; cnt = (int64_t)sl.T * dm; is_half = false; }
#ifdef RK_MEASURE
  else if (n == "attn_trace" && e->attn_trace) { src = e->attn_trace; cnt = 12 * 16 * 16; is_half = false; }
#endif
  else if (n == "enc_out") { src = sl.enc_out; cnt = (int64_t)sl.T * dm; }
  else if (n == "qkv") { src = sl.qkv; cnt = (int64_t)sl.T * 3 * I; }
  else if (n == "ctx") { src = sl.ctx; cnt = (int64_t)sl.T * I; }
  else if (n == "xn") { src = sl.enc.xn; cnt = (int64_t)sl.T * dm; }
  else if (n == "llama_last") { src = sl.dlast; cnt = (int64_t)sl.n_seq * dm; }
  else if (n == "dec_hidden") { src = sl.dec.hidden; cnt = (int64_t)sl.n_seq * e->d.max_dec_len * dm; is_half = false; }
  else return fail(e, RK_ERR_INVALID, "unknown buffer %s", name);
  cnt = std::min(cnt, max_floats);
  if (is_half) {
    std::vector<half_t> tmp(cnt);
    if (hipMemcpy(tmp.data(), src, cnt * 2, hipMemcpyDeviceToHost) != hipSuccess) return fail(e, RK_ERR_HIP, "copy failed");
    for (int64_t i = 0; i < cnt; ++i) out[i] = (float)tmp[i];
  } else if (hipMemcpy(out, src, cnt * 4, hipMemcpyDeviceToHost) != hipSuccess) return fail(e, RK_ERR_HIP, "copy failed");
  return cnt;
}

}
```

Baseline: 7749.

## Batch two slots' one-position T5 score decoders into a single paired pass

When two consecutive single-position rk_t5_score calls on the two slots share the decoder prefix and output ids, the first slot's decoder is deferred. The second encoder writes its output next to the first's, and one decoder pass runs over both slots' sequences with merged sequence offsets. This halves the number of small decoder launches and gives the decoder matmuls more rows per launch. In exchange, the first slot's scores are delayed until the pair forms or a flush happens, and every API entry point now has to flush any pending decode, which adds state and ordering complexity.

```diff
diff --git a/llm-rankers_amd/csrc/rk_engine.hip b/llm-rankers_amd/csrc/rk_engine.hip
--- a/llm-rankers_amd/csrc/rk_engine.hip
+++ b/llm-rankers_amd/csrc/rk_engine.hip
@@ -112,6 +112,7 @@
   int *stg_tokens[2] = {nullptr, nullptr}, *stg_seq_off[2] = {nullptr, nullptr};
   int gen = 0; bool gen_launched = false; unsigned stage_no = 0, off_of = 0;
   int n_seq = 0, T = 0, maxL = 0, minL = 0; bool staged = false; int last_floats = 0;
+  std::vector<int> h_off;
   half_t* cross_kv = nullptr;
   DecIndex idx; int* d_argmax = nullptr;
   NormStream dec;
@@ -146,8 +147,15 @@
         gemm_persistent = 1, fold_norm = 1, s64_stages = 0, dec_fold_norm = 1, greedy_spec = 160, consumer_stats = 1, xattn_mfma = 1,
         dec_ffn_tiled = 1, gemm_split = 1, dec_fuse = 1, dec_fuse_rows = 0, dec_attn_seq = 1, attn_long = 1, attn_long_nw = 0,
         llama_attn_dma = 1, attn_long_xcd = 1, llama_attn_nw = 0, dec_graph = 1, gemm_sk = 1, dec_cross_mfma = 1, dec_gemv = 1, dec_gemv_rows = 4,
-        dec_cached_attn = 1, llama_dec_r = 0, enc_serial = 0;
+        dec_cached_attn = 1, llama_dec_r = 0, enc_serial = 0, dec_pair = 1;
   } opt;
+  struct PairPass {
+    static constexpr int RING = 4;
+    Slot ws; bool ok = false;
+    int slot = -1, prefix = 0, n_out = 0, out_ids[64] = {0};
+    int* pin_off = nullptr; hipEvent_t ev_off[RING] = {nullptr}; unsigned off_no = 0; std::vector<int> off_held;
+    hipEvent_t ev_join = nullptr;
+  } pair;
   float* attn_trace = nullptr;
   int n_cu = 256;
   struct SkWs { hipStream_t st = nullptr; float* slabs = nullptr; int* cnt = nullptr; };
@@ -200,6 +208,8 @@
   } while (0)
 #define RC(x) do { rc = (x); if (rc) return rc; } while (0)
 
+int flush_pending(rk_engine* e, int slot = -1);
+
 template <class T>
 int dalloc(rk_engine* e, T** p, size_t n) {
   void* q = nullptr;
@@ -1054,13 +1064,13 @@
   });
 }
 
-int wait_prev_decoder(rk_engine* e, Slot& sl) {
-  hipStream_t se = enc_stream(e, sl);
+int wait_prev_decoder(rk_engine* e, Slot& sl, hipStream_t on = nullptr) {
+  hipStream_t se = on ? on : enc_stream(e, sl);
   if (sl.dec_pending && dec_stream(e, sl) != se) HIPCHK(e, hipStreamWaitEvent(se, sl.ev_dec, 0));
   return RK_OK;
 }
 
-int run_encoder(rk_engine* e, Slot& sl, bool need_cross_kv) {
+int run_encoder(rk_engine* e, Slot& sl, bool need_cross_kv, half_t* enc_out_to = nullptr) {
   const rk_model_desc& d = e->d;
   hipStream_t st = enc_stream(e, sl);
   const int T = sl.T, I = e->inner, dm = d.d_model, F = d.d_ff;
@@ -1081,13 +1091,15 @@
     RC(ns.producer(e, st, Gemm(PC_ENC_GEMM_FFN_OUT, EPI_RESID_F32, sl.ffh, F, w.ffn_out, F, ns.hidden, dm, T, dm, F), !last));
   }
   RC(wait_prev_decoder(e, sl));
+  if (enc_out_to) RC(wait_prev_decoder(e, e->slots[(&sl - e->slots) ^ 1], st));
   if (sl.off_of != sl.stage_no) {
     HIPCHK(e, hipMemcpyAsync(sl.dec_seq_off, seq_off, (size_t)(sl.n_seq + 1) * sizeof(int), hipMemcpyDeviceToDevice, st));
     sl.off_of = sl.stage_no;
   }
-  rmsnorm(e, st, ns.hidden, e->enc_final_ln, sl.enc_out, nullptr, T);
+  half_t* enc_out = enc_out_to ? enc_out_to : sl.enc_out;
+  rmsnorm(e, st, ns.hidden, e->enc_final_ln, enc_out, nullptr, T);
   if (need_cross_kv)
-    RC(gemm(e, st, Gemm(PC_GEMM_CROSS_KV, EPI_STORE_F16, sl.enc_out, dm, e->cross_kv_w, dm, sl.cross_kv, 2 * I, T, d.n_dec_layers * 2 * I, dm)
+    RC(gemm(e, st, Gemm(PC_GEMM_CROSS_KV, EPI_STORE_F16, enc_out, dm, e->cross_kv_w, dm, sl.cross_kv, 2 * I, T, d.n_dec_layers * 2 * I, dm)
                        .split(2 * I, (long)d.max_tokens * 2 * I)));
   sl.have_cross_kv = need_cross_kv;
   HIPCHK(e, hipGetLastError());
@@ -1178,14 +1190,14 @@
   return RK_OK;
 }
 
-int encoder_then_handoff_kv(rk_engine* e, Slot& sl, bool need_cross_kv) {
+int encoder_then_handoff_kv(rk_engine* e, Slot& sl, bool need_cross_kv, half_t* enc_out_to = nullptr) {
   hipStream_t se = enc_stream(e, sl), sd = dec_stream(e, sl);
   if (need_cross_kv && !sl.cross_kv) return refuse_wide(e, "encoder", "the materialised cross-attention K / V are not allocated");
   static_assert(RK_SLOTS == 2, "the other slot");
   const Slot& other = e->slots[(&sl - e->slots) ^ 1];
   if (e->opt.enc_serial && sd != se && other.enc_gen >= 0) HIPCHK(e, hipStreamWaitEvent(se, other.ev_enc[other.enc_gen], 0));
   sl.gen_launched = true;
-  const int rc = run_encoder(e, sl, need_cross_kv);
+  const int rc = run_encoder(e, sl, need_cross_kv, enc_out_to);
   HIPCHK(e, hipEventRecord(sl.ev_enc[sl.gen], se));
   sl.enc_gen = sl.gen;
   if (rc) return rc;
@@ -1193,8 +1205,8 @@
   return RK_OK;
 }
 
-int encoder_then_handoff(rk_engine* e, Slot& sl, int max_ld, bool query_side = false) {
-  return encoder_then_handoff_kv(e, sl, !query_side && !use_xattn_direct(e, sl, max_ld));
+int encoder_then_handoff(rk_engine* e, Slot& sl, int max_ld, bool query_side = false, half_t* enc_out_to = nullptr) {
+  return encoder_then_handoff_kv(e, sl, !query_side && !use_xattn_direct(e, sl, max_ld), enc_out_to);
 }
 
 int mark_decoder_done(rk_engine* e, Slot& sl) {
@@ -1204,6 +1216,8 @@
 }
 
 int sync_all(rk_engine* e) {
+  const int rc = flush_pending(e);
+  if (rc) return rc;
   for (Slot& sl : e->slots) {
     HIPCHK(e, hipStreamSynchronize(sl.se));
     HIPCHK(e, hipStreamSynchronize(sl.sd));
@@ -1298,8 +1312,10 @@
   int rc = set_device(e);
   if (rc) return rc;
   Slot& sl = e->slots[slot];
+  if ((rc = flush_pending(e, slot))) return rc;
   sl.staged = false;
   if ((rc = check_batch(e, &sl, tokens, seq_offsets, n_seq))) return rc;
+  sl.h_off.assign(seq_offsets, seq_offsets + n_seq + 1);
   const int g = sl.gen_launched ? sl.gen ^ 1 : sl.gen;
   HIPCHK(e, hipEventSynchronize(sl.ev_enc[g]));
   HIPCHK(e, hipMemcpy(sl.stg_tokens[g], tokens, (size_t)sl.T * sizeof(int), hipMemcpyHostToDevice));
@@ -1388,30 +1404,20 @@
   return RK_OK;
 }
 
-int score_slot(rk_engine* e, int slot, const int32_t* dec_prefix, int dec_len, const int32_t* out_token_ids, int n_out) {
-  if (slot < 0 || slot >= RK_SLOTS) return fail(e, RK_ERR_INVALID, "slot %d out of range", slot);
-  int rc = set_device(e);
-  if (rc) return rc;
-  Slot& sl = e->slots[slot];
-  if (!sl.staged) return fail(e, RK_ERR_STATE, "no staged batch in slot %d", slot);
-  if (!dec_prefix || dec_len <= 0 || dec_len > e->d.max_dec_len) return fail(e, RK_ERR_CAPACITY, "dec_len %d out of range (max %d)", dec_len, e->d.max_dec_len);
-  if (!out_token_ids || n_out <= 0 || n_out > 64) return fail(e, RK_ERR_INVALID, "n_out must be in 1..64 (got %d)", n_out);
-  if ((rc = check_ids(e, dec_prefix, dec_len, "decoder")) || (rc = check_ids(e, out_token_ids, n_out, "output"))) return rc;
-  if (wide_heads(e) && dec_len > 1) return refuse_wide(e, "rk_t5_score", "dec_len > 1 has no 128-wide decoder self-attention");
-  if ((rc = check_wide_one(e, "rk_t5_score"))) return rc;
-  hipStream_t sd = dec_stream(e, sl);
-  if ((rc = put_dec_ids_shared(e, sl, dec_prefix, dec_len))) return rc;
-  if ((rc = sl.idx.put(e, sd, IX_OUT_IDS, out_token_ids, n_out))) return rc;
-  std::vector<int> rows(sl.n_seq);
-  for (int b = 0; b < sl.n_seq; ++b) rows[b] = b * dec_len + dec_len - 1;
-  if ((rc = sl.idx.put(e, sd, IX_LAST_ROWS, rows.data(), sl.n_seq))) return rc;
-  if ((rc = encoder_then_handoff(e, sl, dec_len))) return rc;
+inline bool score_skips_decoder() {
 #ifdef RK_MEASURE
   static const bool skip_dec = getenv("RK_DEBUG_SKIP_DECODER") != nullptr;
+  return skip_dec;
 #else
-  constexpr bool skip_dec = false;
+  return false;
 #endif
-  rc = run_graphed(e, sd, {GK_T5_SCORE, slot, sl.n_seq, dec_len, sl.have_cross_kv ? sl.maxL : (sl.maxL + 63) / 64, (int)sl.have_cross_kv, n_out, (int)skip_dec}, [&]() -> int {
+}
+
+int score_decode(rk_engine* e, int slot, int dec_len, int n_out) {
+  Slot& sl = e->slots[slot];
+  hipStream_t sd = dec_stream(e, sl);
+  const bool skip_dec = score_skips_decoder();
+  int rc = run_graphed(e, sd, {GK_T5_SCORE, slot, sl.n_seq, dec_len, sl.have_cross_kv ? sl.maxL : (sl.maxL + 63) / 64, (int)sl.have_cross_kv, n_out, (int)skip_dec}, [&]() -> int {
     int r = RK_OK;
     if (!skip_dec && (r = run_decoder(e, sl, dec_len))) return r;
     rmsnorm(e, sd, sl.dec.hidden, e->dec_final_ln, sl.dlast, sl.idx.d[IX_LAST_ROWS], sl.n_seq, head_scale(e));
@@ -1422,8 +1428,101 @@
   if (rc) return rc;
   HIPCHK(e, hipMemcpyAsync(sl.h_scores, sl.d_scores, (size_t)sl.n_seq * n_out * sizeof(float), hipMemcpyDeviceToHost, sd));
   HIPCHK(e, hipGetLastError());
+  return mark_decoder_done(e, sl);
+}
+
+int flush_pending(rk_engine* e, int slot) {
+  rk_engine::PairPass& pp = e->pair;
+  if (pp.slot < 0 || (slot >= 0 && slot != pp.slot)) return RK_OK;
+  const int s = pp.slot;
+  pp.slot = -1;
+  const int rc = set_device(e);
+  return rc ? rc : score_decode(e, s, 1, pp.n_out);
+}
+
+int pair_put_ids(rk_engine* e, int prefix, const int32_t* out_ids, int n_out) {
+  Slot& W = e->pair.ws;
+  const std::vector<int> ids((size_t)2 * e->d.max_seqs, prefix);
+  const int rc = W.idx.put(e, dec_stream(e, W), IX_DEC_IDS, ids.data(), (int)ids.size());
+  return rc ? rc : W.idx.put(e, dec_stream(e, W), IX_OUT_IDS, out_ids, n_out);
+}
+
+int pair_decode(rk_engine* e, int a, int b) {
+  rk_engine::PairPass& pp = e->pair;
+  Slot &A = e->slots[a], &B = e->slots[b], &W = pp.ws;
+  const int n_out = pp.n_out, dm = e->d.d_model, n = A.n_seq + B.n_seq;
+  pp.slot = -1;
+  hipStream_t sp = dec_stream(e, W);
+  for (Slot* s : {&A, &B}) {
+    hipStream_t sd = dec_stream(e, *s);
+    if (sd != sp) { HIPCHK(e, hipEventRecord(pp.ev_join, sd)); HIPCHK(e, hipStreamWaitEvent(sp, pp.ev_join, 0)); }
+  }
+  W.n_seq = n; W.T = A.T + B.T; W.maxL = std::max(A.maxL, B.maxL); W.minL = std::min(A.minL, B.minL);
+  W.have_cross_kv = false; W.enc_out = A.enc_out;
+  int rc = RK_OK;
+  std::vector<int> ints(n + 1);
+  for (int s = 0; s <= A.n_seq; ++s) ints[s] = A.h_off[s];
+  for (int s = 1; s <= B.n_seq; ++s) ints[A.n_seq + s] = A.T + B.h_off[s];
+  if (ints != pp.off_held) {
+    const unsigned k = pp.off_no++ % rk_engine::PairPass::RING;
+    HIPCHK(e, hipEventSynchronize(pp.ev_off[k]));
+    int* h = pp.pin_off + (size_t)k * (2 * e->d.max_seqs + 1);
+    memcpy(h, ints.data(), ints.size() * sizeof(int));
+    HIPCHK(e, hipMemcpyAsync(W.dec_seq_off, h, ints.size() * sizeof(int), hipMemcpyHostToDevice, sp));
+    HIPCHK(e, hipEventRecord(pp.ev_off[k], sp));
+    pp.off_held.swap(ints);
+  }
+  RC(run_graphed(e, sp, {GK_T5_SCORE, RK_SLOTS + a, A.n_seq, B.n_seq, (W.maxL + 63) / 64, n_out}, [&]() -> int {
+    const int r = run_decoder(e, W, 1);
+    if (r) return r;
+    rmsnorm(e, sp, W.dec.hidden, e->dec_final_ln, W.dlast, W.idx.d[IX_LAST_ROWS], n, head_scale(e));
+    Bracket br(e, sp, PC_HEAD, 2.0 * n * n_out * dm, 0);
+    launch_head_rows(sp, W.dlast, e->lm_head, W.idx.d[IX_OUT_IDS], A.d_scores, A.n_seq, n_out, dm);
+    launch_head_rows(sp, W.dlast + (size_t)A.n_seq * dm, e->lm_head, W.idx.d[IX_OUT_IDS], B.d_scores, B.n_seq, n_out, dm);
+    return RK_OK;
+  }));
+  for (Slot* s : {&A, &B}) {
+    HIPCHK(e, hipMemcpyAsync(s->h_scores, s->d_scores, (size_t)s->n_seq * n_out * sizeof(float), hipMemcpyDeviceToHost, sp));
+    HIPCHK(e, hipEventRecord(s->ev_dec, sp));
+    s->dec_pending = true;
+    if (dec_stream(e, *s) != sp) HIPCHK(e, hipStreamWaitEvent(dec_stream(e, *s), s->ev_dec, 0));
+  }
+  HIPCHK(e, hipGetLastError());
+  return RK_OK;
+}
+
+int score_slot(rk_engine* e, int slot, const int32_t* dec_prefix, int dec_len, const int32_t* out_token_ids, int n_out) {
+  if (slot < 0 || slot >= RK_SLOTS) return fail(e, RK_ERR_INVALID, "slot %d out of range", slot);
+  int rc = set_device(e);
+  if (rc) return rc;
+  if ((rc = flush_pending(e, slot))) return rc;
+  Slot& sl = e->slots[slot];
+  if (!sl.staged) return fail(e, RK_ERR_STATE, "no staged batch in slot %d", slot);
+  if (!dec_prefix || dec_len <= 0 || dec_len > e->d.max_dec_len) return fail(e, RK_ERR_CAPACITY, "dec_len %d out of range (max %d)", dec_len, e->d.max_dec_len);
+  if (!out_token_ids || n_out <= 0 || n_out > 64) return fail(e, RK_ERR_INVALID, "n_out must be in 1..64 (got %d)", n_out);
+  if ((rc = check_ids(e, dec_prefix, dec_len, "decoder")) || (rc = check_ids(e, out_token_ids, n_out, "output"))) return rc;
+  if (wide_heads(e) && dec_len > 1) return refuse_wide(e, "rk_t5_score", "dec_len > 1 has no 128-wide decoder self-attention");
+  if ((rc = check_wide_one(e, "rk_t5_score"))) return rc;
+  rk_engine::PairPass& pp = e->pair;
+  const bool can_pair = pp.ok && e->opt.dec_pair && dec_len == 1 && use_xattn_direct(e, sl, 1) && !score_skips_decoder();
+  const bool pairs = can_pair && pp.slot >= 0 && pp.slot != slot && pp.prefix == dec_prefix[0] && pp.n_out == n_out &&
+                     !memcmp(pp.out_ids, out_token_ids, n_out * sizeof(int));
+  if (!pairs && (rc = flush_pending(e))) return rc;
+  hipStream_t sd = dec_stream(e, sl);
+  if ((rc = put_dec_ids_shared(e, sl, dec_prefix, dec_len))) return rc;
+  if ((rc = sl.idx.put(e, sd, IX_OUT_IDS, out_token_ids, n_out))) return rc;
+  std::vector<int> rows(sl.n_seq);
+  for (int b = 0; b < sl.n_seq; ++b) rows[b] = b * dec_len + dec_len - 1;
+  if ((rc = sl.idx.put(e, sd, IX_LAST_ROWS, rows.data(), sl.n_seq))) return rc;
+  if (can_pair && !pairs && (rc = pair_put_ids(e, dec_prefix[0], out_token_ids, n_out))) return rc;
+  const Slot& first = e->slots[slot ^ 1];
+  if ((rc = encoder_then_handoff(e, sl, dec_len, false, pairs ? first.enc_out + (size_t)first.T * e->d.d_model : nullptr))) return rc;
   sl.last_floats = sl.n_seq * n_out;
-  return mark_decoder_done(e, sl);
+  if (pairs) return pair_decode(e, slot ^ 1, slot);
+  if (!can_pair) return score_decode(e, slot, dec_len, n_out);
+  pp.slot = slot; pp.prefix = dec_prefix[0]; pp.n_out = n_out;
+  memcpy(pp.out_ids, out_token_ids, n_out * sizeof(int));
+  return RK_OK;
 }
 
 int compare_slot(rk_engine* e, int slot, int dec_start_id, int false_id, int true_id) {
@@ -1431,6 +1530,7 @@
   if (e->family != 0) return fail(e, RK_ERR_STATE, "T5 entry point called on a Llama engine (use rk_llama_*)");
   int rc = set_device(e);
   if (rc) return rc;
+  if ((rc = flush_pending(e))) return rc;
   Slot& sl = e->slots[slot];
   if (!sl.staged) return fail(e, RK_ERR_STATE, "no staged batch in slot %d", slot);
   if (sl.n_seq % 2) return fail(e, RK_ERR_INVALID, "a compare needs pairs of sequences (staged n_seq = %d)", sl.n_seq);
@@ -1618,10 +1718,15 @@
 void rk_engine_destroy(rk_engine* e) {
   if (!e) return;
   hipSetDevice(e->dev);
+  (void)flush_pending(e);
   for (auto& sl : e->slots) {
     if (sl.se) hipStreamSynchronize(sl.se);
     if (sl.sd) hipStreamSynchronize(sl.sd);
   }
+  if (e->pair.ws.idx.pin) hipHostFree(e->pair.ws.idx.pin);
+  if (e->pair.pin_off) hipHostFree(e->pair.pin_off);
+  for (hipEvent_t ev : e->pair.ev_off) if (ev) hipEventDestroy(ev);
+  if (e->pair.ev_join) hipEventDestroy(e->pair.ev_join);
   comm_release(e);
   for (auto& kv : e->graphs) if (kv.second.exec) hipGraphExecDestroy(kv.second.exec);
   e->graphs.clear();
@@ -1819,9 +1924,10 @@
   const size_t Tc = d.max_tokens, Bc = d.max_seqs, Mc = (size_t)d.max_seqs * d.max_dec_len;
   e->scores_cap = Bc * 64;
   if (2 * e->scores_cap < 7 * Bc) return fail(e, RK_ERR_CAPACITY, "score buffer of %zu floats cannot hold a compare of %zu sequences", e->scores_cap, Bc);
+  const bool pair_ok = !wide_heads(e) && 2 * Tc * (size_t)dm * sizeof(half_t) <= ((size_t)1 << 32);
   for (Slot& sl : e->slots) {
     RC(dalloc(e, &sl.enc.hidden, Tc * dm)); RC(dalloc(e, &sl.enc.xn, Tc * dm)); RC(dalloc(e, &sl.qkv, Tc * 3 * I));
-    RC(dalloc(e, &sl.ctx, Tc * I)); RC(dalloc(e, &sl.ffh, Tc * F)); RC(dalloc(e, &sl.enc_out, Tc * dm));
+    RC(dalloc(e, &sl.ctx, Tc * I)); RC(dalloc(e, &sl.ffh, Tc * F)); RC(dalloc(e, &sl.enc_out, (pair_ok ? 2 : 1) * Tc * dm));
     RC(dalloc(e, &sl.enc.xraw[0], Tc * dm)); RC(dalloc(e, &sl.enc.ssq[0], Tc * ((dm + 63) / 64))); RC(dalloc(e, &sl.enc.factors, Tc + 512));
     HIPCHK(e, hipMemset(sl.enc.factors, 0, (Tc + 512) * sizeof(float)));
     for (int g = 0; g < 2; ++g) { RC(dalloc(e, &sl.stg_tokens[g], Tc)); RC(dalloc(e, &sl.stg_seq_off[g], Bc + 1)); }
@@ -1841,6 +1947,29 @@
     HIPCHK(e, hipHostMalloc((void**)&sl.h_scores, e->scores_cap * sizeof(float), hipHostMallocDefault));
     HIPCHK(e, hipHostMalloc((void**)&sl.idx.pin, IX_N_CACHED * DecIndex::PIN_INTS * sizeof(int), hipHostMallocDefault));
   }
+  if (pair_ok) {
+    rk_engine::PairPass& pp = e->pair;
+    Slot& w = pp.ws;
+    const size_t Pc = 2 * Bc;
+    w.sd = e->slots[0].sd;
+    RC(dalloc(e, &w.dec_seq_off, Pc + 1));
+    RC(dalloc(e, &w.idx.d[IX_DEC_IDS], Pc)); RC(dalloc(e, &w.idx.d[IX_LAST_ROWS], Pc)); RC(dalloc(e, &w.idx.d[IX_OUT_IDS], 64));
+    RC(dalloc(e, &w.dec.hidden, Pc * dm)); RC(dalloc(e, &w.dec.xn, Pc * dm));
+    RC(dalloc(e, &w.dctx, Pc * I)); RC(dalloc(e, &w.dq, Pc * I)); RC(dalloc(e, &w.dffh, Pc * F)); RC(dalloc(e, &w.dlast, Pc * dm));
+    for (int i = 0; i < 2; ++i) { RC(dalloc(e, &w.dec.xraw[i], Pc * dm)); RC(dalloc(e, &w.dec.ssq[i], Pc * ((dm + 31) / 32))); }
+    RC(dalloc(e, &w.dec.factors, Pc + 512));
+    HIPCHK(e, hipMemset(w.dec.factors, 0, (Pc + 512) * sizeof(float)));
+    std::vector<int> identity(Pc);
+    for (size_t r = 0; r < Pc; ++r) identity[r] = (int)r;
+    HIPCHK(e, hipMemcpy(w.idx.d[IX_LAST_ROWS], identity.data(), Pc * sizeof(int), hipMemcpyHostToDevice));
+    RC(dalloc(e, &w.xqk, (size_t)XA_MAX_ROWS * d.n_heads * dm)); RC(dalloc(e, &w.xctx, (size_t)XA_MAX_ROWS * d.n_heads * dm));
+    RC(dalloc(e, &w.xpart, (size_t)XA_MAX_CHUNKS * d.n_heads * dm)); RC(dalloc(e, &w.xstat, (size_t)XA_MAX_CHUNKS * d.n_heads * 2));
+    HIPCHK(e, hipHostMalloc((void**)&w.idx.pin, IX_N_CACHED * DecIndex::PIN_INTS * sizeof(int), hipHostMallocDefault));
+    HIPCHK(e, hipHostMalloc((void**)&pp.pin_off, rk_engine::PairPass::RING * (Pc + 1) * sizeof(int), hipHostMallocDefault));
+    for (hipEvent_t& ev : pp.ev_off) HIPCHK(e, hipEventCreateWithFlags(&ev, hipEventDisableTiming));
+    HIPCHK(e, hipEventCreateWithFlags(&pp.ev_join, hipEventDisableTiming));
+    pp.ok = true;
+  }
   const int dec_smem_max = (int)attn_dec_lds(std::max(d.max_tokens, d.max_dec_len));
   (void)hipFuncSetAttribute((const void*)attn_dec_kernel, hipFuncAttributeMaxDynamicSharedMemorySize, std::min(dec_smem_max, 160 * 1024));
   (void)hipFuncSetAttribute((const void*)attn_dec_seq_kernel, hipFuncAttributeMaxDynamicSharedMemorySize, 160 * 1024);
@@ -1882,6 +2011,7 @@
   if (!e || !out_logits || slot < 0 || slot >= RK_SLOTS) return RK_ERR_INVALID;
   Slot& sl = e->slots[slot];
   if (n_floats > sl.last_floats) return fail(e, RK_ERR_INVALID, "asked for %d floats, have %d", n_floats, sl.last_floats);
+  if (int frc = flush_pending(e, slot)) return frc;
   if (sl.dec_pending) { HIPCHK(e, hipEventSynchronize(sl.ev_dec)); sl.dec_pending = false; }
   memcpy(out_logits, sl.h_scores, (size_t)n_floats * sizeof(float));
   return RK_OK;
@@ -1890,6 +2020,7 @@
 
 int rk_t5_scores_device_ptr(rk_engine* e, void** out_ptr) {
   if (!e || !out_ptr) return RK_ERR_INVALID;
+  if (int frc = flush_pending(e, 0)) return frc;
   *out_ptr = e->slots[0].d_scores;
   return RK_OK;
 }
@@ -1899,6 +2030,7 @@
 int rk_t5_score(rk_engine* e, const int32_t* tokens, const int32_t* seq_offsets, int n_seq, const int32_t* dec_prefix,
                 int dec_len, const int32_t* out_token_ids, int n_out, float* out_logits) {
   int rc;
+  if (e && (rc = flush_pending(e))) return rc;
   if ((rc = rk_t5_stage(e, tokens, seq_offsets, n_seq))) return rc;
   if ((rc = rk_t5_score_staged(e, dec_prefix, dec_len, out_token_ids, n_out))) return rc;
   return rk_t5_read_scores(e, out_logits, n_seq * n_out);
@@ -1912,6 +2044,7 @@
 int rk_t5_compare(rk_engine* e, const int32_t* tokens, const int32_t* seq_offsets, int n_pairs, int dec_start_id, int false_id,
                   int true_id, float* out_logits, float* out_p_true, int32_t* out_first_wins) {
   if (!e) return RK_ERR_INVALID;
+  if (int frc = flush_pending(e)) return frc;
   if (n_pairs <= 0 || n_pairs > (1 << 28) || !out_logits || !out_p_true || !out_first_wins) return fail(e, RK_ERR_INVALID, "empty compare (n_pairs=%d)", n_pairs);
   const int n_seq = 2 * n_pairs;
   int rc;
@@ -1952,6 +2085,7 @@
 int rk_t5_qlm(rk_engine* e, const int32_t* tokens, const int32_t* seq_offsets, int n_seq, const int32_t* labels,
               int n_labels, float* out_scores) {
   int rc;
+  if (e && (rc = flush_pending(e))) return rc;
   if (e && wide_heads(e)) return refuse_wide(e, "rk_t5_qlm", "qlm scores several decoder positions");
   if ((rc = rk_t5_stage(e, tokens, seq_offsets, n_seq))) return rc;
   Slot& sl = e->slots[0];
@@ -1968,6 +2102,7 @@
 int rk_t5_qlm_many(rk_engine* e, const int32_t* tokens, const int32_t* seq_offsets, int n_seq, const int32_t* labels,
                    const int32_t* label_offsets, float* out_scores) {
   if (!e) return RK_ERR_INVALID;
+  if (int frc = flush_pending(e)) return frc;
   if (e->family != 0) return fail(e, RK_ERR_STATE, "T5 entry point called on a Llama engine (use rk_llama_*)");
   if (wide_heads(e)) return refuse_wide(e, "rk_t5_qlm_many", "qlm scores several decoder positions");
   int rc;
@@ -2080,6 +2215,7 @@
 int rk_t5_greedy(rk_engine* e, const int32_t* tokens, const int32_t* seq_offsets, int n_seq, const int32_t* dec_prefix,
                  int dec_len, int max_new, int eos_id, int pad_id, int32_t* out_tokens, int32_t* out_steps) {
   int rc;
+  if (e && (rc = flush_pending(e))) return rc;
   if (e && wide_heads(e)) return refuse_wide(e, "rk_t5_greedy", "greedy decoding runs the decoder self-attention");
   if ((rc = rk_t5_stage(e, tokens, seq_offsets, n_seq))) return rc;
   Slot& sl = e->slots[0];
@@ -2122,6 +2258,7 @@
 int rk_t5_generate(rk_engine* e, const int32_t* tokens, const int32_t* seq_offsets, int n_seq, const int32_t* dec_prefix,
                    int dec_len, int max_new, int eos_id, int pad_id, int32_t* out_tokens, int32_t* out_steps) {
   int rc;
+  if (e && (rc = flush_pending(e))) return rc;
   if (e && wide_heads(e)) return refuse_wide(e, "rk_t5_generate", "cached decoding runs the decoder self-attention");
   if ((rc = rk_t5_stage(e, tokens, seq_offsets, n_seq))) return rc;
   Slot& sl = e->slots[0];
@@ -2161,6 +2298,7 @@
 int rk_t5_greedy2(rk_engine* e, const int32_t* tokens, const int32_t* seq_offsets, int n_seq, const int32_t* dec_prefix,
                   int dec_len, const int32_t* cand_ids, int n_cand, int eos_id, int pad_id, int32_t* out_tokens, int32_t* out_steps) {
   if (!e) return RK_ERR_INVALID;
+  if (int frc = flush_pending(e)) return frc;
   if (wide_heads(e)) return refuse_wide(e, "rk_t5_greedy2", "greedy decoding runs the decoder self-attention");
   const int Ld = dec_len + 1;
   const long per_seq = (long)dec_len + n_cand;
@@ -2792,6 +2930,7 @@
   if (!e || !id_bytes || n_bytes != RK_COMM_ID_BYTES) return fail(e, RK_ERR_INVALID, "bad unique id");
   if (world < 1 || rank < 0 || rank >= world || max_floats_per_rank <= 0) return fail(e, RK_ERR_INVALID, "bad rank %d / world %d / capacity %d", rank, world, max_floats_per_rank);
   if (!e->finalized) return fail(e, RK_ERR_STATE, "engine not finalized");
+  if (int frc = flush_pending(e)) return frc;
   int rc = set_device(e);
   if (rc) return rc;
   const RcclApi* r = rccl_api();
@@ -2838,6 +2977,7 @@
   if (n_floats <= 0 || (size_t)n_floats > e->gather_cap || (size_t)n_floats > e->scores_cap) return fail(e, RK_ERR_CAPACITY, "n_floats %d out of range (capacity %zu, score buffer %zu)", n_floats, e->gather_cap, e->scores_cap);
   int rc = set_device(e);
   if (rc) return rc;
+  if ((rc = flush_pending(e, slot))) return rc;
   Slot& sl = e->slots[slot];
   hipStream_t sd = dec_stream(e, sl);
   if (e->gather_pending[slot]) { HIPCHK(e, hipEventSynchronize(e->ev_gather[slot])); e->gather_pending[slot] = false; }
@@ -2866,6 +3006,7 @@
   int rc = set_device(e);
   if (rc) return rc;
   if (n_floats == 0) return RK_OK;
+  if ((rc = flush_pending(e, slot))) return rc;
   Slot& sl = e->slots[slot];
   hipStream_t sd = dec_stream(e, sl);
   if (e->gall_pending) { HIPCHK(e, hipEventSynchronize(e->ev_gall)); e->gall_pending = false; }
@@ -2917,6 +3058,7 @@
 
 int rk_comm_destroy(rk_engine* e) {
   if (!e) return RK_ERR_INVALID;
+  if (int frc = flush_pending(e)) return frc;
   if (set_device(e) == RK_OK) sync_all(e);
   comm_release(e);
   return RK_OK;
@@ -2924,6 +3066,7 @@
 
 int rk_timer_begin(rk_engine* e) {
   if (!e) return RK_ERR_INVALID;
+  if (int frc = flush_pending(e)) return frc;
   int rc = set_device(e);
   if (rc) return rc;
   hipStream_t s0 = e->slots[0].se;
@@ -2937,6 +3080,7 @@
 
 int rk_timer_end(rk_engine* e, float* out_ms) {
   if (!e || !out_ms) return RK_ERR_INVALID;
+  if (int frc = flush_pending(e)) return frc;
   int rc = set_device(e);
   if (rc) return rc;
   hipStream_t s0 = e->slots[0].se;
@@ -2950,10 +3094,16 @@
   return RK_OK;
 }
 
-int rk_profile_enable(rk_engine* e, int on) { if (!e) return RK_ERR_INVALID; e->prof_on = on != 0; return RK_OK; }
+int rk_profile_enable(rk_engine* e, int on) {
+  if (!e) return RK_ERR_INVALID;
+  if (int frc = flush_pending(e)) return frc;
+  e->prof_on = on != 0;
+  return RK_OK;
+}
 
 int rk_profile_reset(rk_engine* e) {
   if (!e) return RK_ERR_INVALID;
+  if (int frc = flush_pending(e)) return frc;
   int rc = set_device(e);
   if (rc) return rc;
   if ((rc = sync_all(e))) return rc;
@@ -2964,6 +3114,7 @@
 
 int rk_profile_get(rk_engine* e, int cls, double* total_ms, int64_t* launches, double* flops, double* bytes) {
   if (!e || cls < 0 || cls >= PC_COUNT) return RK_ERR_INVALID;
+  if (int frc = flush_pending(e)) return frc;
   int rc = set_device(e);
   if (rc) return rc;
   if ((rc = sync_all(e))) return rc;
@@ -3016,6 +3167,7 @@
   {"dec_cached_attn", &rk_engine::Options::dec_cached_attn, 0, 1, nullptr, "rk_t5_generate's self-attention: attn_dec_cached_kernel (1) or the cache append + attn_dec_kernel's tree form (0); same bits"},
   {"llama_dec_r", &rk_engine::Options::llama_dec_r, 0, 2, nullptr, "rk_llama_generate's attention: query heads per workgroup by plan_llama_dec_attn's rule (0), one (1), or, where a kv head has 7, all seven (2: measurement and tests; every cached K / V byte read once per step); same bits"},
   {"enc_serial", &rk_engine::Options::enc_serial, 0, 1, nullptr, "two slots: an encoder chain starts behind the other slot's (1: one encoder at a time beside the decoder before it) or as soon as it is enqueued (0: two chains interleave); same bits"},
+  {"dec_pair", &rk_engine::Options::dec_pair, 0, 1, nullptr, "one-position rk_t5_score launches on the two slots back to back: ONE decoder pass over both slots' sequences (1) or each launch's own decoder at once (0); same bits"},
   {"gemm_split", &rk_engine::Options::gemm_split, 0, 1, nullptr, "rows beyond the ping-pong kernel's last whole round on a fill-in tile variant (1) or one launch (0); same bits"},
 #ifdef RK_MEASURE
   {"attn_ko", &rk_engine::Options::attn_ko, 0, 1 << 20, nullptr, "timing-only knock-outs of the attention kernels (measurement builds)"},
@@ -3037,6 +3189,7 @@
 
 int rk_engine_set_option(rk_engine* e, const char* key, int value) {
   if (!e || !key) return RK_ERR_INVALID;
+  if (int frc = flush_pending(e)) return frc;
   if (!strcmp(key, "overlap")) {
     if (value < 0 || value > 1) return fail(e, RK_ERR_INVALID, "option overlap: 0..1");
     if (set_device(e) || sync_all(e)) return RK_ERR_HIP;
@@ -3066,6 +3219,7 @@
 
 int rk_debug_gemm_ex(rk_engine* e, rk_debug_gemm_call* q) {
   if (!e || !q) return RK_ERR_INVALID;
+  if (int frc = flush_pending(e)) return frc;
   int rc = set_device(e);
   if (rc) return rc;
   const int epi = q->epi, M = q->M, N = q->N, K = q->K, batch = q->batch > 0 ? q->batch : 1;
@@ -3162,6 +3316,7 @@
 
 int rk_debug_gemm_chain(rk_engine* e, rk_debug_gemm_chain_call* q) {
   if (!e || !q) return RK_ERR_INVALID;
+  if (int frc = flush_pending(e)) return frc;
   int rc = set_device(e);
   if (rc) return rc;
   const int epi = q->epi, M = q->M, N = q->N, K = q->K, nl = q->n_launch;
@@ -3274,6 +3429,7 @@
 
 int rk_debug_attn(rk_engine* e, rk_debug_attn_call* q) {
   if (!e || !q) return RK_ERR_INVALID;
+  if (int frc = flush_pending(e)) return frc;
   int rc = set_device(e);
   if (rc) return rc;
   if (!e->finalized) return fail(e, RK_ERR_STATE, "debug attn: engine not finalized");
@@ -3506,6 +3662,7 @@
 
 int rk_debug_xattn_chain(rk_engine* e, rk_debug_xattn_chain_call* q) {
   if (!e || !q) return RK_ERR_INVALID;
+  if (int frc = flush_pending(e)) return frc;
   int rc = set_device(e);
   if (rc) return rc;
   if (!e->finalized) return fail(e, RK_ERR_STATE, "debug xattn chain: engine not finalized");
@@ -3646,6 +3803,7 @@
 
 int rk_debug_rows(rk_engine* e, rk_debug_rows_call* q) {
   if (!e || !q) return RK_ERR_INVALID;
+  if (int frc = flush_pending(e)) return frc;
   int rc = set_device(e);
   if (rc) return rc;
   const int op = q->op, rows = q->rows, d = q->d;
@@ -3901,6 +4059,7 @@
 
 int rk_debug_gemm(rk_engine* e, const uint16_t* A, const uint16_t* W, float* C, int M, int N, int K, int use_glds) {
   if (!e || !A || !W || !C) return RK_ERR_INVALID;
+  if (int frc = flush_pending(e)) return frc;
   if (K % 64 || N % 4) return fail(e, RK_ERR_INVALID, "debug gemm needs K%%64==0 and N%%4==0");
   if (M <= 0) return RK_OK;
   rk_debug_gemm_call q{};
@@ -3921,6 +4080,7 @@
 
 int rk_debug_gemm_bench(rk_engine* e, int M, int N, int K, int epi, int iters, float* out_ms) {
   if (!e || !out_ms || M <= 0 || N <= 0 || K <= 0 || iters <= 0) return RK_ERR_INVALID;
+  if (int frc = flush_pending(e)) return frc;
   int rc = set_device(e);
   if (rc) return rc;
   if (K % 64 || N % 4) return fail(e, RK_ERR_INVALID, "gemm bench needs K%%64==0 and N%%4==0");
@@ -3962,6 +4122,7 @@
 
 int rk_debug_graph_stats(rk_engine* e, rk_debug_graph_stats_t* out) {
   if (!e || !out) return RK_ERR_INVALID;
+  if (int frc = flush_pending(e)) return frc;
   int ready = 0;
   for (const auto& kv : e->graphs) ready += kv.second.exec != nullptr;
   const auto& n = e->graph_count;
@@ -3972,6 +4133,7 @@
 
 int rk_debug_buffers(rk_engine* e, rk_debug_buffers_t* out) {
   if (!e || !out) return RK_ERR_INVALID;
+  if (int frc = flush_pending(e)) return frc;
   int i = 0;
   auto put = [&](const auto& b) { out->addr[i] = (uint64_t)(uintptr_t)b.p; out->cap[i] = (uint64_t)b.cap; ++i; };
   put(e->logits); put(e->amax_val); put(e->amax_idx); put(e->kv_cache); put(e->gen_buf); put(e->lkv); put(e->lpart); put(e->lints);
@@ -3982,6 +4144,7 @@
 
 int rk_debug_sample(rk_engine* e, rk_debug_sample_call* q) {
   if (!e || !q) return RK_ERR_INVALID;
+  if (int frc = flush_pending(e)) return frc;
   if (q->rows <= 0 || q->rows > (1 << 20) || q->logit_rows <= 0 || q->logit_rows > q->rows || q->V <= 0 || q->V > sampling::MAX_VOCAB)
     return fail(e, RK_ERR_INVALID, "rk_debug_sample: rows %d (1 .. 2^20), logit_rows %d (1 .. rows), V %d (1 .. %d)", q->rows, q->logit_rows, q->V, sampling::MAX_VOCAB);
   if (!q->logits || !q->seeds || !q->index || !q->out_token) return fail(e, RK_ERR_INVALID, "rk_debug_sample: null logits, seeds, index or out_token");
@@ -4019,6 +4182,7 @@
 
 int64_t rk_debug_read(rk_engine* e, const char* name, float* out, int64_t max_floats) {
   if (!e || !name || !out) return RK_ERR_INVALID;
+  if (flush_pending(e)) return RK_ERR_HIP;
   if (set_device(e)) return RK_ERR_HIP;
   if (sync_all(e)) return RK_ERR_HIP;
   if (!strcmp(name, "occupancy")) {
```

Measured after the change: 7772, median of 6. Within noise of the previous version (+0.3%).
